# QizhiPei/FABind

Measured on AMD Instinct MI355X. Metric: complexes/sec fwd+bwd (1500p/40l nodes), full IaBNet on the whole graph (pocket model + 4-layer complex model + distance-map head on all nodes / pairs) with the pocket-cls + pocket-centre + coord + distmap + distmap-by-coords + distill losses (BASELINE configs[2] read literally), higher is better.
Workload: dtype bf16

## Files before the change

### fabind_amd/_lib.py

```python
import ctypes
import os

import torch

from . import config as _cfg

_HERE = os.path.dirname(os.path.abspath(__file__))
LIB_PATH = _cfg.knob("FABIND_LIB") or os.path.join(_HERE, "libfabind_hip.so")

ABI_VERSION = 19
DT_F32, DT_BF16 = 0, 1
ACT_NONE, ACT_SILU, ACT_RELU, ACT_SIGMOID, ACT_STORED_DERIV = 0, 1, 2, 3, 4
GEMM_FAM_NT_F32, GEMM_FAM_NT_F32_BF16, GEMM_FAM_NT_BF16, GEMM_FAM_GLDS, GEMM_FAM_PIPE, GEMM_FAM_X3, GEMM_FAM_X3_PRO, GEMM_FAM_PERSIST = range(8)

LNR_8S16, LNR_8S32, LNR_V8_1, LNR_V8_2, LNR_V8_3, LNR_V8_4, LNR_S2, LNR_S8, LNR_S16, LNR_S32, LNR_COUNT = range(11)
LNB_8S16, LNB_8S32, LNB_V8_1, LNB_V8_2, LNB_V8_3, LNB_S2, LNB_S8, LNB_S16, LNB_S20, LNB_S32, LNB_COUNT = range(11)
RST_BF16_1, RST_BF16_2, RST_BF16_4, RST_GENERIC, RST_COUNT = range(5)
ELF_WAVE1, ELF_WAVE1_TAIL, ELF_WAVE2_TAIL, ELF_CHUNK, ELF_COUNT = range(5)
ELB_NPL1, ELB_NPL2, ELB_NPL3, ELB_COUNT = range(4)

_vp, _i, _f, _l = ctypes.c_void_p, ctypes.c_int, ctypes.c_float, ctypes.c_long


class GemmArgs(ctypes.Structure):
    _fields_ = [(n, _vp) for n in ("A", "A2", "W", "C", "bias", "R", "r_index", "dotvec", "dot_out", "aux", "groups", "C2")] + \
               [(n, _i) for n in ("M", "N", "K", "K1", "lda", "lda2", "ldw", "ldc", "ldr", "ldaux", "dot_ld",
                                  "a_dtype", "w_dtype", "c_dtype", "aux_dtype", "act_pro", "act_epi", "dact_epi",
                                  "accumulate", "store_preact", "n_groups", "max_m", "max_n", "groups_ext", "epi_fast", "k_splits")] + \
               [("alpha", _f), ("p_drop", _f), ("drop_seed", ctypes.c_uint)] + \
               [(n, _vp) for n in ("row_mu", "row_rs", "col_c", "C16")] + [("ldc16", _i), ("split3", _i), ("r_dtype", _i), ("c2_bf16", _i)]


class EdgeBwdArgs(ctypes.Structure):
    _fields_ = [(n, _vp) for n in ("AB", "row", "col", "rhohat", "w_r", "W2p", "Wcp", "W2Tp", "WcTp", "b2", "bc", "w3", "ds",
                                  "dagg", "S1", "Mm", "dT", "dP2", "dP1", "drh", "dABrow", "part", "dbg", "bnd", "d2scratch")] + \
               [(n, _i) for n in ("ldab", "lddagg", "lddab", "E")] + [("p_drop", _f), ("seed", ctypes.c_uint), ("xcd_aware", _i), ("lddab16", _i), ("dAB16", _vp),
                                                                  ("d2f", _vp), ("z3f", _vp)]


class PairUpdateArgs(ctypes.Structure):
    _fields_ = [(n, _vp) for n in ("T", "p_node", "c_node", "z_in", "z_out", "Wop", "bo", "ln_w", "ln_b", "W1p", "b1", "W2p", "b2",
                                  "Wbp", "bb", "bias_out")] + \
               [(n, _i) for n in ("ldt", "b_off", "n_pairs")] + [("eps", _f), ("p_drop", _f), ("seed", ctypes.c_uint)]


class TnJob(ctypes.Structure):
    _fields_ = [(n, _vp) for n in ("Y", "X", "C_part", "out", "out_tail")] + \
               [(n, _i) for n in ("ldy", "ldx", "M", "N", "E", "splits", "e_per", "n_tiles", "with_colsum", "out_dt", "ldo",
                                  "wg0", "n_wg", "blk0", "n_blk", "pad_")]


class AttnFusedBwdArgs(ctypes.Structure):
    _fields_ = [(n, _vp) for n in ("qg", "kv", "a0", "bo", "boT", "toff", "koff", "bconst", "desc", "desc_p", "out", "lse", "dout",
                                  "dqg", "dkv", "dO", "Dv", "da0", "acat", "colpart", "part")] + \
               [(n, _i) for n in ("ldq", "ldkv", "lda0", "ldda0", "ldacat", "kcol0", "ldcolpart", "kp")] + [("scale", _f)] + \
               [(n, _i) for n in ("nsplit", "B", "part_rows")]


class AdamRow(ctypes.Structure):
    _fields_ = [(n, _vp) for n in ("p", "g", "m", "v")] + [("numel", ctypes.c_longlong), ("chunk0", _i), ("step_idx", _i)] + \
               [(n, ctypes.c_double) for n in ("lr", "beta1", "beta2", "eps", "weight_decay")] + [("decoupled", _i), ("pad_", _i)]


SIGNATURES = {
    "fabind_gemm": [ctypes.POINTER(GemmArgs), _vp],
    "fabind_gemm_plan": [ctypes.POINTER(GemmArgs), ctypes.POINTER(_i), ctypes.POINTER(_i), ctypes.POINTER(_i)],
    "fabind_gemm_tn_multi": [_vp, _vp, _i, _vp, _i, _vp, _i, _vp, _vp],
    "fabind_gemm_tn": [_vp, _i, _vp, _i, _vp, _i, _i, _i, _i, _vp, _vp, _i, _i, _vp],
    "fabind_transpose_act": [_vp, _i, _i, _vp, _i, _i, _i, _i, _i, _vp],
    "fabind_colsum": [_vp, _i, _i, _vp, _i, _i, _i, _vp, _i, _vp],
    "fabind_edges_count": [_vp, _vp, _vp, _i, _i, _vp, _vp, _f, _f, _vp, _vp, _vp],
    "fabind_edges_fill": [_vp, _vp, _vp, _i, _i, _vp, _vp, _vp, _f, _f, _vp, _vp, _vp, _vp, _vp, _vp, _vp],
    "fabind_exclusive_scan": [_vp, _vp, _i, _vp],
    "fabind_inter_meta": [_vp, _vp, _i, _vp, _vp, _vp, _i, _vp, _vp, _vp, _vp, _vp, _vp],
    "fabind_edge_geom": [_vp, _vp, _vp, _vp, _vp, _i, _vp, _vp, _vp, _vp, _vp],
    "fabind_gcl_pre": [_vp, _i, _i, _i, _vp, _vp, _vp, _vp, _vp, _i, _i, _i, _vp, _vp],
    "fabind_gcl_edge_fused": [_vp, _i, _i, _vp, _vp, _vp, _vp, _vp, _vp, _vp, _vp, _vp, _i, _vp, _vp, _f, ctypes.c_uint, _vp, _vp, _vp],
    "fabind_gcl_edge_fused_train": [_vp, _i, _i, _vp, _vp, _vp, _vp, _vp, _vp, _vp, _vp, _vp, _i, _vp, _vp, _f, ctypes.c_uint, _vp, _vp, _vp, _vp, _vp, _vp],
    "fabind_gcl_edge_fused_x3": [_vp, _i, _i, _i, _vp, _vp, _vp, _vp, _vp, _vp, _vp, _vp, _vp, _vp, _vp, _i, _vp, _vp, _f, ctypes.c_uint, _vp, _vp],
    "fabind_gcl_edge_fused_x3_train": [_vp, _i, _i, _i, _vp, _vp, _vp, _vp, _vp, _vp, _vp, _vp, _vp, _vp, _vp, _i, _vp, _vp, _f, ctypes.c_uint, _vp, _vp, _vp, _vp, _vp],
    "fabind_gcl_edge_fused_bwd": [ctypes.POINTER(EdgeBwdArgs), _i, _i, _vp],
    "fabind_pair_update_fused": [ctypes.POINTER(PairUpdateArgs), _i, _vp],
    "fabind_gcl_edge_fused_bwd_set_tile": [_i],
    "fabind_gcl_edge_fused_bwd_tile": [],
    "fabind_gcl_edge_fused_bwd_set_variant": [_i],
    "fabind_gcl_edge_fused_set_variant": [_i],
    "fabind_gcl_edge_fused_variant": [],
    "fabind_gcl_edge_fused_bwd_variant": [],
    "fabind_gcl_edge_fused_bwd_variant_for": [_i],
    "fabind_row_stats": [_vp, _i, _i, _f, _i, _i, _vp, _vp, _vp],
    "fabind_layernorm_rows": [_vp, _i, _i, _vp, _vp, _f, _i, _i, _vp, _i, _i, _i, _vp],
    "fabind_edge_ln_concat": [_vp, _i, _i, _vp, _vp, _vp, _vp, _vp, _f, _i, _vp, _i, _i, _i, _vp],
    "fabind_edge_lnfold": [_vp, _i, _i, _i, _vp, _vp, _vp, _vp, _f, _vp, _vp, _vp, _vp, _i, _vp, _f, ctypes.c_uint, _vp],
    "fabind_edge_lnfold_bwd_blocks": [_i],
    "fabind_edge_lnfold_bwd": [_vp, _i, _i, _i, _vp, _vp, _vp, _vp, _f, _vp, _vp, _vp, _vp, _vp, _i, _f, _vp, _vp, _vp, _vp, _i, _vp],
    "fabind_layernorm_rows_form": [_vp, _i, _i, _vp, _i, _i],
    "fabind_layernorm_rows_bwd_form": [_vp, _i, _vp, _i, _vp, _i, _i],
    "fabind_row_stats_form": [_vp, _i, _i, _i],
    "fabind_edge_lnfold_form": [_i, _i, ctypes.POINTER(_i)],
    "fabind_edge_lnfold_blocks": [_i],
    "fabind_edge_lnfold_bwd_form": [_i, ctypes.POINTER(_i)],
    "fabind_inter_coord_fold_blocks": [_i],
    "fabind_inter_coord_fold": [_vp, _i, _i, _vp, _vp, _vp, _f, _f, _vp, _vp, _vp, _i, _vp, _f, ctypes.c_uint, _vp],
    "fabind_post_optimize": [_vp, _vp, _vp, _vp, _vp, _i, _i, _i, _i, _f, _vp, _vp, _vp, _vp],
    "fabind_distmap_generate": [_vp, _vp, _vp, _vp, _vp, _vp, _vp, _vp, _vp, _vp, _i, _i, _i, _i, _i, _i, _l, _i, _i, _i, _i,
                                _vp, _vp, _vp, _vp, _vp, _vp, _vp, _vp],
    "fabind_sym_automorphisms": [_vp, _vp, _vp, _vp, _i, _i, _i, _vp, _vp, _vp, _vp, _vp, _vp],
    "fabind_sym_score": [_vp, _i, _i, _vp, _vp, _vp, _vp, _vp, _i, _i, _vp, _vp, _vp, _vp, _vp, _vp],
    "fabind_pose_stats": [_vp, _vp, _vp, _i, _vp, _vp, _vp],
    "fabind_rank_loss_fwd": [_vp, _vp, _vp, _i, _i, _i, _vp, _vp, _vp, _vp],
    "fabind_multi_copy": [_vp, _i, _i, _vp],
    "fabind_adam_chunk": [],
    "fabind_multi_sqnorm": [_vp, _i, _i, _vp, _vp, _vp, _vp],
    "fabind_multi_adam": [_vp, _i, _i, _vp, _vp, _vp, _f, _i, _vp, _vp, _vp],
    "fabind_zero_empty_rows": [_vp, _i, _vp, _i, _i, _i, _vp, _i, _i, _vp],
    "fabind_split_sum": [_vp, _i, ctypes.c_long, _vp, _i, ctypes.c_long, _vp, _vp],
    "fabind_segment_sum": [_vp, _i, _i, _i, _vp, _vp, _i, _i, _i, _vp, _i, _vp, _i, _vp],
    "fabind_coord_update": [_vp, _vp, _vp, _i, _vp, _vp, _i, _i, _f, _vp, _vp, _vp],
    "fabind_cross_attn_fwd": [_vp, _i, _vp, _vp, _i, _vp, _i, _vp, _i, _i, _i, _vp, _i, _i, _f, _vp, _i, _vp, _i, _vp, _i,
                              _vp],
    "fabind_cross_attn_mfma_fwd": [_vp, _i, _vp, _vp, _i, _vp, _i, _vp, _i, _i, _i, _vp, _i, _i, _f, _vp, _i, _vp, _i, _vp, _i,
                                   _vp],
    "fabind_cross_attn_fused_fwd": [_vp, _i, _vp, _vp, _i, _vp, _i, _vp, _i, _vp, _vp, _vp, _vp, _i, _i, _i, _i, _i, _f, _vp, _i, _vp, _i, _vp, _vp],
    "fabind_cross_attn_fused_bwd": [ctypes.POINTER(AttnFusedBwdArgs), _i, _i, _i, _i, _i, _i, _vp],
    "fabind_pair_bot_pack": [_vp, _i, _vp, _i, _vp, _vp, _vp, _vp, _i, _vp, _i, _l, _vp],
    "fabind_pair_bo_pack": [_vp, _i, _vp, _i, _vp, _vp, _vp, _vp, _i, _vp, _i, _l, _vp],
    "fabind_cross_attn_mfma_bwd": [_vp, _i, _vp, _i, _vp, _i, _i, _i, _vp, _i, _i, _i, _f, _vp, _vp, _vp, _vp, _vp, _vp, _vp,
                                   _vp, _vp, _vp],
    "fabind_pair_bmat": [_vp, _i, _vp, _i, _i, _vp, _i, _vp, _i, _vp],
    "fabind_pair_hadamard": [_vp, _vp, _i, _i, _vp, _vp, _i, _i, _vp, _vp, _i, _vp, _i, _i, _vp],
    "fabind_inter_attn_fwd": [_vp, _i, _vp, _i, _i, _vp, _i, _vp, _vp, _vp, _vp, _vp, _vp, _vp, _i, _vp, _vp, _vp,
                              _vp, _f, _i, _vp, _vp, _vp, _vp, _vp, _vp, _vp],
    "fabind_inter_attn_fwd_rows": [_vp, _i, _vp, _i, _i, _vp, _i, _vp, _vp, _vp, _vp, _vp, _vp, _vp, _i, _vp, _vp, _vp,
                                   _vp, _f, _i, _vp, _vp, _vp, _vp, _vp, _vp, _vp, _i, _i, _vp],
    "fabind_layernorm_rows_bwd": [_vp, _i, _i, _vp, _vp, _i, _i, _f, _i, _i, _vp, _i, _i, _vp, _vp, _i, _vp],
    "fabind_edge_concat": [_vp, _i, _i, _vp, _vp, _vp, _i, _vp, _i, _i, _i, _vp],
    "fabind_las_step": [_vp, _vp, _vp, _vp, _vp, _vp, _vp, _i, _i, _f, _f, _vp, _vp, _vp],
    "fabind_select_rows": [_vp, _vp, _vp, _i, _i, _vp, _vp],
    "fabind_add": [_vp, _vp, _vp, _l, _vp],
    "fabind_mul_dact": [_vp, _i, _vp, _i, _i, _vp, _i, _l, _f, _vp],
    "fabind_mul_dact_colsum": [_vp, _i, _vp, _i, _i, _vp, _i, _i, _i, _vp, _vp, _i, _f, _vp],
    "fabind_drop_mix": [_vp, _vp, _vp, _l, _f, ctypes.c_uint, _vp],
    "fabind_drop_mix_bwd": [_vp, _vp, _vp, _l, _f, ctypes.c_uint, _vp],
    "fabind_mul_dropmask_colsum": [_vp, _i, _vp, _i, _i, _i, _f, ctypes.c_uint, _vp, _vp, _i, _vp],
    "fabind_rowdot_bwd": [_vp, _i, _vp, _i, _vp, _i, _i, _i, _vp, _vp, _vp, _i, _vp],
    "fabind_edge_geom_bwd": [_vp, _vp, _vp, _vp, _vp, _vp, _vp, _vp, _vp, _vp, _i, _i, _i, _vp, _vp, _vp, _vp],
    "fabind_gcl_pre_bwd": [_vp, _i, _i, _vp, _vp, _i, _vp, _vp, _vp, _i, _vp],
    "fabind_gather_dact": [_vp, _i, _vp, _vp, _i, _i, _vp, _i, _i, _i, _vp],
    "fabind_coord_update_bwd": [_vp, _vp, _vp, _i, _i, _f, _vp, _vp, _vp, _vp],
    "fabind_cross_attn_bwd": [_vp, _i, _vp, _i, _vp, _i, _i, _i, _vp, _i, _i, _i, _f, _vp, _vp, _vp, _vp, _vp, _vp, _vp,
                              _vp, _vp, _vp],
    "fabind_pair_bias_cat": [_vp, _i, _vp, _i, _i, _i, _vp, _i, _vp, _i, _vp, _vp, _i, _vp, _i, _vp, _vp],
    "fabind_batched_transpose_pad": [_vp, _i, _vp, _i, _i, _i, _i, _vp, _vp],
    "fabind_node_chain_fwd": [_vp, _i, _vp, _i, _vp, _vp, _vp, _vp, _vp, _vp, _i, _i, _vp, _i, _vp, _i, _vp, _i, _i, _i, _vp],
    "fabind_node_chain_x3_fwd": [_vp, _i, _vp, _i, _vp, _vp, _vp, _vp, _vp, _vp, _vp, _vp, _vp, _vp, _i, _i, _vp, _i, _vp, _i, _vp, _i, _vp, _i, _vp, _i,
                                 _i, _i, _vp],
    "fabind_rows_hadamard_bwd": [_vp, _i, _i, _vp, _i, _i, _vp, _vp, _vp, _i, _vp, _i, _vp],
    "fabind_pair_hadamard_bwd_grid": [_vp, _i, _i, _vp, _i, _i, _vp, _vp, _vp, _vp, _i, _vp, _i, _vp],
    "fabind_pair_hadamard_bwd_rows": [_vp, _i, _i, _vp, _i, _i, _vp, _i, _i, _vp, _vp, _vp, _vp, _i, _vp, _i, _vp, _i, _vp],
    "fabind_pair_hadamard_bwd": [_vp, _i, _i, _vp, _vp, _i, _i, _vp, _vp, _i, _i, _vp, _vp, _i, _vp, _vp, _i, _vp, _vp, _i,
                                 _vp],
    "fabind_inter_attn_bwd": [_vp, _i, _vp, _i, _i, _vp, _vp, _vp, _vp, _vp, _vp, _vp, _vp, _vp, _vp, _vp, _vp, _f, _i,
                              _vp, _vp, _vp, _vp, _vp, _vp, _vp, _vp, _vp, _vp, _i, _vp],
    "fabind_inter_attn_bwd_rows": [_vp, _i, _vp, _i, _i, _vp, _vp, _vp, _vp, _vp, _vp, _vp, _vp, _vp, _vp, _vp, _vp, _f, _i,
# ... 104 lines not shown
```

### fabind_amd/csrc/fused_common.h

```cpp
#pragma once
#include "common.h"

#define FE_BM 64
#define FE_PRIO(x) __builtin_amdgcn_s_setprio(x)

__device__ __forceinline__ float fe_sigmoid(float x) { return __builtin_amdgcn_rcpf(1.0f + __builtin_amdgcn_exp2f(-1.44269504f * x)); }
__device__ __forceinline__ float fe_silu(float x) { return x * fe_sigmoid(x); }

__device__ __forceinline__ uint32_t fe_hash(uint32_t x) {
    x ^= x >> 16; x *= 0x7feb352dU; x ^= x >> 15; x *= 0x846ca68bU; x ^= x >> 16;
    return x;
}
__device__ __forceinline__ float fe_keep(uint32_t seed, uint32_t e, uint32_t c, uint32_t H, uint32_t thr16, float scale) {
    const uint32_t h = fe_hash(seed + (e >> 1) * H + c);
    return (((e & 1u) ? (h >> 16) : (h & 0xffffu)) >= thr16) ? scale : 0.f;
}

__device__ __forceinline__ void unpack8(const uint4 u, float* f) {
    f[0] = __uint_as_float(u.x << 16); f[1] = __uint_as_float(u.x & 0xffff0000u);
    f[2] = __uint_as_float(u.y << 16); f[3] = __uint_as_float(u.y & 0xffff0000u);
    f[4] = __uint_as_float(u.z << 16); f[5] = __uint_as_float(u.z & 0xffff0000u);
    f[6] = __uint_as_float(u.w << 16); f[7] = __uint_as_float(u.w & 0xffff0000u);
}
__device__ __forceinline__ uint4 pack8(const float* f) {
// ... 279 lines not shown
__device__ __forceinline__ float fe_scan_runs64(const bf16_t* sX, const int* sRow, const float* sRh, int ne, bool head_cont,
                                                bool tail_cont, float* out, unsigned ld, float* bnd_tile, int c,
                                                bf16_t* out16 = nullptr, unsigned ld16 = 0, const bf16_t* sXlo = nullptr) {
    const int lane = threadIdx.x & 63;
    const int mine = sRow[lane], prev = sRow[max(lane - 1, 0)];
    const float rhl = WITH_RH ? sRh[lane] : 0.f;
    const unsigned long long m = __ballot(lane < ne && lane > 0 && mine != prev);
    const int c8 = c >> 3, c7 = c & 7;
    float v[64];
#pragma unroll
    for (int rw = 0; rw < 64; ++rw) v[rw] = bf16_to_f32(sX[rw * H + ((c8 ^ (rw & SWZ)) * 8) + c7]);
    if (sXlo) {
#pragma unroll
        for (int rw = 0; rw < 64; ++rw) v[rw] += bf16_to_f32(sXlo[rw * H + ((c8 ^ (rw & SWZ)) * 8) + c7]);
    }
    float run = 0.f, pwr = 0.f;
    int rs = 0;
    auto flush = [&](bool last) {
        if (rs == 0 && head_cont) bnd_tile[c] = run;
        else if (last && tail_cont) bnd_tile[H + c] = run;
        else {
            const unsigned node = (unsigned)__builtin_amdgcn_readlane(mine, rs);
            if (out) out[node * ld + c] = run;
            if (out16) out16[node * ld16 + c] = f32_to_bf16(run);
        }
    };
#pragma unroll
    for (int rw = 0; rw < 64; ++rw) {
        if (rw < ne) {
            if ((m >> rw) & 1ull) {
                flush(false);
                run = 0.f;
                rs = rw;
            }
            run += v[rw];
            if (WITH_RH) pwr += __builtin_bit_cast(float, __builtin_amdgcn_readlane(__builtin_bit_cast(int, rhl), rw)) * v[rw];
        }
    }
    if (ne > 0) flush(true);
    return pwr;
}

template <int BM>
__global__ void fe_boundary_fix_kernel(const int* __restrict__ row, int E, int H, const float* __restrict__ bnd, float* out,
                                       unsigned ld, bf16_t* out16 = nullptr, unsigned ld16 = 0) {
    const int t = blockIdx.x, e0 = t * BM, ne = min(BM, E - e0);
    if (ne <= 0 || e0 + ne >= E) return;
    const int r = row[e0 + ne - 1];
    if (row[e0 + ne] != r) return;
    if (row[e0] == r && e0 > 0 && row[e0 - 1] == r) return;
    for (int c = threadIdx.x; c < H; c += blockDim.x) {
        float sum = bnd[((size_t)t * 2 + 1) * H + c];
        for (int u = t + 1;; ++u) {
            const int f0 = u * BM, fn = min(BM, E - f0);
            sum += bnd[((size_t)u * 2) * H + c];
            const bool through = row[f0 + fn - 1] == r && f0 + fn < E && row[f0 + fn] == r;
            if (!through) break;
        }
        if (out) out[(unsigned)r * ld + c] = sum;
        if (out16) out16[(unsigned)r * ld16 + c] = f32_to_bf16(sum);
    }
}

__device__ __forceinline__ float fe3_row16_sum(float v) {
#define FE_DPP_ADD(ctrl_) v += __builtin_bit_cast(float, __builtin_amdgcn_update_dpp(0, __builtin_bit_cast(int, v), (ctrl_), 0xF, 0xF, true))
    FE_DPP_ADD(0xB1);
    FE_DPP_ADD(0x4E);
    FE_DPP_ADD(0x141);
    FE_DPP_ADD(0x140);
#undef FE_DPP_ADD
    return v;
}

typedef float fe_f2 __attribute__((ext_vector_type(2)));
__device__ __forceinline__ void fe3_silu_pair(const fe_f2 z, fe_f2& m, fe_f2& d) {
    const fe_f2 t = z * -1.44269504f;
    const fe_f2 o = fe_f2{__builtin_amdgcn_exp2f(t.x), __builtin_amdgcn_exp2f(t.y)} + 1.0f;
    const fe_f2 s = fe_f2{__builtin_amdgcn_rcpf(o.x), __builtin_amdgcn_rcpf(o.y)};
    m = z * s;
    d = s + (m - m * s);
}
__device__ __forceinline__ uint32_t fe3_pack(const fe_f2 v) { return pack2_bf16(v.x, v.y); }
__device__ __forceinline__ fe_f2 fe3_unpack(const uint32_t u) { return fe_f2{__uint_as_float(u << 16), __uint_as_float(u & 0xffff0000u)}; }

__device__ __forceinline__ uint4 fe3_bload16(const __amdgpu_buffer_rsrc_t rs, const unsigned voff, const unsigned soff) {
    const fe_u32x4_t v = __builtin_amdgcn_raw_buffer_load_b128(rs, (int)voff, (int)soff, 0);
    return make_uint4(v.x, v.y, v.z, v.w);
}
__device__ __forceinline__ void fe3_bstore16(const __amdgpu_buffer_rsrc_t rs, const unsigned voff, const unsigned soff, const uint4 v) {
    __builtin_amdgcn_raw_buffer_store_b128(fe_u32x4_t{v.x, v.y, v.z, v.w}, rs, (int)voff, (int)soff, 0);
}

struct FabindEdgeBwdArgs;
int fe_bwd3_launch(const FabindEdgeBwdArgs* a, int H, int bm, int n_groups, hipStream_t stream);
int fe_fwd3_launch(const float* AB, int ldab, int H, const int* row, const int* col, const float* rhohat, const float* w_r,
                   const void* W2ph, const void* W2pl, const float* b2, const void* Wcph, const void* Wcpl, const float* bc,
                   const float* w3, int E, float* agg, float* s_out, uint32_t thr16, float dscale, unsigned seed, float* bnd,
                   int xcd_aware, hipStream_t stream, void* Msave = nullptr, void* d2f = nullptr, void* z3f = nullptr);
int fe_fwd2_launch(const void* AB, int ldab, int H, const int* row, const int* col, const float* rhohat, const float* w_r,
                   const void* W2p, const float* b2, const void* Wcp, const float* bc, const float* w3, int E, float* agg,
                   float* s_out, uint32_t thr16, float dscale, unsigned seed, float* bnd, void* agg16, int xcd_aware, hipStream_t stream,
                   void* Msave = nullptr, void* d2f = nullptr, void* z3f = nullptr);
int fe_bwd4_launch(const FabindEdgeBwdArgs* a, int H, int n_groups, hipStream_t stream);
```

### fabind_amd/csrc/fused_edge.hip

```cpp
#include "common.h"
#include "fabind_hip.h"
#include "fused_common.h"

static int g_fe_xcd_aware = 1;
extern "C" void fabind_gcl_edge_fused_set_xcd_aware(int on) { g_fe_xcd_aware = on ? 1 : 0; }
static int g_fe_fwd_variant = 1;
extern "C" int fabind_gcl_edge_fused_set_variant(int v) {
    FB_REQUIRE(v == 1, "fabind_gcl_edge_fused_set_variant: 1 (row-wise / operand-swapped) is the only forward form built (variant 0 was retired in round 5)");
    g_fe_fwd_variant = v;
    return 0;
}
extern "C" int fabind_gcl_edge_fused_variant(void) { return g_fe_fwd_variant; }

static int fe_fwd_entry(const void* AB, int ldab, int H, const int* row, const int* col, const float* rhohat,
                        const float* w_r, const void* W2p, const float* b2, const void* Wcp, const float* bc,
                        const float* w3, int E, float* agg, float* s_out, float p_drop, unsigned seed,
                        float* bnd, void* agg16, void* Msave, void* d2f, void* z3f, hipStream_t stream) {
    if (E <= 0) return 0;
    FB_REQUIRE((Msave != nullptr) == (d2f != nullptr) && (Msave != nullptr) == (z3f != nullptr),
               "fabind_gcl_edge_fused_train: M, d2f and z3f come together");
    FB_REQUIRE(Msave == nullptr || g_fe_fwd_variant == 1, "fabind_gcl_edge_fused_train: the saving forward is the row-wise / operand-swapped kernel (variant 1)");
    FB_REQUIRE(bnd != nullptr, "fabind_gcl_edge_fused: bnd (ceil(E/64) x 2 x H floats of scratch) is required");
    FB_REQUIRE(p_drop >= 0.f && p_drop < 1.f, "fabind_gcl_edge_fused: p_drop in [0, 1)");
    const uint32_t thr16 = (uint32_t)(p_drop * 65536.0f + 0.5f);
    const float dscale = 1.0f / (1.0f - (float)thr16 / 65536.0f);
    FB_REQUIRE(H == 512 || H == 256 || H == 128 || H == 64, "fabind_gcl_edge_fused: H must be 64, 128, 256 or 512");
    FB_REQUIRE(ldab % 8 == 0, "fabind_gcl_edge_fused: ldab % 8");
    {
        const int rc = fe_fwd2_launch(AB, ldab, H, row, col, rhohat, w_r, W2p, b2, Wcp, bc, w3, E, agg, s_out, thr16, dscale, seed, bnd,
                                      agg16, g_fe_xcd_aware, stream, Msave, d2f, z3f);
        if (rc) return rc;
    }
    hipLaunchKernelGGL((fe_boundary_fix_kernel<FE_BM>), dim3((E + FE_BM - 1) / FE_BM), dim3(H < 256 ? H : 256), 0, stream, row, E, H,
                       bnd, agg, (unsigned)H, (bf16_t*)agg16, (unsigned)H);
    FB_CHECK_LAUNCH();
    return 0;
}

extern "C" int fabind_gcl_edge_fused(const void* AB, int ldab, int H, const int* row, const int* col, const float* rhohat,
                                     const float* w_r, const void* W2p, const float* b2, const void* Wcp, const float* bc,
                                     const float* w3, int E, float* agg, float* s_out, float p_drop, unsigned seed,
                                     float* bnd, void* agg16, hipStream_t stream) {
    return fe_fwd_entry(AB, ldab, H, row, col, rhohat, w_r, W2p, b2, Wcp, bc, w3, E, agg, s_out, p_drop, seed, bnd, agg16, nullptr, nullptr,
                        nullptr, stream);
}
extern "C" int fabind_gcl_edge_fused_train(const void* AB, int ldab, int H, const int* row, const int* col, const float* rhohat,
                                           const float* w_r, const void* W2p, const float* b2, const void* Wcp, const float* bc,
                                           const float* w3, int E, float* agg, float* s_out, float p_drop, unsigned seed,
                                           float* bnd, void* agg16, void* M, void* d2f, void* z3f, hipStream_t stream) {
    FB_REQUIRE(M != nullptr && d2f != nullptr && z3f != nullptr, "fabind_gcl_edge_fused_train: M, d2f, z3f are required");
    return fe_fwd_entry(AB, ldab, H, row, col, rhohat, w_r, W2p, b2, Wcp, bc, w3, E, agg, s_out, p_drop, seed, bnd, agg16, M, d2f, z3f, stream);
}

static int fe_x3_entry(const float* AB, int ldab, int n_rows, int H, const int* row, const int* col, const float* rhohat,
                       const float* w_r, const void* W2ph, const void* W2pl, const float* b2, const void* Wcph,
                       const void* Wcpl, const float* bc, const float* w3, int E, float* agg, float* s_out,
                       float p_drop, unsigned seed, float* bnd, void* Msave, void* d2f, void* z3f, hipStream_t stream) {
    if (E <= 0) return 0;
    FB_REQUIRE(bnd != nullptr, "fabind_gcl_edge_fused_x3: bnd (ceil(E/64) x 2 x H floats of scratch) is required");
    FB_REQUIRE(p_drop >= 0.f && p_drop < 1.f, "fabind_gcl_edge_fused_x3: p_drop in [0, 1)");
    FB_REQUIRE(H == 512 || H == 256 || H == 128 || H == 64, "fabind_gcl_edge_fused_x3: H must be 64, 128, 256 or 512");
    FB_REQUIRE(ldab % 4 == 0 && ((uintptr_t)AB & 15) == 0, "fabind_gcl_edge_fused_x3: AB must be 16-byte aligned with ldab % 4 == 0");
    FB_REQUIRE(n_rows >= 0 && (size_t)n_rows * (size_t)ldab * 4 < ((size_t)1 << 32), "fabind_gcl_edge_fused_x3: AB larger than 4 GiB (n_rows * ldab * 4 bytes): split the batch");
    const uint32_t thr16 = (uint32_t)(p_drop * 65536.0f + 0.5f);
    const float dscale = 1.0f / (1.0f - (float)thr16 / 65536.0f);
    const int rc = fe_fwd3_launch(AB, ldab, H, row, col, rhohat, w_r, W2ph, W2pl, b2, Wcph, Wcpl, bc, w3, E, agg, s_out, thr16, dscale,
                                  seed, bnd, g_fe_xcd_aware, stream, Msave, d2f, z3f);
    if (rc) return rc;
    hipLaunchKernelGGL((fe_boundary_fix_kernel<FE_BM>), dim3((E + FE_BM - 1) / FE_BM), dim3(H < 256 ? H : 256), 0, stream, row, E, H,
                       bnd, agg, (unsigned)H, (bf16_t*)nullptr, 0u);
    FB_CHECK_LAUNCH();
    return 0;
}
extern "C" int fabind_gcl_edge_fused_x3(const float* AB, int ldab, int n_rows, int H, const int* row, const int* col, const float* rhohat,
                                        const float* w_r, const void* W2ph, const void* W2pl, const float* b2, const void* Wcph,
                                        const void* Wcpl, const float* bc, const float* w3, int E, float* agg, float* s_out,
                                        float p_drop, unsigned seed, float* bnd, hipStream_t stream) {
    return fe_x3_entry(AB, ldab, n_rows, H, row, col, rhohat, w_r, W2ph, W2pl, b2, Wcph, Wcpl, bc, w3, E, agg, s_out, p_drop, seed, bnd,
                       nullptr, nullptr, nullptr, stream);
}
extern "C" int fabind_gcl_edge_fused_x3_train(const float* AB, int ldab, int n_rows, int H, const int* row, const int* col, const float* rhohat,
                                              const float* w_r, const void* W2ph, const void* W2pl, const float* b2, const void* Wcph,
                                              const void* Wcpl, const float* bc, const float* w3, int E, float* agg, float* s_out,
                                              float p_drop, unsigned seed, float* bnd, void* M, void* d2f, void* z3f, hipStream_t stream) {
    FB_REQUIRE(M != nullptr && d2f != nullptr && z3f != nullptr, "fabind_gcl_edge_fused_x3_train: M, d2f, z3f are required");
    return fe_x3_entry(AB, ldab, n_rows, H, row, col, rhohat, w_r, W2ph, W2pl, b2, Wcph, Wcpl, bc, w3, E, agg, s_out, p_drop, seed, bnd,
                       M, d2f, z3f, stream);
}

template <int H, int BM, bool DBG>
__global__ __launch_bounds__(H, (BM == 32 ? 4 : 2)) void gcl_edge_fused_bwd_kernel(const FabindEdgeBwdArgs p) {
    constexpr int TPE = H / BM;
    constexpr int CPT = BM / 8;
    constexpr int MI = BM / 16;
    extern __shared__ __attribute__((aligned(16))) unsigned char smem[];
    bf16_t* sX = (bf16_t*)smem;
    bf16_t* sY = sX + BM * H;
    int* sRow = (int*)(sY + BM * H);
    float* sDs = (float*)(sRow + BM);
    float* sRh = sDs + BM;
    const bf16_t* __restrict__ AB = (const bf16_t*)p.AB;
    const int tid = threadIdx.x, lane = tid & 63, wave = tid >> 6;
    const int fr = lane & 15, cq = lane >> 4;
    const int el = tid / TPE, cth = tid % TPE;
    const int n_tiles = (p.E + BM - 1) / BM;
    const uint32_t thr16 = (uint32_t)(p.p_drop * 65536.0f + 0.5f);
    const float dscale = 1.0f / (1.0f - (float)thr16 / 65536.0f);
    int cbase[2][2];
#pragma unroll
    for (int f0 = 0; f0 < 2; ++f0)
#pragma unroll
        for (int f2 = 0; f2 < 2; ++f2)
            cbase[f0][f2] = cq * 4 * H + (wave * 8 + (((cq & 1) ^ f2) << 2) + ((fr >> 3) ^ f0)) * 8 + (fr & 7);
#define FE_COFF(i, j, r) (cbase[(r) & 1][(j) >> 1] + ((i) * 16 + (r)) * H + ((((j) & 1) ^ ((r) >> 1)) * 16))
    long long tph[12] = {0, 0, 0, 0, 0, 0, 0, 0, 0, 0, 0, 0};
    long long tlast = 0;
#define FE_TICK(k_)                                                   \
    if constexpr (DBG) {                                              \
        const long long now_ = __builtin_readcyclecounter();         \
        tph[k_] += now_ - tlast;                                      \
        tlast = now_;                                                 \
    }
    float pb2[4] = {0.f, 0.f, 0.f, 0.f}, pbc[4] = {0.f, 0.f, 0.f, 0.f}, pw3[4] = {0.f, 0.f, 0.f, 0.f}, pwr = 0.f;

    uint4 pfa[CPT], pfb[CPT];
    const unsigned uld = (unsigned)p.ldab;
    auto fe_prefetch = [&](unsigned r, unsigned c) {
        const unsigned aoff = r * uld + cth * (CPT * 8), boff = c * uld + H + cth * (CPT * 8);
#pragma unroll
        for (int q = 0; q < CPT; ++q) {
            pfa[q] = *(const uint4*)(AB + (aoff + q * 8));
            pfb[q] = *(const uint4*)(AB + (boff + q * 8));
        }
    };
    int t_first, t_end, t_step;
    if (p.xcd_aware && (gridDim.x & 7) == 0) {
        const int tpx = (n_tiles + 7) / 8, xcd = blockIdx.x & 7;
        t_first = xcd * tpx + (int)(blockIdx.x >> 3);
        t_end = min(n_tiles, (xcd + 1) * tpx);
        t_step = (int)(gridDim.x >> 3);
    } else {
        t_first = blockIdx.x; t_end = n_tiles; t_step = gridDim.x;
    }
    unsigned ur = 0, uc = 0;
    if (t_first < t_end) {
        const int e0 = t_first * BM;
        if (el < min(BM, p.E - e0)) {
            ur = (unsigned)(p.row + e0)[(unsigned)el];
            uc = (unsigned)(p.col + e0)[(unsigned)el];
        }
    }
    fe_prefetch(ur, uc);

    for (int tile = t_first; tile < t_end; tile += t_step) {
        const int e0 = tile * BM;
        const int ne = min(BM, p.E - e0);
        int lz = 0;
        asm volatile("" : "+s"(lz));
        const float* w_r = p.w_r + lz;
        const float* b2 = p.b2 + lz;
        const float* bc = p.bc + lz;
        const float* w3 = p.w3 + lz;
        const bf16_t* W2p = (const bf16_t*)p.W2p + lz;
        const bf16_t* Wcp = (const bf16_t*)p.Wcp + lz;
        const bf16_t* W2Tp = (const bf16_t*)p.W2Tp + lz;
        const bf16_t* WcTp = (const bf16_t*)p.WcTp + lz;
        if constexpr (DBG) tlast = __builtin_readcyclecounter();
        const int* grow = p.row + e0;
        const int* gcol = p.col + e0;
        const float* grh = p.rhohat + e0;
// ... 171 lines not shown
                unpack8(pfa[q], fa);
                unpack8(pfb[q], fb);
                uint4* sp = (uint4*)&sX[el * H + (((cth * CPT + q) ^ (el & 7)) * 8)];
                unpack8(*sp, g);
                const float4 w0 = *(const float4*)(wp + q * 8), w1 = *(const float4*)(wp + q * 8 + 4);
                const float wv[8] = {w0.x, w0.y, w0.z, w0.w, w1.x, w1.y, w1.z, w1.w};
#pragma unroll
                for (int k = 0; k < 8; ++k) {
                    const float z = fa[k] + fb[k] + rh * wv[k], sg = fe_sigmoid(z);
                    g[k] *= sg * (1.0f + z * (1.0f - sg));
                    dot += g[k] * wv[k];
                }
                *sp = pack8(g);
            }
#pragma unroll
            for (int o = 1; o < TPE; o <<= 1) dot += __shfl_xor(dot, o, 64);
            if (cth == 0) (p.drh + e0)[(unsigned)el] = dot;
        }
        ur = nr; uc = nc;
        fe_prefetch(ur, uc);
        __syncthreads();
        FE_TICK(8)
        fe_tile_store<H>(sX, (bf16_t*)p.dP1, e0, ne, tid);
        FE_TICK(1)

        {
            const bool head_cont = e0 > 0 && p.row[e0 - 1] == sRow[0];
            const bool tail_cont = e0 + ne < p.E && p.row[e0 + ne] == sRow[ne - 1];
            pwr += fe_scan_rows<H, true, BM>(sX, sRow, sRh, ne, head_cont, tail_cont, p.dABrow, (unsigned)p.lddab,
                                             p.bnd + (size_t)tile * 2 * H, tid);
        }
        __syncthreads();
        FE_TICK(9)
    }
    if constexpr (DBG) {
        if (p.dbg && blockIdx.x == 0 && tid == 0)
            for (int k = 0; k < 12; ++k) ((long long*)p.dbg)[k] = tph[k];
    }

    float* part = p.part + (size_t)blockIdx.x * 4 * H;
#pragma unroll
    for (int j = 0; j < 4; ++j) {
        float a = pb2[j], b = pbc[j], c = pw3[j];
        a += __shfl_xor(a, 16, 64); a += __shfl_xor(a, 32, 64);
        b += __shfl_xor(b, 16, 64); b += __shfl_xor(b, 32, 64);
        c += __shfl_xor(c, 16, 64); c += __shfl_xor(c, 32, 64);
        if (cq == 0) {
            const int colj = wave * 64 + j * 16 + fr;
            part[colj] = a; part[H + colj] = b; part[2 * H + colj] = c;
        }
    }
    part[3 * H + tid] = pwr;
}

#undef FE_COFF
#undef FE_ROT4
#undef FE_ROT_ACC
#undef FE_ROT_D2
#undef FE_JADDR
#undef FE_LOFF
#undef FE_TICK

static int g_fe_bwd_bm = 64;
extern "C" int fabind_gcl_edge_fused_bwd_set_tile(int bm) {
    FB_REQUIRE(bm == 64, "fabind_gcl_edge_fused_bwd_set_tile: 64 edges per tile (the 32-edge build of the two-tile kernel was retired in round 5)");
    g_fe_bwd_bm = bm;
    return 0;
}
extern "C" int fabind_gcl_edge_fused_bwd_tile(void) { return g_fe_bwd_bm; }
static bool g_fe_bwd_variant_set = false;
static int g_fe_bwd_variant = 5;
extern "C" int fabind_gcl_edge_fused_bwd_set_variant(int v) {
    FB_REQUIRE(v == 0 || v == 5,
               "fabind_gcl_edge_fused_bwd_set_variant: 0 (two LDS tiles of 64 edges: the default for H <= 128) or 5 (row-wise, operand-swapped in-place tile + store wave: the recompute default above); variants 1-4 were knobs nobody reached and were retired in round 5");
    g_fe_bwd_variant = v;
    g_fe_bwd_variant_set = true;
    return 0;
}
extern "C" int fabind_gcl_edge_fused_bwd_variant(void) { return g_fe_bwd_variant; }
extern "C" int fabind_gcl_edge_fused_bwd_variant_for(int H) {
    return (!g_fe_bwd_variant_set && g_fe_bwd_variant == 5 && H <= 128) ? 0 : g_fe_bwd_variant;
}

extern "C" int fabind_gcl_edge_fused_bwd(const FabindEdgeBwdArgs* a_in, int H, int n_groups, hipStream_t stream) {
    FabindEdgeBwdArgs a_copy = *a_in;
    a_copy.xcd_aware = g_fe_xcd_aware;
    const FabindEdgeBwdArgs* a = &a_copy;
    if (a->E <= 0 || n_groups <= 0) return 0;
    FB_REQUIRE(H == 512 || H == 256 || H == 128 || H == 64, "fabind_gcl_edge_fused_bwd: H must be 64, 128, 256 or 512");
    FB_REQUIRE(a->ldab % 8 == 0, "fabind_gcl_edge_fused_bwd: ldab % 8");
    FB_REQUIRE(a->p_drop >= 0.f && a->p_drop < 1.f, "fabind_gcl_edge_fused_bwd: p_drop in [0, 1)");
    const int g_fe_bwd_variant = fabind_gcl_edge_fused_bwd_variant_for(H);
    if (a->d2f != nullptr || a->z3f != nullptr) {
        FB_REQUIRE(a->d2f != nullptr && a->z3f != nullptr, "fabind_gcl_edge_fused_bwd: d2f and z3f (saved by fabind_gcl_edge_fused_train) come together");
        return fe_bwd4_launch(a, H, n_groups, stream);
    }
    if (g_fe_bwd_variant == 5) return fe_bwd3_launch(a, H, 64, n_groups, stream);
    FB_REQUIRE(a->dAB16 == nullptr, "fabind_gcl_edge_fused_bwd: dAB16 (bf16 receiving-side sums) exists in variant 5 only");
    FB_REQUIRE(a->bnd != nullptr, "fabind_gcl_edge_fused_bwd: bnd (ceil(E / tile) x 2 x H floats of scratch) is required");
    const int BMr = g_fe_bwd_bm;
    const size_t lds = (size_t)2 * BMr * H * 2 + BMr * (sizeof(int) + 2 * sizeof(float));
#define FE_LAUNCH2(HH, BB)                                                                                         \
    do {                                                                                                           \
        static bool set_ = false;                                                                                  \
        if (!set_) { (void)hipFuncSetAttribute((const void*)gcl_edge_fused_bwd_kernel<HH, BB, false>, hipFuncAttributeMaxDynamicSharedMemorySize, (int)lds); set_ = true; } \
        hipLaunchKernelGGL((gcl_edge_fused_bwd_kernel<HH, BB, false>), dim3(n_groups), dim3(HH), lds, stream, *a);  \
    } while (0)
#define FE_LAUNCH(HH) FE_LAUNCH2(HH, 64)
    if (a->dbg != nullptr && H == 512) {
        static bool setd_ = false;
        if (!setd_) { (void)hipFuncSetAttribute((const void*)gcl_edge_fused_bwd_kernel<512, 64, true>, hipFuncAttributeMaxDynamicSharedMemorySize, (int)lds); }
        hipLaunchKernelGGL((gcl_edge_fused_bwd_kernel<512, 64, true>), dim3(n_groups), dim3(512), lds, stream, *a);
    } else
    if (H == 512) FE_LAUNCH(512); else if (H == 256) FE_LAUNCH(256); else if (H == 128) FE_LAUNCH(128); else FE_LAUNCH(64);
    hipLaunchKernelGGL((fe_boundary_fix_kernel<64>), dim3((a->E + 63) / 64), dim3(H < 256 ? H : 256), 0, stream, a->row, a->E, H,
                           a->bnd, a->dABrow, (unsigned)a->lddab);
#undef FE_LAUNCH
#undef FE_LAUNCH2
#undef FE_COFF
#undef FE_ROT4
#undef FE_ROT_ACC
#undef FE_ROT_D2
#undef FE_JADDR
#undef FE_LOFF
#undef FE_TICK
    FB_CHECK_LAUNCH();
    return 0;
}
```

### fabind_amd/csrc/fused_edge_bwd4.hip

```cpp
#include "common.h"
#include "fabind_hip.h"
#include "fused_common.h"

#ifndef FE4_E3_DB
#define FE4_E3_DB 0
#endif
#ifndef FE4_SCAN64
#define FE4_SCAN64 0
#endif
#ifndef FE4_P5_BATCH
#define FE4_P5_BATCH 4
#endif

#ifndef FE4_NT_LOADS
#define FE4_NT_LOADS 1
#endif
#if FE4_NT_LOADS
typedef unsigned fe_u32x2_nt_t __attribute__((ext_vector_type(2)));
__device__ __forceinline__ uint2 fe4_ldq(const bf16_t* p_) { const fe_u32x2_nt_t v = __builtin_nontemporal_load((const fe_u32x2_nt_t*)p_); return make_uint2(v.x, v.y); }
#else
__device__ __forceinline__ uint2 fe4_ldq(const bf16_t* p_) { return *(const uint2*)p_; }
#endif

template <int H>
__global__ __launch_bounds__(H, 4) void gcl_edge_fused_bwd4_kernel(const FabindEdgeBwdArgs p, const int xf) {
    constexpr int BM = FE_BM, MI = BM / 16;
    constexpr int NW = H / 64;
    constexpr int CH = H / 8;
    constexpr int EPW = 64 / CH;
    constexpr int EPI = NW * EPW;
    constexpr int NIT = BM / EPI;
    constexpr int SWZ = (H >= 128) ? 15 : 7;
    static_assert(BM <= H, "one thread per table row");
    extern __shared__ __attribute__((aligned(16))) unsigned char smem[];
    bf16_t* sX = (bf16_t*)smem;
    int* sTab = (int*)(sX + BM * H);
    float* sPart = (float*)(sTab + 8 * BM);
    const int tid = threadIdx.x, lane = tid & 63, wave = tid >> 6;
    const int fr = lane & 15, cq = lane >> 4;
    const int sub = lane / CH, ch = lane % CH;
    const int n_tiles = (p.E + BM - 1) / BM;
    int t_first, t_end, t_step;
    if (p.xcd_aware && (gridDim.x & 7) == 0) {
        const int tpx = (n_tiles + 7) / 8, xcd = blockIdx.x & 7;
        t_first = xcd * tpx + (int)(blockIdx.x >> 3);
        t_end = min(n_tiles, (xcd + 1) * tpx);
        t_step = (int)(gridDim.x >> 3);
    } else {
        t_first = blockIdx.x; t_end = n_tiles; t_step = gridDim.x;
    }
    for (int k = 0; k < 4; ++k) sPart[k * H + tid] = 0.f;
    const unsigned uld = (unsigned)p.ldab;
    const __amdgpu_buffer_rsrc_t rs_ab = fe_rsrc(const_cast<void*>(p.AB), 0xffffffffu);
    const __amdgpu_buffer_rsrc_t rs_dagg = fe_rsrc(const_cast<float*>(p.dagg), 0xffffffffu);
    const bf16_t* __restrict__ d2f = (const bf16_t*)p.d2f;
    const bf16_t* __restrict__ z3f = (const bf16_t*)p.z3f;
    const int cx = (wave * 8 + (cq >> 1)) ^ (fr & SWZ);
    const int lbase = fr * H + (cq & 1) * 4;
#define FE_OPAQUE(v_) asm volatile("" : "+v"(v_))
#define FE_QOFF(i, j) (lb_ + (i) * 16 * H + ((cx_ ^ ((j) * 2)) * 8))
#define FE_FOFF(i, j) (fbase + (size_t)((i) * 4 + (j)) * 256)
    const int fcol = wave * 64 + cq * 4;

    int tb_r = -1, tb_c = 0;
    float tb_d = 0.f, tb_h = 0.f;
    auto fetch_tables = [&](int tile) {
        const int e0 = tile * BM;
        const int ne = min(BM, p.E - e0);
        if (tid < BM) {
            const bool ok = tid < ne;
            const unsigned ge = (unsigned)(e0 + (ok ? tid : 0));
            const int r = p.row[ge], c = p.col[ge];
            const float d = p.ds[ge], h = p.rhohat[ge];
            tb_r = ok ? r : -1; tb_c = ok ? c : 0; tb_d = ok ? d : 0.f; tb_h = ok ? h : 0.f;
        }
    };
    auto commit_tables = [&](int hb) {
        int* tb = sTab + hb * 4 * BM;
        if (tid < BM) {
            tb[tid] = tb_r;
            tb[BM + tid] = tb_c;
            ((float*)tb)[2 * BM + tid] = tb_d;
            ((float*)tb)[3 * BM + tid] = tb_h;
        }
    };
    if (t_first < t_end) { fetch_tables(t_first); commit_tables(0); }
    __syncthreads();
    int hb = 0;

    for (int tile = t_first; tile < t_end; tile += t_step, hb ^= 1) {
        const int e0 = tile * BM;
        const int ne = min(BM, p.E - e0);
        const int* sRow = sTab + hb * 4 * BM;
        const int* sCol = sRow + BM;
        const float* sDs = (const float*)(sRow + 2 * BM);
        const float* sRh = (const float*)(sRow + 3 * BM);
        int lz = 0;
        asm volatile("" : "+s"(lz));
        const float* w_r = p.w_r + lz;
        const float* w3 = p.w3 + lz;
        const bf16_t* W2Tp = (const bf16_t*)p.W2Tp + lz;
        const bf16_t* WcTp = (const bf16_t*)p.WcTp + lz;
        int ln_ = lane;
        FE_OPAQUE(ln_);
        const size_t fbase = (((size_t)tile * NW + wave) * (MI * 4) * 64 + ln_) * 4;
        auto copy_out = [&](void* dst) {
            const __amdgpu_buffer_rsrc_t rs = fe_rsrc((bf16_t*)dst + (size_t)e0 * H, (unsigned)ne * H * 2);
            int t_ = tid;
            FE_OPAQUE(t_);
#pragma unroll
            for (int it = 0; it < BM * CH / H; ++it) {
                const int q = t_ + it * H;
                const int rw = q / CH, c8 = q % CH;
                const uint4 v = *(const uint4*)&sX[rw * H + ((c8 ^ (rw & SWZ)) * 8)];
                __builtin_amdgcn_raw_buffer_store_b128(fe_u32x4_t{v.x, v.y, v.z, v.w}, rs, (int)((rw * H + c8 * 8) * 2), 0,  2);
            }
        };

        {
            int cx_ = cx, lb_ = lbase;
            FE_OPAQUE(cx_); FE_OPAQUE(lb_);
            uint2 zq[4][MI];
#pragma unroll
            for (int j = 0; j < 4; ++j)
#pragma unroll
                for (int i = 0; i < MI; ++i) zq[j][i] = fe4_ldq(&z3f[FE_FOFF(i, j)]);
            float dsr[MI];
#pragma unroll
            for (int i = 0; i < MI; ++i) dsr[i] = sDs[i * 16 + fr];
            float4 wq4[4];
#pragma unroll
            for (int j = 0; j < 4; ++j) wq4[j] = *(const float4*)(w3 + fcol + j * 16);
#pragma unroll
            for (int j = 0; j < 4; ++j) {
                const fe_f2 w01 = fe_f2{wq4[j].x, wq4[j].y}, w23 = fe_f2{wq4[j].z, wq4[j].w};
                fe_f2 a3a = fe_f2{0.f, 0.f}, a3b = a3a, aca = a3a, acb = a3a;
#pragma unroll
                for (int i = 0; i < MI; ++i) {
                    fe_f2 m01, d01, m23, d23;
                    fe3_silu_pair(fe3_unpack(zq[j][i].x), m01, d01);
                    fe3_silu_pair(fe3_unpack(zq[j][i].y), m23, d23);
                    const fe_f2 t01 = (w01 * dsr[i]) * d01, t23 = (w23 * dsr[i]) * d23;
                    a3a += m01 * dsr[i]; a3b += m23 * dsr[i];
                    aca += t01; acb += t23;
                    *(uint2*)&sX[FE_QOFF(i, j)] = make_uint2(fe3_pack(t01), fe3_pack(t23));
                }
                float a3[4] = {a3a.x, a3a.y, a3b.x, a3b.y}, ac[4] = {aca.x, aca.y, acb.x, acb.y};
#pragma unroll
                for (int r = 0; r < 4; ++r) { a3[r] = fe3_row16_sum(a3[r]); ac[r] = fe3_row16_sum(ac[r]); }
                if (fr < 4) {
                    const float va = fr == 0 ? a3[0] : fr == 1 ? a3[1] : fr == 2 ? a3[2] : a3[3];
                    const float vc = fr == 0 ? ac[0] : fr == 1 ? ac[1] : fr == 2 ? ac[2] : ac[3];
                    sPart[2 * H + fcol + j * 16 + fr] += va;
                    sPart[1 * H + fcol + j * 16 + fr] += vc;
                }
                __builtin_amdgcn_sched_barrier(0);
            }
        }
        __syncthreads();

        if (!(xf & 1)) copy_out(p.dT);
        f32x4_t acc[MI][4];
        fe_zero(acc);
        if (!(xf & 8)) fe_gemm_rolled<H, MI, true, SWZ>(sX, WcTp, wave, lane, acc);
        __syncthreads();

        {
            int cx_ = cx, lb_ = lbase;
            FE_OPAQUE(cx_); FE_OPAQUE(lb_);
            float4 dg[FE4_E3_DB ? 2 : 1][MI];
            uint2 dq[FE4_E3_DB ? 2 : 1][MI];
            unsigned dgo[MI];
            float dgk[MI];
#pragma unroll
            for (int i = 0; i < MI; ++i) {
                const int rr = sRow[i * 16 + fr];
                dgk[i] = rr >= 0 ? 1.f : 0.f;
                dgo[i] = ((unsigned)max(rr, 0) * (unsigned)p.lddagg + fcol) * 4;
            }
            auto fetch_block = [&](int j, int slot) {
#pragma unroll
                for (int i = 0; i < MI; ++i) {
                    const uint4 v = fe3_bload16(rs_dagg, dgo[i], (unsigned)(j * 64));
                    dg[slot][i] = make_float4(__uint_as_float(v.x), __uint_as_float(v.y), __uint_as_float(v.z), __uint_as_float(v.w));
                    dq[slot][i] = fe4_ldq(&d2f[FE_FOFF(i, j)]);
                }
            };
            if (FE4_E3_DB) fetch_block(0, 0);
#pragma unroll
            for (int j = 0; j < 4; ++j) {
                if (FE4_E3_DB) { if (j < 3) fetch_block(j + 1, (j + 1) & 1); } else fetch_block(j, 0);
                fe_f2 a2a = fe_f2{0.f, 0.f}, a2b = a2a;
#pragma unroll
                for (int i = 0; i < MI; ++i) {
                    const float4 g4 = dg[FE4_E3_DB ? (j & 1) : 0][i];
                    const uint2 dd = dq[FE4_E3_DB ? (j & 1) : 0][i];
                    const fe_f2 p01 = (fe_f2{acc[i][j][0], acc[i][j][1]} + fe_f2{g4.x, g4.y} * dgk[i]) * fe3_unpack(dd.x);
                    const fe_f2 p23 = (fe_f2{acc[i][j][2], acc[i][j][3]} + fe_f2{g4.z, g4.w} * dgk[i]) * fe3_unpack(dd.y);
                    a2a += p01; a2b += p23;
                    *(uint2*)&sX[FE_QOFF(i, j)] = make_uint2(fe3_pack(p01), fe3_pack(p23));
                }
                float a2[4] = {a2a.x, a2a.y, a2b.x, a2b.y};
#pragma unroll
                for (int r = 0; r < 4; ++r) a2[r] = fe3_row16_sum(a2[r]);
                if (fr < 4) sPart[fcol + j * 16 + fr] += fr == 0 ? a2[0] : fr == 1 ? a2[1] : fr == 2 ? a2[2] : a2[3];
                __builtin_amdgcn_sched_barrier(0);
            }
        }
        __syncthreads();

        if (!(xf & 1)) copy_out(p.dP2);
        fe_zero(acc);
        if (!(xf & 8)) fe_gemm_rolled<H, MI, true, SWZ>(sX, W2Tp, wave, lane, acc);
        __syncthreads();
        {
            int cx_ = cx, lb_ = lbase;
            FE_OPAQUE(cx_); FE_OPAQUE(lb_);
#pragma unroll
            for (int j = 0; j < 4; ++j)
#pragma unroll
                for (int i = 0; i < MI; ++i)
                    *(uint2*)&sX[FE_QOFF(i, j)] = make_uint2(pack2_bf16(acc[i][j][0], acc[i][j][1]), pack2_bf16(acc[i][j][2], acc[i][j][3]));
        }
        __syncthreads();

        const bool has_next = tile + t_step < t_end;
        {
            int ch_ = ch, es_ = wave * EPW + sub;
            FE_OPAQUE(ch_); FE_OPAQUE(es_);
#define ch ch_
            fe_f2 wv2[4];
            {
                const float4 w0 = *(const float4*)(w_r + ch * 8), w1 = *(const float4*)(w_r + ch * 8 + 4);
                wv2[0] = fe_f2{w0.x, w0.y}; wv2[1] = fe_f2{w0.z, w0.w}; wv2[2] = fe_f2{w1.x, w1.y}; wv2[3] = fe_f2{w1.z, w1.w};
            }
            const __amdgpu_buffer_rsrc_t rs_s1 = fe_rsrc((bf16_t*)p.S1 + (size_t)e0 * H, (unsigned)ne * H * 2);
            const __amdgpu_buffer_rsrc_t rs_p1 = fe_rsrc((bf16_t*)p.dP1 + (size_t)e0 * H, (unsigned)ne * H * 2);
            constexpr int PB = (NIT % FE4_P5_BATCH == 0) ? FE4_P5_BATCH : NIT;
#pragma unroll
            for (int u0 = 0; u0 < NIT; u0 += PB) {
            uint4 ga[PB], gb[PB];
#pragma unroll
            for (int v = 0; v < PB; ++v) {
                const int e = (u0 + v) * EPI + es_;
                const unsigned r = (unsigned)max(sRow[e], 0), c = (unsigned)sCol[e];
                ga[v] = fe3_bload16(rs_ab, (r * uld + ch * 8) * 2, 0);
                gb[v] = fe3_bload16(rs_ab, (c * uld + H + ch * 8) * 2, 0);
            }
#pragma unroll
            for (int v = 0; v < PB; ++v) {
                const int u = v;
                const int e = (u0 + v) * EPI + es_;
                const float rh = sRh[e];
                uint4* sp = (uint4*)&sX[e * H + ((ch ^ (e & SWZ)) * 8)];
                const uint4 gs = *sp;
                const uint32_t ua[4] = {ga[u].x, ga[u].y, ga[u].z, ga[u].w}, ub[4] = {gb[u].x, gb[u].y, gb[u].z, gb[u].w};
                const uint32_t ug[4] = {gs.x, gs.y, gs.z, gs.w};
                uint32_t po[4], pg[4];
                fe_f2 dot2 = fe_f2{0.f, 0.f};
#pragma unroll
                for (int k = 0; k < 4; ++k) {
                    const fe_f2 z = fe3_unpack(ua[k]) + fe3_unpack(ub[k]) + wv2[k] * rh;
                    fe_f2 m, d;
                    fe3_silu_pair(z, m, d);
                    const fe_f2 g = fe3_unpack(ug[k]) * d;
                    dot2 += g * wv2[k];
                    po[k] = fe3_pack(m);
                    pg[k] = fe3_pack(g);
                }
                *sp = make_uint4(pg[0], pg[1], pg[2], pg[3]);
                const unsigned goff = (unsigned)(e * H + ch * 8) * 2;
                if (!(xf & 2)) {
                    __builtin_amdgcn_raw_buffer_store_b128(fe_u32x4_t{po[0], po[1], po[2], po[3]}, rs_s1, (int)goff, 0,  2);
                    __builtin_amdgcn_raw_buffer_store_b128(fe_u32x4_t{pg[0], pg[1], pg[2], pg[3]}, rs_p1, (int)goff, 0,  2);
                }
                float dot = dot2.x + dot2.y;
                if constexpr (CH >= 16) {
                    dot = fe3_row16_sum(dot);
#pragma unroll
                    for (int o = 16; o < CH; o <<= 1) dot += __shfl_xor(dot, o, 64);
                } else {
#pragma unroll
                    for (int o = 1; o < CH; o <<= 1) dot += __shfl_xor(dot, o, 64);
                }
                if (ch == 0 && e < ne) (p.drh + e0)[(unsigned)e] = dot;
            }
            }
#undef ch
        }
        __syncthreads();

        if (has_next) fetch_tables(tile + t_step);
        if (!(xf & 4)) {
            const bool head_cont = e0 > 0 && p.row[e0 - 1] == sRow[0];
            const bool tail_cont = e0 + ne < p.E && p.row[e0 + ne] == sRow[ne - 1];
#if FE4_SCAN64
            sPart[3 * H + tid] += fe_scan_runs64<H, true, SWZ>(sX, sRow, sRh, ne, head_cont, tail_cont, p.dAB16 ? nullptr : p.dABrow, (unsigned)p.lddab,
                                                              p.bnd + (size_t)tile * 2 * H, tid, (bf16_t*)p.dAB16, (unsigned)p.lddab16);
#else
            sPart[3 * H + tid] += fe_scan_rows<H, true, BM, SWZ>(sX, sRow, sRh, ne, head_cont, tail_cont, p.dAB16 ? nullptr : p.dABrow, (unsigned)p.lddab,
                                                                p.bnd + (size_t)tile * 2 * H, tid, (bf16_t*)p.dAB16, (unsigned)p.lddab16);
#endif
        }
        if (has_next) commit_tables(hb ^ 1);
        __syncthreads();
    }
    __syncthreads();
    float* part = p.part + (size_t)blockIdx.x * 4 * H;
    for (int k = 0; k < 4; ++k) part[k * H + tid] = sPart[k * H + tid];
#undef FE_QOFF
#undef FE_FOFF
#undef FE_OPAQUE
}

static int g_fe_bwd4_exp = 0;
extern "C" void fabind_gcl_edge_fused_bwd4_set_exp(int m) { g_fe_bwd4_exp = m; }

int fe_bwd4_launch(const FabindEdgeBwdArgs* a, int H, int n_groups, hipStream_t stream) {
    FB_REQUIRE(a->bnd != nullptr, "fabind_gcl_edge_fused_bwd: bnd (ceil(E / 64) x 2 x H floats of scratch) is required");
    FB_REQUIRE(a->lddagg % 4 == 0 && ((uintptr_t)a->dagg & 15) == 0, "fabind_gcl_edge_fused_bwd: dagg must be 16-byte aligned with lddagg % 4 == 0");
    const size_t lds = (size_t)FE_BM * H * 2 + (size_t)8 * FE_BM * sizeof(int) + (size_t)4 * H * sizeof(float);
#define FE_LAUNCH4(HH)                                                                                                \
    do {                                                                                                           \
        static bool set_ = false;                                                                                  \
        if (!set_) {                                                                                               \
            const hipError_t e_ = hipFuncSetAttribute((const void*)gcl_edge_fused_bwd4_kernel<HH>,                    \
                                                      hipFuncAttributeMaxDynamicSharedMemorySize, (int)lds);       \
            if (e_ != hipSuccess) { fabind_set_error(hipGetErrorString(e_)); return (int)e_; }                     \
            set_ = true;                                                                                           \
        }                                                                                                          \
        hipLaunchKernelGGL((gcl_edge_fused_bwd4_kernel<HH>), dim3(n_groups), dim3(HH), lds, stream, *a, g_fe_bwd4_exp); \
    } while (0)
    if (H == 512) FE_LAUNCH4(512); else if (H == 256) FE_LAUNCH4(256); else if (H == 128) FE_LAUNCH4(128); else FE_LAUNCH4(64);
#undef FE_LAUNCH4
    hipLaunchKernelGGL((fe_boundary_fix_kernel<64>), dim3((a->E + 63) / 64), dim3(H < 256 ? H : 256), 0, stream, a->row, a->E, H,
                       a->bnd, a->dAB16 ? nullptr : a->dABrow, (unsigned)a->lddab, (bf16_t*)a->dAB16, (unsigned)a->lddab16);
    FB_CHECK_LAUNCH();
    return 0;
}
```

### fabind_amd/csrc/fused_edge_fwd2.hip

```cpp
#include "common.h"
#include "fabind_hip.h"
#include "fused_common.h"

typedef float fw_f2 __attribute__((ext_vector_type(2)));
__device__ __forceinline__ fw_f2 fw_silu_pair(const fw_f2 z) {
    const fw_f2 t = z * -1.44269504f;
    const fw_f2 o = fw_f2{__builtin_amdgcn_exp2f(t.x), __builtin_amdgcn_exp2f(t.y)} + 1.0f;
    return z * fw_f2{__builtin_amdgcn_rcpf(o.x), __builtin_amdgcn_rcpf(o.y)};
}
__device__ __forceinline__ uint32_t fw_pack(const fw_f2 v) { return pack2_bf16(v.x, v.y); }
__device__ __forceinline__ fw_f2 fw_unpack(const uint32_t u) { return fw_f2{__uint_as_float(u << 16), __uint_as_float(u & 0xffff0000u)}; }

__device__ __forceinline__ void fw_silu_pair_d(const fw_f2 z, fw_f2& m, fw_f2& d) {
    const fw_f2 t = z * -1.44269504f;
    const fw_f2 o = fw_f2{__builtin_amdgcn_exp2f(t.x), __builtin_amdgcn_exp2f(t.y)} + 1.0f;
    const fw_f2 s = fw_f2{__builtin_amdgcn_rcpf(o.x), __builtin_amdgcn_rcpf(o.y)};
    m = z * s;
    d = s + (m - m * s);
}

#ifndef FW2_NT_SAVE
#define FW2_NT_SAVE 1
#endif
typedef unsigned fw_u32x2_t __attribute__((ext_vector_type(2)));
__device__ __forceinline__ void fw_stq(bf16_t* p_, uint32_t a, uint32_t b) {
#if FW2_NT_SAVE
    __builtin_nontemporal_store(fw_u32x2_t{a, b}, (fw_u32x2_t*)p_);
#else
    *(uint2*)p_ = make_uint2(a, b);
#endif
}

template <int H, bool DROP, bool SAVE>
__global__ __launch_bounds__(H, 4) void gcl_edge_fused2_kernel(const bf16_t* __restrict__ AB, int ldab, const int* __restrict__ row,
                                                            const int* __restrict__ col, const float* __restrict__ rhohat,
                                                            const float* __restrict__ w_r, const bf16_t* __restrict__ W2p,
                                                            const float* __restrict__ b2, const bf16_t* __restrict__ Wcp,
                                                            const float* __restrict__ bc, const float* __restrict__ w3, int E,
                                                            float* agg, float* s_out, uint32_t thr16, float dscale,
                                                            uint32_t seed, float* bnd, bf16_t* agg16, int xcd_aware,
                                                            bf16_t* __restrict__ Msave, bf16_t* __restrict__ d2f, bf16_t* __restrict__ z3f) {
    constexpr int BM = FE_BM, MI = BM / 16;
    constexpr int NW = H / 64;
    constexpr int CH = H / 8;
    constexpr int EPW = 64 / CH;
    constexpr int EPI = NW * EPW;
    constexpr int NIT = BM / EPI;
    constexpr int SWZ = (H >= 128) ? 15 : 7;
    extern __shared__ __attribute__((aligned(16))) unsigned char smem[];
    bf16_t* sX = (bf16_t*)smem;
    int* sRow = (int*)(sX + BM * H);
    int* sCol = sRow + BM;
    float* sRh = (float*)(sCol + BM);
    float* sDot = sRh + BM;
    const int tid = threadIdx.x, lane = tid & 63, wave = tid >> 6;
    const int fr = lane & 15, cq = lane >> 4;
    const int sub = lane / CH, ch = lane % CH;
    const int n_tiles = (E + BM - 1) / BM, tpx = (n_tiles + 7) / 8;
    const int tile = xcd_aware ? (int)((blockIdx.x & 7) * tpx + (blockIdx.x >> 3)) : (int)blockIdx.x;
    if ((xcd_aware && (int)(blockIdx.x >> 3) >= tpx) || tile >= n_tiles) return;
    const int e0 = tile * BM;
    const int ne = min(BM, E - e0);

    if (tid < BM) {
        const bool ok = tid < ne;
        const unsigned ge = (unsigned)(e0 + (ok ? tid : 0));
        const int r = row[ge], c = col[ge];
        const float h = rhohat[ge];
        sRow[tid] = ok ? r : -1;
        sCol[tid] = ok ? c : 0;
        sRh[tid] = ok ? h : 0.f;
    }
    __syncthreads();

    {
        const __amdgpu_buffer_rsrc_t rs_ab = fe_rsrc(const_cast<bf16_t*>(AB), 0xffffffffu);
        fw_f2 wv2[4];
        {
            const float4 w0 = *(const float4*)(w_r + ch * 8), w1 = *(const float4*)(w_r + ch * 8 + 4);
            wv2[0] = fw_f2{w0.x, w0.y}; wv2[1] = fw_f2{w0.z, w0.w}; wv2[2] = fw_f2{w1.x, w1.y}; wv2[3] = fw_f2{w1.z, w1.w};
        }
        fe_u32x4_t ga[NIT], gb[NIT];
#pragma unroll
        for (int u = 0; u < NIT; ++u) {
            const int e = u * EPI + wave * EPW + sub;
            const unsigned r = (unsigned)max(sRow[e], 0), c = (unsigned)sCol[e];
            ga[u] = __builtin_amdgcn_raw_buffer_load_b128(rs_ab, (int)((r * (unsigned)ldab + ch * 8) * 2), 0, 0);
            gb[u] = __builtin_amdgcn_raw_buffer_load_b128(rs_ab, (int)((c * (unsigned)ldab + H + ch * 8) * 2), 0, 0);
        }
#pragma unroll
        for (int u = 0; u < NIT; ++u) {
            const int e = u * EPI + wave * EPW + sub;
            const float rh = sRh[e];
            uint32_t po[4];
#pragma unroll
            for (int k = 0; k < 4; ++k) po[k] = fw_pack(fw_silu_pair(fw_unpack(ga[u][k]) + fw_unpack(gb[u][k]) + wv2[k] * rh));
            *(uint4*)&sX[e * H + ((ch ^ (e & SWZ)) * 8)] = e < ne ? make_uint4(po[0], po[1], po[2], po[3]) : make_uint4(0u, 0u, 0u, 0u);
        }
    }
    __syncthreads();

    const int cx = (wave * 8 + (cq >> 1)) ^ (fr & SWZ);
    const int lbase = fr * H + (cq & 1) * 4;
#define FW_QOFF(i, j) (lbase + (i) * 16 * H + ((cx ^ ((j) * 2)) * 8))
    const size_t fbase = (((size_t)tile * NW + wave) * (MI * 4) * 64 + lane) * 4;
#define FW_FOFF(i, j) (fbase + (size_t)((i) * 4 + (j)) * 256)
    const int fcol = wave * 64 + cq * 4;

    f32x4_t acc[MI][4];
    fe_zero(acc);
    fe_gemm_rolled<H, MI, true, SWZ>(sX, W2p, wave, lane, acc);
    float4 bq4[4];
#pragma unroll
    for (int j = 0; j < 4; ++j) bq4[j] = *(const float4*)(b2 + fcol + j * 16);
    __syncthreads();
#pragma unroll
    for (int j = 0; j < 4; ++j) {
        const fw_f2 b01 = fw_f2{bq4[j].x, bq4[j].y}, b23 = fw_f2{bq4[j].z, bq4[j].w};
#pragma unroll
        for (int i = 0; i < MI; ++i) {
            fw_f2 m01, m23, d01, d23;
            if constexpr (SAVE) {
                fw_silu_pair_d(fw_f2{acc[i][j][0], acc[i][j][1]} + b01, m01, d01);
                fw_silu_pair_d(fw_f2{acc[i][j][2], acc[i][j][3]} + b23, m23, d23);
            } else {
                m01 = fw_silu_pair(fw_f2{acc[i][j][0], acc[i][j][1]} + b01);
                m23 = fw_silu_pair(fw_f2{acc[i][j][2], acc[i][j][3]} + b23);
            }
            if constexpr (DROP) {
                const uint32_t ee = (uint32_t)(e0 + i * 16 + fr), cc = (uint32_t)(fcol + j * 16);
                const fw_f2 k01 = fw_f2{fe_keep(seed, ee, cc, H, thr16, dscale), fe_keep(seed, ee, cc + 1, H, thr16, dscale)};
                const fw_f2 k23 = fw_f2{fe_keep(seed, ee, cc + 2, H, thr16, dscale), fe_keep(seed, ee, cc + 3, H, thr16, dscale)};
                m01 *= k01; m23 *= k23;
                if constexpr (SAVE) { d01 *= k01; d23 *= k23; }
            }
            *(uint2*)&sX[FW_QOFF(i, j)] = make_uint2(fw_pack(m01), fw_pack(m23));
            if constexpr (SAVE) fw_stq(&d2f[FW_FOFF(i, j)], fw_pack(d01), fw_pack(d23));
        }
        __builtin_amdgcn_sched_barrier(0);
    }
    __syncthreads();
    if constexpr (SAVE) {
        const __amdgpu_buffer_rsrc_t rs_m = fe_rsrc(Msave + (size_t)e0 * H, (unsigned)ne * H * 2);
#pragma unroll
        for (int q = tid; q < BM * CH; q += H) {
            const int rw = q / CH, c8 = q % CH;
            const uint4 v = *(const uint4*)&sX[rw * H + ((c8 ^ (rw & SWZ)) * 8)];
            __builtin_amdgcn_raw_buffer_store_b128(fe_u32x4_t{v.x, v.y, v.z, v.w}, rs_m, (int)((rw * H + c8 * 8) * 2), 0,  2);
        }
    }

    {
        const bool head_cont = e0 > 0 && row[e0 - 1] == sRow[0];
        const bool tail_cont = e0 + ne < E && row[e0 + ne] == sRow[ne - 1];
        (void)fe_scan_runs64<H, false, SWZ>(sX, sRow, nullptr, ne, head_cont, tail_cont, agg, (unsigned)H, bnd + (size_t)tile * 2 * H, tid, agg16, (unsigned)H);
    }

    fe_zero(acc);
    fe_gemm_rolled<H, MI, true, SWZ>(sX, Wcp, wave, lane, acc);
    {
        fw_f2 da[MI], db[MI];
#pragma unroll
        for (int i = 0; i < MI; ++i) { da[i] = fw_f2{0.f, 0.f}; db[i] = da[i]; }
#pragma unroll
        for (int j = 0; j < 4; ++j) {
            const float4 bq = *(const float4*)(bc + fcol + j * 16), wq = *(const float4*)(w3 + fcol + j * 16);
            const fw_f2 b01 = fw_f2{bq.x, bq.y}, b23 = fw_f2{bq.z, bq.w}, w01 = fw_f2{wq.x, wq.y}, w23 = fw_f2{wq.z, wq.w};
#pragma unroll
            for (int i = 0; i < MI; ++i) {
                const fw_f2 z01 = fw_f2{acc[i][j][0], acc[i][j][1]} + b01, z23 = fw_f2{acc[i][j][2], acc[i][j][3]} + b23;
                da[i] += fw_silu_pair(z01) * w01;
                db[i] += fw_silu_pair(z23) * w23;
                if constexpr (SAVE) fw_stq(&z3f[FW_FOFF(i, j)], fw_pack(z01), fw_pack(z23));
            }
            __builtin_amdgcn_sched_barrier(0);
        }
#pragma unroll
        for (int i = 0; i < MI; ++i) {
            float t = (da[i].x + da[i].y) + (db[i].x + db[i].y);
            t += __shfl_xor(t, 16, 64);
            t += __shfl_xor(t, 32, 64);
            if (cq == 0) sDot[wave * BM + i * 16 + fr] = t;
        }
    }
    __syncthreads();
    if (tid < ne) {
        float s = 0.f;
#pragma unroll
        for (int w = 0; w < NW; ++w) s += sDot[w * BM + tid];
        s_out[e0 + tid] = s;
    }
#undef FW_QOFF
#undef FW_FOFF
}

int fe_fwd2_launch(const void* AB, int ldab, int H, const int* row, const int* col, const float* rhohat, const float* w_r,
                   const void* W2p, const float* b2, const void* Wcp, const float* bc, const float* w3, int E, float* agg,
                   float* s_out, uint32_t thr16, float dscale, unsigned seed, float* bnd, void* agg16, int xcd_aware, hipStream_t stream,
                   void* Msave, void* d2f, void* z3f) {
    const dim3 grid((((E + FE_BM - 1) / FE_BM + 7) / 8) * 8);
    const size_t lds = (size_t)FE_BM * H * 2 + 3 * FE_BM * sizeof(int) + (size_t)(H / 64) * FE_BM * sizeof(float);
#define FW_LAUNCH_(HH, DD, SS)                                                                                       \
    do {                                                                                                           \
        static bool set_ = false;                                                                                  \
        if (!set_) { (void)hipFuncSetAttribute((const void*)gcl_edge_fused2_kernel<HH, DD, SS>, hipFuncAttributeMaxDynamicSharedMemorySize, (int)lds); set_ = true; } \
        hipLaunchKernelGGL((gcl_edge_fused2_kernel<HH, DD, SS>), grid, dim3(HH), lds, stream, (const bf16_t*)AB, ldab, row, col, rhohat, \
                           w_r, (const bf16_t*)W2p, b2, (const bf16_t*)Wcp, bc, w3, E, agg, s_out, thr16, dscale, \
                           (uint32_t)seed, bnd, (bf16_t*)agg16, xcd_aware, (bf16_t*)Msave, (bf16_t*)d2f, (bf16_t*)z3f); \
    } while (0)
#define FW_LAUNCH(HH)                                                                  \
    do {                                                                               \
        if (Msave) { if (thr16) FW_LAUNCH_(HH, true, true); else FW_LAUNCH_(HH, false, true); } \
        else { if (thr16) FW_LAUNCH_(HH, true, false); else FW_LAUNCH_(HH, false, false); }    \
    } while (0)
    if (H == 512) FW_LAUNCH(512); else if (H == 256) FW_LAUNCH(256); else if (H == 128) FW_LAUNCH(128); else FW_LAUNCH(64);
#undef FW_LAUNCH
#undef FW_LAUNCH_
    return 0;
}
```

### fabind_amd/csrc/fused_edge_fwd3.hip

```cpp
#include "common.h"
#include "fabind_hip.h"
#include "fused_common.h"

typedef float f3_f2 __attribute__((ext_vector_type(2)));
__device__ __forceinline__ f3_f2 f3_silu_pair(const f3_f2 z) {
    const f3_f2 t = z * -1.44269504f;
    const f3_f2 o = f3_f2{__builtin_amdgcn_exp2f(t.x), __builtin_amdgcn_exp2f(t.y)} + 1.0f;
    return z * f3_f2{__builtin_amdgcn_rcpf(o.x), __builtin_amdgcn_rcpf(o.y)};
}

__device__ __forceinline__ void f3_silu_pair_d(const f3_f2 z, f3_f2& m, f3_f2& d) {
    const f3_f2 t = z * -1.44269504f;
    const f3_f2 o = f3_f2{__builtin_amdgcn_exp2f(t.x), __builtin_amdgcn_exp2f(t.y)} + 1.0f;
    const f3_f2 s = f3_f2{__builtin_amdgcn_rcpf(o.x), __builtin_amdgcn_rcpf(o.y)};
    m = z * s;
    d = s + (m - m * s);
}
__device__ __forceinline__ uint32_t f3_pack(const f3_f2 v) { return pack2_bf16(v.x, v.y); }
typedef unsigned f3_u32x2_t __attribute__((ext_vector_type(2)));
__device__ __forceinline__ void f3_stq(bf16_t* p_, uint32_t a, uint32_t b) { __builtin_nontemporal_store(f3_u32x2_t{a, b}, (f3_u32x2_t*)p_); }

template <int H, bool DROP, bool SAVE>
__global__ __launch_bounds__(H, 2) void gcl_edge_fused_x3_kernel(const float* __restrict__ AB, int ldab, const int* __restrict__ row,
                                                              const int* __restrict__ col, const float* __restrict__ rhohat,
                                                              const float* __restrict__ w_r, const bf16_t* __restrict__ W2ph,
                                                              const bf16_t* __restrict__ W2pl, const float* __restrict__ b2,
                                                              const bf16_t* __restrict__ Wcph, const bf16_t* __restrict__ Wcpl,
                                                              const float* __restrict__ bc, const float* __restrict__ w3, int E,
                                                              float* agg, float* s_out, uint32_t thr16, float dscale, uint32_t seed,
                                                              float* bnd, int xcd_aware, bf16_t* __restrict__ Msave,
                                                              bf16_t* __restrict__ d2f, bf16_t* __restrict__ z3f) {
    constexpr int BM = FE_BM, MI = BM / 16;
    constexpr int NW = H / 64;
    constexpr int CH = H / 8;
    constexpr int EPW = 64 / CH;
    constexpr int EPI = NW * EPW;
    constexpr int NIT = BM / EPI;
    constexpr int PB = 4;
    constexpr int SWZ = (H >= 128) ? 15 : 7;
    extern __shared__ __attribute__((aligned(16))) unsigned char smem[];
    bf16_t* sXh = (bf16_t*)smem;
    bf16_t* sXl = sXh + BM * H;
    int* sRow = (int*)(sXl + BM * H);
    int* sCol = sRow + BM;
    float* sRh = (float*)(sCol + BM);
    float* sDot = sRh + BM;
    const int tid = threadIdx.x, lane = tid & 63, wave = tid >> 6;
    const int fr = lane & 15, cq = lane >> 4;
    const int sub = lane / CH, ch = lane % CH;
    const int n_tiles = (E + BM - 1) / BM, tpx = (n_tiles + 7) / 8;
    const int tile = xcd_aware ? (int)((blockIdx.x & 7) * tpx + (blockIdx.x >> 3)) : (int)blockIdx.x;
    if ((xcd_aware && (int)(blockIdx.x >> 3) >= tpx) || tile >= n_tiles) return;
    const int e0 = tile * BM;
    const int ne = min(BM, E - e0);

    if (tid < BM) {
        const bool ok = tid < ne;
        const unsigned ge = (unsigned)(e0 + (ok ? tid : 0));
        const int r = row[ge], c = col[ge];
        const float h = rhohat[ge];
        sRow[tid] = ok ? r : -1;
        sCol[tid] = ok ? c : 0;
        sRh[tid] = ok ? h : 0.f;
    }
    __syncthreads();

    {
        const __amdgpu_buffer_rsrc_t rs_ab = fe_rsrc(const_cast<float*>(AB), 0xffffffffu);
        float wv[8];
        {
            const float4 w0 = *(const float4*)(w_r + ch * 8), w1 = *(const float4*)(w_r + ch * 8 + 4);
            wv[0] = w0.x; wv[1] = w0.y; wv[2] = w0.z; wv[3] = w0.w; wv[4] = w1.x; wv[5] = w1.y; wv[6] = w1.z; wv[7] = w1.w;
        }
#pragma unroll
        for (int b0 = 0; b0 < NIT; b0 += PB) {
            fe_u32x4_t ga[PB][2], gb[PB][2];
#pragma unroll
            for (int u = 0; u < PB; ++u) {
                const int e = (b0 + u) * EPI + wave * EPW + sub;
                const unsigned r = (unsigned)max(sRow[e], 0), c = (unsigned)sCol[e];
                const int oa = (int)((r * (unsigned)ldab + ch * 8) * 4), ob = (int)((c * (unsigned)ldab + H + ch * 8) * 4);
                ga[u][0] = __builtin_amdgcn_raw_buffer_load_b128(rs_ab, oa, 0, 0);
                ga[u][1] = __builtin_amdgcn_raw_buffer_load_b128(rs_ab, oa + 16, 0, 0);
                gb[u][0] = __builtin_amdgcn_raw_buffer_load_b128(rs_ab, ob, 0, 0);
                gb[u][1] = __builtin_amdgcn_raw_buffer_load_b128(rs_ab, ob + 16, 0, 0);
            }
#pragma unroll
            for (int u = 0; u < PB; ++u) {
                const int e = (b0 + u) * EPI + wave * EPW + sub;
                const float rh = sRh[e];
                uint32_t ph[4], pl[4];
#pragma unroll
                for (int k = 0; k < 4; ++k) {
                    const int q = k >> 1, w = (k & 1) * 2;
                    const f3_f2 a = f3_f2{__uint_as_float(ga[u][q][w]), __uint_as_float(ga[u][q][w + 1])};
                    const f3_f2 b = f3_f2{__uint_as_float(gb[u][q][w]), __uint_as_float(gb[u][q][w + 1])};
                    const f3_f2 m = f3_silu_pair(a + b + f3_f2{wv[2 * k], wv[2 * k + 1]} * rh);
                    fe_split2(m.x, m.y, ph[k], pl[k]);
                }
                const bool ok = e < ne;
                const int o = e * H + ((ch ^ (e & SWZ)) * 8);
                *(uint4*)&sXh[o] = ok ? make_uint4(ph[0], ph[1], ph[2], ph[3]) : make_uint4(0u, 0u, 0u, 0u);
                *(uint4*)&sXl[o] = ok ? make_uint4(pl[0], pl[1], pl[2], pl[3]) : make_uint4(0u, 0u, 0u, 0u);
            }
        }
    }
    __syncthreads();

    const int cx = (wave * 8 + (cq >> 1)) ^ (fr & SWZ);
    const int lbase = fr * H + (cq & 1) * 4;
#define F3_QOFF(i, j) (lbase + (i) * 16 * H + ((cx ^ ((j) * 2)) * 8))
    const int fcol = wave * 64 + cq * 4;
    const size_t fbase = (((size_t)tile * NW + wave) * (MI * 4) * 64 + lane) * 4;
#define F3_FOFF(i, j) (fbase + (size_t)((i) * 4 + (j)) * 256)

    f32x4_t acc[MI][4];
    fe_zero(acc);
    fe_gemm_x3<H, MI, SWZ>(sXh, sXl, W2ph, W2pl, wave, lane, acc);
    float4 bq4[4];
#pragma unroll
    for (int j = 0; j < 4; ++j) bq4[j] = *(const float4*)(b2 + fcol + j * 16);
    __syncthreads();
#pragma unroll
    for (int j = 0; j < 4; ++j) {
        const f3_f2 b01 = f3_f2{bq4[j].x, bq4[j].y}, b23 = f3_f2{bq4[j].z, bq4[j].w};
#pragma unroll
        for (int i = 0; i < MI; ++i) {
            f3_f2 m01, m23, d01, d23;
            if constexpr (SAVE) {
                f3_silu_pair_d(f3_f2{acc[i][j][0], acc[i][j][1]} + b01, m01, d01);
                f3_silu_pair_d(f3_f2{acc[i][j][2], acc[i][j][3]} + b23, m23, d23);
            } else {
                m01 = f3_silu_pair(f3_f2{acc[i][j][0], acc[i][j][1]} + b01);
                m23 = f3_silu_pair(f3_f2{acc[i][j][2], acc[i][j][3]} + b23);
            }
            if constexpr (DROP) {
                const uint32_t ee = (uint32_t)(e0 + i * 16 + fr), cc = (uint32_t)(fcol + j * 16);
                const f3_f2 k01 = f3_f2{fe_keep(seed, ee, cc, H, thr16, dscale), fe_keep(seed, ee, cc + 1, H, thr16, dscale)};
                const f3_f2 k23 = f3_f2{fe_keep(seed, ee, cc + 2, H, thr16, dscale), fe_keep(seed, ee, cc + 3, H, thr16, dscale)};
                m01 *= k01; m23 *= k23;
                if constexpr (SAVE) { d01 *= k01; d23 *= k23; }
            }
            if constexpr (SAVE) f3_stq(&d2f[F3_FOFF(i, j)], f3_pack(d01), f3_pack(d23));
            uint32_t h01, l01, h23, l23;
            fe_split2(m01.x, m01.y, h01, l01);
            fe_split2(m23.x, m23.y, h23, l23);
            *(uint2*)&sXh[F3_QOFF(i, j)] = make_uint2(h01, h23);
            *(uint2*)&sXl[F3_QOFF(i, j)] = make_uint2(l01, l23);
        }
        __builtin_amdgcn_sched_barrier(0);
    }
    __syncthreads();
    if constexpr (SAVE) {
        const __amdgpu_buffer_rsrc_t rs_m = fe_rsrc(Msave + (size_t)e0 * H, (unsigned)ne * H * 2);
#pragma unroll
        for (int q = tid; q < BM * CH; q += H) {
            const int rw = q / CH, c8 = q % CH;
            const uint4 v = *(const uint4*)&sXh[rw * H + ((c8 ^ (rw & SWZ)) * 8)];
            __builtin_amdgcn_raw_buffer_store_b128(fe_u32x4_t{v.x, v.y, v.z, v.w}, rs_m, (int)((rw * H + c8 * 8) * 2), 0,  2);
        }
    }

    {
        const bool head_cont = e0 > 0 && row[e0 - 1] == sRow[0];
        const bool tail_cont = e0 + ne < E && row[e0 + ne] == sRow[ne - 1];
        (void)fe_scan_runs64<H, false, SWZ>(sXh, sRow, nullptr, ne, head_cont, tail_cont, agg, (unsigned)H, bnd + (size_t)tile * 2 * H, tid,
                                            nullptr, 0u, sXl);
    }

    fe_zero(acc);
    fe_gemm_x3<H, MI, SWZ>(sXh, sXl, Wcph, Wcpl, wave, lane, acc);
    {
        f3_f2 da[MI], db[MI];
#pragma unroll
        for (int i = 0; i < MI; ++i) { da[i] = f3_f2{0.f, 0.f}; db[i] = da[i]; }
#pragma unroll
        for (int j = 0; j < 4; ++j) {
            const float4 bq = *(const float4*)(bc + fcol + j * 16), wq = *(const float4*)(w3 + fcol + j * 16);
            const f3_f2 b01 = f3_f2{bq.x, bq.y}, b23 = f3_f2{bq.z, bq.w}, w01 = f3_f2{wq.x, wq.y}, w23 = f3_f2{wq.z, wq.w};
#pragma unroll
            for (int i = 0; i < MI; ++i) {
                const f3_f2 z01 = f3_f2{acc[i][j][0], acc[i][j][1]} + b01, z23 = f3_f2{acc[i][j][2], acc[i][j][3]} + b23;
                da[i] += f3_silu_pair(z01) * w01;
                db[i] += f3_silu_pair(z23) * w23;
                if constexpr (SAVE) f3_stq(&z3f[F3_FOFF(i, j)], f3_pack(z01), f3_pack(z23));
            }
            __builtin_amdgcn_sched_barrier(0);
        }
#pragma unroll
        for (int i = 0; i < MI; ++i) {
            float t = (da[i].x + da[i].y) + (db[i].x + db[i].y);
            t += __shfl_xor(t, 16, 64);
            t += __shfl_xor(t, 32, 64);
            if (cq == 0) sDot[wave * BM + i * 16 + fr] = t;
        }
    }
    __syncthreads();
    if (tid < ne) {
        float s = 0.f;
#pragma unroll
        for (int w = 0; w < NW; ++w) s += sDot[w * BM + tid];
        s_out[e0 + tid] = s;
    }
#undef F3_QOFF
#undef F3_FOFF
}

int fe_fwd3_launch(const float* AB, int ldab, int H, const int* row, const int* col, const float* rhohat, const float* w_r,
                   const void* W2ph, const void* W2pl, const float* b2, const void* Wcph, const void* Wcpl, const float* bc,
                   const float* w3, int E, float* agg, float* s_out, uint32_t thr16, float dscale, unsigned seed, float* bnd,
                   int xcd_aware, hipStream_t stream, void* Msave, void* d2f, void* z3f) {
    const dim3 grid((((E + FE_BM - 1) / FE_BM + 7) / 8) * 8);
    const size_t lds = (size_t)2 * FE_BM * H * 2 + 3 * FE_BM * sizeof(int) + (size_t)(H / 64) * FE_BM * sizeof(float);
#define F3_LAUNCH_(HH, DD, SS)                                                                                     \
    do {                                                                                                           \
        static bool set_ = false;                                                                                  \
        if (!set_) { (void)hipFuncSetAttribute((const void*)gcl_edge_fused_x3_kernel<HH, DD, SS>, hipFuncAttributeMaxDynamicSharedMemorySize, (int)lds); set_ = true; } \
        hipLaunchKernelGGL((gcl_edge_fused_x3_kernel<HH, DD, SS>), grid, dim3(HH), lds, stream, AB, ldab, row, col, rhohat, w_r,  \
                           (const bf16_t*)W2ph, (const bf16_t*)W2pl, b2, (const bf16_t*)Wcph, (const bf16_t*)Wcpl, bc, w3, E, agg, \
                           s_out, thr16, dscale, (uint32_t)seed, bnd, xcd_aware, (bf16_t*)Msave, (bf16_t*)d2f, (bf16_t*)z3f); \
    } while (0)
#define F3_LAUNCH(HH)                                                                                              \
    do {                                                                                                           \
        if (Msave) { if (thr16) F3_LAUNCH_(HH, true, true); else F3_LAUNCH_(HH, false, true); }                    \
        else { if (thr16) F3_LAUNCH_(HH, true, false); else F3_LAUNCH_(HH, false, false); }                        \
    } while (0)
    if (H == 512) F3_LAUNCH(512); else if (H == 256) F3_LAUNCH(256); else if (H == 128) F3_LAUNCH(128); else F3_LAUNCH(64);
#undef F3_LAUNCH
#undef F3_LAUNCH_
    return 0;
}
```

### fabind_amd/kernels.py

```python
import ctypes

import numpy as np
import torch

from . import _lib
from . import config as _cfg
from ._lib import ACT_NONE, ACT_RELU, ACT_SIGMOID, ACT_SILU, ACT_STORED_DERIV, GemmArgs, check, dt_code, ptr, stream

__all__ = ["gemm", "colsum", "edges_count", "edges_fill", "exclusive_scan", "inter_meta",
           "edge_geom", "gcl_pre", "segment_sum", "coord_update", "cross_attn_fwd", "pair_bmat", "pair_hadamard",
           "inter_attn_fwd", "las_step", "select_rows", "ACT_NONE", "ACT_SILU", "ACT_RELU", "ACT_SIGMOID", "ACT_STORED_DERIV"]

GEMM_BN = 128
GEMM_DEFAULT_CONFIG = 13
PROFILE = None
PROFILE_ONLY = None


PROFILE_BYTES = {}
PROFILE_ALGO = {}


def _profiled(label, flops, fn, nbytes=0.0, algo=None):
    if PROFILE is None or (PROFILE_ONLY is not None and not label.startswith(PROFILE_ONLY)):
# ... 410 lines not shown
        assert W1.shape == (H, 2 * H) and W2.shape == (H, H)
        return pack_frag(W1[:, :H].contiguous()), pack_frag(W1[:, H:].contiguous()), pack_frag(W2), None
    assert W1.shape == (2 * H, H) and W2.shape == (H, 2 * H)
    return pack_frag(W1[:H].contiguous()), pack_frag(W1[H:].contiguous()), pack_frag(W2[:, :H].contiguous()), pack_frag(W2[:, H:].contiguous())


def node_chain_fwd(X1, X2, packs, b1, b2, act, kind, residual=None, want16=False):
    M, H = X1.shape
    assert X1.dtype == torch.bfloat16 and (X2 is None or X2.dtype == torch.bfloat16)
    out = torch.empty((M, H), dtype=torch.float32, device=X1.device)
    out16 = torch.empty((M, H), dtype=torch.bfloat16, device=X1.device) if want16 else None
    W1a, W1b, W2a, W2b = packs
    hidden = H if kind == 0 else 2 * H
    _profiled("fabind_node_chain_fwd kind=%d M=%d H=%d" % (kind, M, H), 2.0 * M * (2 * H * hidden),
              lambda: check(_lib.load().fabind_node_chain_fwd(
                  ptr(X1), _ld(X1), ptr(X2), _ld(X2) if X2 is not None else 0, ptr(W1a), ptr(W1b), ptr(b1), ptr(W2a), ptr(W2b), ptr(b2), act,
                  kind, ptr(residual), _ld(residual) if residual is not None else 0, ptr(out), _ld(out), ptr(out16),
                  H if want16 else 0, M, H, stream()), "fabind_node_chain_fwd"))
    return out, out16


def node_chain_x3_blocks(W1, W2, kind):
    H = W2.shape[0]
    if kind == 0:
        assert W1.shape == (H, 2 * H) and W2.shape == (H, H)
        return [W1[:, :H], W1[:, H:], W2, None]
    assert W1.shape == (2 * H, H) and W2.shape == (H, 2 * H)
    return [W1[:H], W1[H:], W2[:, :H], W2[:, H:]]


def node_chain_x3_pack_many(chains):
    ws, lo, slots = [], [], []
    for ci, (W1, W2, kind) in enumerate(chains):
        for bi, b_ in enumerate(node_chain_x3_blocks(W1, W2, kind)):
            if b_ is None:
                continue
            ws += [b_, b_]
            lo += [False, True]
            slots.append((ci, bi))
    packs = pack_frag_multi(ws, lo)
    out = [[None] * 8 for _ in chains]
    for k, (ci, bi) in enumerate(slots):
        out[ci][2 * bi], out[ci][2 * bi + 1] = packs[2 * k], packs[2 * k + 1]
    return [tuple(o) for o in out]


def node_chain_x3_pack(W1, W2, kind):
    H = W2.shape[0]
    if kind == 0:
        assert W1.shape == (H, 2 * H) and W2.shape == (H, H)
        blocks = (W1[:, :H], W1[:, H:], W2, None)
    else:
        assert W1.shape == (2 * H, H) and W2.shape == (H, 2 * H)
        blocks = (W1[:H], W1[H:], W2[:, :H], W2[:, H:])
    out = []
    for b_ in blocks:
        out.extend(pack_frag_split(b_.contiguous()) if b_ is not None else (None, None))
    return tuple(out)


def node_chain_x3_fwd(X1, X2, packs, b1, b2, act, kind, residual=None, want16=False, save=False):
    M, H = X1.shape
    assert X1.dtype == torch.float32 and (X2 is None or X2.dtype == torch.float32)
    out = torch.empty((M, H), dtype=torch.float32, device=X1.device)
    out16 = torch.empty((M, H), dtype=torch.bfloat16, device=X1.device) if want16 else None
    hidden = H if kind == 0 else 2 * H
    t16 = torch.empty((M, hidden), dtype=torch.bfloat16, device=X1.device) if save else None
    d16 = torch.empty((M, hidden), dtype=torch.bfloat16, device=X1.device) if (save and act == ACT_SILU) else None
    _profiled("fabind_node_chain_x3_fwd kind=%d M=%d H=%d" % (kind, M, H), 2.0 * M * (2 * H * hidden),
              lambda: check(_lib.load().fabind_node_chain_x3_fwd(
                  ptr(X1), _ld(X1), ptr(X2), _ld(X2) if X2 is not None else 0, *[ptr(t_) for t_ in packs[:4]], ptr(b1),
                  *[ptr(t_) for t_ in packs[4:]], ptr(b2), act, kind, ptr(residual), _ld(residual) if residual is not None else 0,
                  ptr(out), _ld(out), ptr(out16), H if want16 else 0, ptr(t16), hidden if save else 0, ptr(d16), hidden if d16 is not None else 0,
                  M, H, stream()), "fabind_node_chain_x3_fwd"))
    return (out, out16, t16, d16) if save else (out, out16)


def pack_frag_split(W):
    hi = W.to(torch.bfloat16)
    lo = (W.float() - hi.float()).to(torch.bfloat16)
    return pack_frag(hi), pack_frag(lo)


def gcl_edge_fused_x3(AB, H, row, col, rhohat, w_r, W2, b2, Wc, bc, w3, n_rows, p_drop=0.0, seed=0, rowptr=None, save=False):
    E = row.shape[0]
    if save and E > 0:
        nt = (E + 63) // 64
        Msave = torch.empty((E, H), dtype=torch.bfloat16, device=AB.device)
        d2f = torch.empty((nt * 64, H), dtype=torch.bfloat16, device=AB.device)
        z3f = torch.empty((nt * 64, H), dtype=torch.bfloat16, device=AB.device)
    else:
        save = False
    assert AB.dtype == torch.float32 and AB.stride(1) == 1
    alloc = torch.zeros if (rowptr is None or E == 0) else torch.empty
    agg = alloc((n_rows, H), dtype=torch.float32, device=AB.device)
    if alloc is torch.empty:
        zero_empty_rows(rowptr, agg, H)
    s = torch.empty((max(E, 1), 1), dtype=torch.float32, device=AB.device)
    bnd = torch.empty(((E + 63) // 64 * 2 + 2, H), dtype=torch.float32, device=AB.device)
    W2h, W2l = pack_frag_split(W2)
    Wch, Wcl = pack_frag_split(Wc)
    if save:
        _profiled("gcl_edge_fused_x3_kernel<%d> E=%d saving (gather + 2 chained H x H split-bf16 contractions + segment-sum per edge; M, silu'(pre2), pre3 kept)" % (H, E),
                  4.0 * E * H * H,
                  lambda: check(_lib.load().fabind_gcl_edge_fused_x3_train(ptr(AB), _ld(AB), AB.shape[0], H, ptr(row), ptr(col), ptr(rhohat), ptr(w_r),
                                                                           ptr(W2h), ptr(W2l), ptr(b2), ptr(Wch), ptr(Wcl), ptr(bc), ptr(w3), E,
                                                                           ptr(agg), ptr(s), float(p_drop), int(seed) & 0xFFFFFFFF, ptr(bnd),
                                                                           ptr(Msave), ptr(d2f), ptr(z3f), stream()), "fabind_gcl_edge_fused_x3_train"),
                  E * (6.0 * H + 16) + n_rows * (8.0 * H + 4.0 * H),
                  algo=2.0 * n_rows * H * 4 + E * 8.0 + n_rows * 24.0)
        return agg, s[:E], (Msave, d2f, z3f)
    _profiled("gcl_edge_fused_x3_kernel<%d> E=%d (gather + 2 chained H x H split-bf16 contractions + segment-sum per edge)" % (H, E),
              4.0 * E * H * H,
              lambda: check(_lib.load().fabind_gcl_edge_fused_x3(ptr(AB), _ld(AB), AB.shape[0], H, ptr(row), ptr(col), ptr(rhohat), ptr(w_r),
                                                                 ptr(W2h), ptr(W2l), ptr(b2), ptr(Wch), ptr(Wcl), ptr(bc), ptr(w3), E,
                                                                 ptr(agg), ptr(s), float(p_drop), int(seed) & 0xFFFFFFFF, ptr(bnd),
                                                                 stream()), "fabind_gcl_edge_fused_x3"),
              E * 16.0 + n_rows * (8.0 * H + 4.0 * H), algo=2.0 * n_rows * H * 4 + E * 8.0 + n_rows * 24.0)
    return agg, s[:E]


def zero_empty_rows(rowptr, out, C, out2=None):
    n_rows = rowptr.shape[0] - 1
    check(_lib.load().fabind_zero_empty_rows(ptr(rowptr), n_rows, ptr(out), dt_code(out.dtype), _ld(out), C, ptr(out2),
                                             dt_code(out2.dtype) if out2 is not None else 0, _ld(out2) if out2 is not None else 0,
                                             stream()), "fabind_zero_empty_rows")


def gcl_edge_fused(AB16, H, row, col, rhohat, w_r, W2p, b2, Wcp, bc, w3, n_rows, p_drop=0.0, seed=0, want16=False, rowptr=None, save=False):
    E = row.shape[0]
    if save and E > 0:
        nt = (E + 63) // 64
        Msave = torch.empty((E, H), dtype=torch.bfloat16, device=AB16.device)
        d2f = torch.empty((nt * 64, H), dtype=torch.bfloat16, device=AB16.device)
        z3f = torch.empty((nt * 64, H), dtype=torch.bfloat16, device=AB16.device)
    else:
        save, Msave, d2f, z3f = False, None, None, None
    alloc = torch.zeros if (rowptr is None or E == 0) else torch.empty
    agg = alloc((n_rows, H), dtype=torch.float32, device=AB16.device)
    agg16 = alloc((n_rows, H), dtype=torch.bfloat16, device=AB16.device) if want16 else None
    if alloc is torch.empty:
        zero_empty_rows(rowptr, agg, H, agg16)
    s = torch.empty((max(E, 1), 1), dtype=torch.float32, device=AB16.device)
    bnd = torch.empty(((E + 63) // 64 * 2 + 2, H), dtype=torch.float32, device=AB16.device)
    if save:
        _profiled("gcl_edge_fused_kernel<%d> E=%d saving (gather + 2 chained H x H contractions + segment-sum per edge; M, silu'(pre2), pre3 kept)" % (H, E),
                  4.0 * E * H * H,
                  lambda: check(_lib.load().fabind_gcl_edge_fused_train(ptr(AB16), _ld(AB16), H, ptr(row), ptr(col), ptr(rhohat), ptr(w_r),
                                                                        ptr(W2p), ptr(b2), ptr(Wcp), ptr(bc), ptr(w3), E, ptr(agg), ptr(s),
                                                                        float(p_drop), int(seed) & 0xFFFFFFFF, ptr(bnd), ptr(agg16),
                                                                        ptr(Msave), ptr(d2f), ptr(z3f), stream()),
                                "fabind_gcl_edge_fused_train"),
                  E * (6.0 * H + 16) + n_rows * (4.0 * H + 4.0 * H + (2.0 * H if want16 else 0.0)),
                  algo=2.0 * n_rows * H * 2 + E * 8.0 + n_rows * 24.0)
    else:
        _profiled("gcl_edge_fused_kernel<%d> E=%d (gather + 2 chained H x H contractions + segment-sum per edge)" % (H, E), 4.0 * E * H * H,
                  lambda: check(_lib.load().fabind_gcl_edge_fused(ptr(AB16), _ld(AB16), H, ptr(row), ptr(col), ptr(rhohat), ptr(w_r),
                                                                  ptr(W2p), ptr(b2), ptr(Wcp), ptr(bc), ptr(w3), E, ptr(agg), ptr(s),
                                                                  float(p_drop), int(seed) & 0xFFFFFFFF, ptr(bnd), ptr(agg16), stream()),
                                "fabind_gcl_edge_fused"),
                  E * 16.0 + n_rows * (4.0 * H + 4.0 * H + (2.0 * H if want16 else 0.0)),
                  algo=2.0 * n_rows * H * 2 + E * 8.0 + n_rows * 24.0)
    out = (agg, s[:E], agg16) if want16 else (agg, s[:E])
    return out + ((Msave, d2f, z3f),) if save else out


def edge_lnfold(AB16, Kp, H, row, col, rho, stat, eps, w_r, c_r, c_c, dvec, p_drop=0.0, seed=0):
    E = row.shape[0]
    out = torch.empty((E, Kp), dtype=torch.bfloat16, device=AB16.device)
    assert AB16.dtype == torch.bfloat16 and stat.dtype == torch.float32 and stat.is_contiguous()
    check(_lib.load().fabind_edge_lnfold(ptr(AB16), _ld(AB16), Kp, H, ptr(row), ptr(col), ptr(rho), ptr(stat), float(eps),
                                         ptr(w_r), ptr(c_r), ptr(c_c), ptr(dvec), E, ptr(out), float(p_drop), int(seed) & 0xFFFFFFFF,
                                         stream()), "fabind_edge_lnfold")
    return out


def edge_lnfold_bwd(AB16, Kp, H, row, col, rho, stat, eps, w_r, c_r, c_c, out, dout, p_drop=0.0):
    E = row.shape[0]
    dev = AB16.device
    if E == 0:
        return (torch.zeros((0, Kp), dtype=torch.bfloat16, device=dev), torch.zeros((0, 8), dtype=torch.float32, device=dev),
                torch.zeros(0, dtype=torch.float32, device=dev), torch.zeros((4, Kp), dtype=torch.float32, device=dev))
    lib = _lib.load()
    nb = max(1, int(lib.fabind_edge_lnfold_bwd_blocks(E)))
    du = torch.empty((max(E, 1), Kp), dtype=torch.bfloat16, device=dev)
    es = torch.empty((max(E, 1), 8), dtype=torch.float32, device=dev)
    drho = torch.empty(max(E, 1), dtype=torch.float32, device=dev)
    part = torch.empty((nb, 4 * Kp), dtype=torch.float32, device=dev)
    assert AB16.dtype == torch.bfloat16 and out.dtype == torch.bfloat16 and dout.dtype == torch.bfloat16 and dout.is_contiguous() and out.is_contiguous()
    check(lib.fabind_edge_lnfold_bwd(ptr(AB16), _ld(AB16), Kp, H, ptr(row), ptr(col), ptr(rho), ptr(stat), float(eps), ptr(w_r), ptr(c_r),
                                     ptr(c_c), ptr(out), ptr(dout), E, float(p_drop), ptr(du), ptr(es), ptr(drho), ptr(part), nb,
                                     stream()), "fabind_edge_lnfold_bwd")
    return du[:E], es[:E], drho[:E], colsum(part).view(4, Kp)


def inter_coord_fold(P16, H, col, rho, stat, q_w, eps, u, d, w3, p_drop=0.0, seed=0):
    E = col.shape[0]
    out = torch.empty(max(E, 1), dtype=torch.float32, device=P16.device)
    assert P16.dtype == torch.bfloat16 and stat.dtype == torch.float32 and stat.is_contiguous()
    check(_lib.load().fabind_inter_coord_fold(ptr(P16), _ld(P16), H, ptr(col), ptr(rho), ptr(stat), float(q_w), float(eps),
                                              ptr(u), ptr(d), ptr(w3), E, ptr(out), float(p_drop), int(seed) & 0xFFFFFFFF,
                                              stream()), "fabind_inter_coord_fold")
    return out[:E]


def row_stats(x, eps):
    R, C = x.shape
    mu = torch.empty(max(R, 1), dtype=torch.float32, device=x.device)
    rs = torch.empty(max(R, 1), dtype=torch.float32, device=x.device)
    check(_lib.load().fabind_row_stats(ptr(x), dt_code(x.dtype), _ld(x), float(eps), R, C, ptr(mu), ptr(rs), stream()),
          "fabind_row_stats")
    return mu, rs


def layernorm_rows_form(x, out, C=None, pad_to=None):
    C = x.shape[1] if C is None else C
    pad_to = out.shape[1] if pad_to is None else pad_to
    return int(_lib.load().fabind_layernorm_rows_form(ptr(x), _ld(x), C, ptr(out), _ld(out), pad_to))


def layernorm_rows_bwd_form(x, dy, dx, C=None):
    C = x.shape[1] if C is None else C
    return int(_lib.load().fabind_layernorm_rows_bwd_form(ptr(x), _ld(x), ptr(dy), _ld(dy), ptr(dx), _ld(dx), C))


def row_stats_form(x):
    return int(_lib.load().fabind_row_stats_form(ptr(x), dt_code(x.dtype), _ld(x), x.shape[1]))


def edge_lnfold_form(Kp, H):
    u = ctypes.c_int(0)
    lib = _lib.load()
    return int(lib.fabind_edge_lnfold_form(Kp, H, ctypes.byref(u))), u.value, int(lib.fabind_edge_lnfold_blocks(2 ** 31 - 1))


def edge_lnfold_bwd_form(Kp):
    u = ctypes.c_int(0)
    lib = _lib.load()
    return int(lib.fabind_edge_lnfold_bwd_form(Kp, ctypes.byref(u))), u.value, int(lib.fabind_edge_lnfold_bwd_blocks(2 ** 31 - 1))


def inter_coord_fold_blocks(E=2 ** 31 - 1):
    return int(_lib.load().fabind_inter_coord_fold_blocks(E))


def pair_update_fused(T, b_off, p_node, c_node, z, Wop, bo, ln_w, ln_b, eps, W1p, b1, W2p, b2, Wbp=None, bb=None, p_drop=0.0,
                      seed=0):
    n, H = z.shape
    assert z.dtype == torch.bfloat16 and z.is_contiguous() and T.dtype == torch.float32
    z_out = torch.empty_like(z)
    bias_out = torch.empty((max(n, 1), 16), dtype=torch.float32, device=z.device) if Wbp is not None else None
    a = _lib.PairUpdateArgs()
    for name, t in (("T", T), ("p_node", p_node), ("c_node", c_node), ("z_in", z), ("z_out", z_out), ("Wop", Wop), ("bo", bo),
                    ("ln_w", ln_w), ("ln_b", ln_b), ("W1p", W1p), ("b1", b1), ("W2p", W2p), ("b2", b2), ("Wbp", Wbp), ("bb", bb),
                    ("bias_out", bias_out)):
        setattr(a, name, ptr(t))
    a.ldt, a.b_off, a.n_pairs = _ld(T), int(b_off), n
    a.eps, a.p_drop, a.seed = float(eps), float(p_drop), int(seed) & 0xFFFFFFFF
    _profiled("pair_update_fused_kernel<%d> pairs=%d (Hadamard + LN + 2 chained H x H contractions + 16 biases)" % (H, n),
              2.0 * n * H * (2 * H + 32 + 16),
              lambda: check(_lib.load().fabind_pair_update_fused(ctypes.byref(a), H, stream()), "fabind_pair_update_fused"))
    return z_out, (bias_out[:n] if bias_out is not None else None)


_N_CU = {}
EDGE_BWD_GROUPS = 0
EDGE_BWD_TIMES = None


def gcl_edge_fused_bwd(AB16, H, row, col, rhohat, w_r, W2, b2, Wc, bc, w3, ds, dagg, colptr, perm, p_drop=0.0, seed=0,
                       dab_bf16=False, w_dtype=torch.float32, rowptr=None, frags=None, saved=None):
    E, N, dev = row.shape[0], AB16.shape[0], AB16.device
    ng = _N_CU.get(dev)
    if ng is None:
        ng = _N_CU[dev] = torch.cuda.get_device_properties(dev).multi_processor_count
    lib = _lib.load()
    variant = lib.fabind_gcl_edge_fused_bwd_variant_for(H)
    if saved is not None and E > 0:
        variant = 6
    bm = 64
    if variant == 6:
        per_cu = max(1, min(8, (160 * 1024) // (2 * bm * H + 16 * H + 32 * bm), 16 // max(1, H // 64)))
    elif variant == 5:
        per_cu = max(1, min(8, (160 * 1024) // (4 * bm * H + 16 * H + 32 * bm), 12 // (H // 64 + 1)))
    else:
        per_cu = max(1, min(8, (160 * 1024) // (4 * bm * H + 1024), 512 // H))
    ng = max(1, min(ng * per_cu, (E + bm - 1) // bm))
    if EDGE_BWD_GROUPS:
        ng = int(EDGE_BWD_GROUPS)
    if ng >= 8:
        ng -= ng % 8
    d2scratch = torch.empty((2, ng, bm * H), dtype=torch.bfloat16, device=dev) if variant == 5 else None
    bnd = torch.empty(((E + bm - 1) // bm * 2 + 2, H), dtype=torch.float32, device=dev)
    if variant == 6:
        buf = torch.empty((4, max(E, 1), H), dtype=torch.bfloat16, device=dev)
        S1, Mm, dT, dP2, dP1 = buf[0], saved[0], buf[1], buf[2], buf[3]
    else:
        buf = torch.empty((5, max(E, 1), H), dtype=torch.bfloat16, device=dev)
        S1, Mm, dT, dP2, dP1 = buf[0], buf[1], buf[2], buf[3], buf[4]
    dab_bf16 = bool(dab_bf16) and variant in (5, 6)
    dAB = (torch.zeros if (rowptr is None or E == 0) else torch.empty)((N, 2 * H), dtype=torch.bfloat16 if dab_bf16 else torch.float32, device=dev)
    if rowptr is not None and E > 0:
        zero_empty_rows(rowptr, dAB, H)
    drh = torch.empty(max(E, 1), dtype=torch.float32, device=dev)
    part = torch.zeros((ng, 4, H), dtype=torch.float32, device=dev)
    dagg = dagg.contiguous()
    ds = ds.contiguous()
    a = _lib.EdgeBwdArgs()
    W2p, Wcp, W2Tp, WcTp = frags if (frags is not None and len(frags) == 4) else (pack_frag(W2), pack_frag(Wc), pack_frag(W2.t()), pack_frag(Wc.t()))
    keep = (W2p, Wcp, W2Tp, WcTp)
    for name, t in (("AB", AB16), ("row", row), ("col", col), ("rhohat", rhohat), ("w_r", w_r), ("W2p", W2p), ("Wcp", Wcp),
                    ("W2Tp", W2Tp), ("WcTp", WcTp), ("b2", b2), ("bc", bc), ("w3", w3), ("ds", ds), ("dagg", dagg),
                    ("S1", S1), ("Mm", Mm), ("dT", dT), ("dP2", dP2), ("dP1", dP1), ("drh", drh),
                    ("dABrow", None if dab_bf16 else dAB), ("dAB16", dAB if dab_bf16 else None),
                    ("part", part), ("d2scratch", d2scratch), ("bnd", bnd)):
        setattr(a, name, ptr(t))
    a.ldab, a.lddagg, a.lddab, a.E = _ld(AB16), _ld(dagg), _ld(dAB), E
    a.lddab16 = _ld(dAB)
    a.p_drop, a.seed = float(p_drop), int(seed) & 0xFFFFFFFF
    a.dbg = ptr(EDGE_BWD_TIMES) if (EDGE_BWD_TIMES is not None and variant != 6) else None
    if variant == 6:
        a.d2f, a.z3f = ptr(saved[1]), ptr(saved[2])
    _profiled(("gcl_edge_fused_bwd4_kernel<%d> E=%d (2 chained H x H contractions per edge over the forward's saved tiles)" % (H, E)) if variant == 6 else
              "gcl_edge_fused_bwd%s_kernel<%d> E=%d (recompute + 4 chained H x H contractions per edge)" % ("3" if variant == 5 else "", H, E),
              (4.0 if variant == 6 else 8.0) * E * H * H,
              lambda: check(_lib.load().fabind_gcl_edge_fused_bwd(ctypes.byref(a), H, ng, stream()),
                            "fabind_gcl_edge_fused_bwd"),
              E * ((12.0 if variant == 6 else 10.0) * H + 20) + N * (4.0 * H + 4.0 * H + (2.0 if dab_bf16 else 4.0) * H),
              algo=N * (2.0 * H * 2 + 4.0 * H + 2.0 * H * (2.0 if dab_bf16 else 4.0)) + E * 20.0)
    del keep
    if E > 0:
        if dab_bf16:
            segment_sum(dP1[:E], colptr, N, eidx=perm, out16=dAB[:, H:])
        else:
            segment_sum(dP1[:E], colptr, N, eidx=perm, out=dAB[:, H:])
        if tn_can_queue(dP2[:E], S1[:E], W2.data_ptr()) and tn_can_queue(dT[:E], Mm[:E], Wc.data_ptr()):
            dW2, dWc = torch.empty((H, H), dtype=w_dtype, device=dev), torch.empty((H, H), dtype=w_dtype, device=dev)
            gemm_tn_queued(dP2[:E], S1[:E], dW2, key=W2.data_ptr())
            gemm_tn_queued(dT[:E], Mm[:E], dWc, key=Wc.data_ptr())
        else:
            TN_STATS["direct"] += 2
            dW2 = gemm_tn(dP2[:E], S1[:E], out_dtype=w_dtype)
            dWc = gemm_tn(dT[:E], Mm[:E], out_dtype=w_dtype)
    else:
        dW2 = torch.zeros((H, H), dtype=w_dtype, device=dev)
        dWc = torch.zeros((H, H), dtype=w_dtype, device=dev)
    ps = part.sum(0)
    out = (dAB, drh[:E], ps[3], dW2, ps[0], dWc, ps[1], ps[2])
    return out


_ZERO_PAGE = {}


_TN_SPLITS = {}


def _tn_splits(M, N, E, tn):
    key = (M, N, E, tn)
    s = _TN_SPLITS.get(key)
    if s is not None:
        return s
    if tn != 256:
        tiles = ((M + 255) // 256) * ((N + 127) // 128)
        s = max(1, min(256, max(E // 2048, min(E // 256, 16)), max(1, 1024 // tiles)))
    elif E < 4096:
        s = max(1, min(16, E // 256))
    else:
        tiles = ((M + 255) // 256) * ((N + 255) // 256)
        best = None
        for c in range(8, 257, 8):
            if E // c < 256:
                break
            rounds = -(-(tiles * c // 8) // 32)
            cost = rounds * (-(-E // c) / 32.0 * 0.45 + 3.0) + c * M * N * 8 / 3e6
            if best is None or cost < best[0]:
                best = (cost, c)
        s = best[1] if best else 8
    _TN_SPLITS[key] = s
    return s


TN_DEFER = _cfg.knob("FABIND_TN_DEFER")
TN_DEFER_JOB_BYTES = 1024 << 20
TN_DEFER_QUEUE_BYTES = 6144 << 20
_TNQ = {"jobs": [], "bytes": 0, "armed": False, "outs": set()}
_TNJOB = np.dtype([(n_, np.uint64) for n_ in ("Y", "X", "C_part", "out", "out_tail")] +
                  [(n_, np.int32) for n_ in ("ldy", "ldx", "M", "N", "E", "splits", "e_per", "n_tiles", "with_colsum", "out_dt", "ldo",
                                             "wg0", "n_wg", "blk0", "n_blk", "pad_")])
TN_STATS = {"queued": 0, "flushes": 0, "direct": 0}


def tn_pending():
    return len(_TNQ["jobs"])


def _tn_multi_splits(E):
    return max(8, min(64, (E // 4096 + 7) // 8 * 8))


def gemm_tn_queued(Y, X, out, out_tail=None, key=None):
    E, M = Y.shape
    N = X.shape[1]
    nb = (Y.numel() + X.numel()) * 2
    q = _TNQ
    q["jobs"].append((Y, X, out, out_tail, M, N, E))
    q["bytes"] += nb
    if key is not None:
        q["outs"].add(key)
    TN_STATS["queued"] += 1
    if q["bytes"] > TN_DEFER_QUEUE_BYTES:
# ... 149 lines not shown
```

### fabind_amd/ops.py

```python
import ctypes

import numpy as np
import torch

from . import config as _cfg
from . import kernels as K
from ._lib import GemmArgs, check, dt_code, load, ptr, stream


def act_dtype():
    return torch.float32 if _cfg.fp32_storage() else torch.bfloat16


mm_dtype = act_dtype


def needs_grad(*ts):
    return torch.is_grad_enabled() and any(torch.is_tensor(t) and t.requires_grad for t in ts)


_needs_grad = needs_grad


def _nchunk(rows):
# ... 496 lines not shown
    @staticmethod
    def forward(ctx, x, W, b, u, act_pro, act_epi):
        z, part = _gemm_rowdot(x, W, b, u, act_pro, act_epi, store=True)
        ctx.act_pro, ctx.act_epi, ctx.Wt = act_pro, act_epi, _stored_wt(W)
        ctx.save_for_backward(x, W, u, z)
        return part

    @staticmethod
    def backward(ctx, dpart):
        x, W, u, z = ctx.saved_tensors
        assert ctx.act_pro == K.ACT_NONE
        dz, du = _rowdot_bwd(z, dpart.contiguous(), u, ctx.act_epi)
        dx, _ = K.gemm(dz, _wt(ctx.Wt, W), out_dtype=x.dtype)
        dW, db = _param_grads(dz, x, None, W, True, True)
        return dx, dW, db, du, None, None


class _LinearRowdotDrop(torch.autograd.Function):

    @staticmethod
    def forward(ctx, x, W, b, u, p_drop, seed):
        z, part = _gemm_rowdot(x, W, b, u, K.ACT_NONE, K.ACT_RELU, store=True, p_drop=p_drop, seed=seed, post=True)
        ctx.scale, ctx.Wt = _drop_scale(p_drop), _stored_wt(W)
        ctx.save_for_backward(x, W, u, z)
        return part

    @staticmethod
    def backward(ctx, dpart):
        x, W, u, z = ctx.saved_tensors
        dz, du = _rowdot_bwd(z, (dpart * ctx.scale).contiguous(), u, K.ACT_RELU)
        ni = ctx.needs_input_grad
        dx = K.gemm(dz, _wt(ctx.Wt, W), out_dtype=x.dtype)[0] if ni[0] else None
        dW, db = _param_grads(dz, x, None, W, ni[1], ni[2])
        return dx, dW, db, (du / ctx.scale if ni[3] else None), None, None


def linear_rowdot(x, W, b, u, act_pro=K.ACT_NONE, act_epi=K.ACT_NONE, p_drop=0.0, fold=None):
    if _needs_grad(x, W, b, u):
        assert fold is None, "the LayerNorm fold has no autograd path"
        K.tn_hook(W, b)
        if p_drop > 0.0:
            assert act_pro == K.ACT_NONE and act_epi == K.ACT_RELU, "epilogue dropout under autograd: ReLU outputs only"
            assert b is not None, "linear_rowdot with epilogue dropout under autograd needs a bias"
            return _LinearRowdotDrop.apply(x, W, b, u, p_drop, _drop_seed(p_drop))
        return _LinearRowdot.apply(x, W, b, u, act_pro, act_epi)
    return _gemm_rowdot(x, W, b, u, act_pro, act_epi, store=False, p_drop=p_drop, seed=_drop_seed(p_drop), fold=fold)[1]


class _EdgeTail(torch.autograd.Function):
    @staticmethod
    def forward(ctx, Mm, Wc, bc, w3, rowptr, row, n_rows, act_epi):
        z, part = _gemm_rowdot(Mm, Wc, bc, w3, K.ACT_NONE, act_epi, store=True)
        agg = K.segment_sum(Mm, rowptr, n_rows)
        ctx.act_epi, ctx.Wt = act_epi, _stored_wt(Wc)
        ctx.save_for_backward(Mm, Wc, w3, z, row)
        return part, agg

    @staticmethod
    def backward(ctx, dpart, dagg):
        Mm, Wc, w3, z, row = ctx.saved_tensors
        M, N = z.shape
        if dpart is None:
            dpart = torch.zeros((M, (N + K.GEMM_BN - 1) // K.GEMM_BN), dtype=torch.float32, device=z.device)
        dz, du = _rowdot_bwd(z, dpart.contiguous(), w3, ctx.act_epi)
        Wt = _wt(ctx.Wt, Wc)
        if dagg is not None:
            dM, _ = K.gemm(dz, Wt, residual=dagg.contiguous(), r_index=row, out_dtype=Mm.dtype)
        else:
            dM, _ = K.gemm(dz, Wt, out_dtype=Mm.dtype)
        dW, dbc = _param_grads(dz, Mm, None, Wc, True, True)
        return dM, dW, dbc, du, None, None, None, None


def edge_tail(Mm, Wc, bc, w3, rowptr, row, n_rows, act_epi=K.ACT_SILU):
    if _needs_grad(Mm, Wc, bc, w3):
        K.tn_hook(Wc, bc)
        return _EdgeTail.apply(Mm, Wc, bc, w3, rowptr, row, n_rows, act_epi)
    part = _gemm_rowdot(Mm, Wc, bc, w3, K.ACT_NONE, act_epi, store=False)[1]
    return part, K.segment_sum(Mm, rowptr, n_rows)


EDGE_SAVE_FWD = _cfg.knob("FABIND_EDGE_SAVE_FWD")
EDGE_SAVE_MIN_H = 256


class _FusedEdge(torch.autograd.Function):

    @staticmethod
    def forward(ctx, AB16, rhohat, w_r, W2, b2, Wc, bc, w3, H, g, p_drop, seed, holder=None, frags=None):
        ctx.H, ctx.g, ctx.p_drop, ctx.seed, ctx.frags = H, g, p_drop, seed, frags
        W2p, Wcp = (frags[0], frags[1]) if frags is not None else (K.pack_frag(W2), K.pack_frag(Wc))
        E = g.row_ctx.shape[0]
        save = EDGE_SAVE_FWD and H >= EDGE_SAVE_MIN_H and E >= 1 and AB16.dtype == torch.bfloat16
        out = K.gcl_edge_fused(AB16, H, g.row_ctx, g.col_ctx, rhohat, w_r, W2p, b2, Wcp, bc, w3,
                               AB16.shape[0], p_drop, seed, want16=holder is not None, rowptr=g.rp_ctx, save=save)
        ctx.n_saved = 3 if save else 0
        ctx.save_for_backward(AB16, rhohat, w_r, W2, b2, Wc, bc, w3, *(out[-1] if save else ()))
        if holder is not None:
            holder.append(out[2])
        return out[0], out[1]

    @staticmethod
    def backward(ctx, dagg, ds):
        AB16, rhohat, w_r, W2, b2, Wc, bc, w3 = ctx.saved_tensors[:8]
        saved = tuple(ctx.saved_tensors[8:]) if ctx.n_saved else None
        g = ctx.g
        colptr, perm = g.ctx_by_col()
        if dagg is None:
            dagg = torch.zeros((AB16.shape[0], ctx.H), dtype=torch.float32, device=AB16.device)
        if ds is None:
            ds = torch.zeros(g.row_ctx.shape[0], dtype=torch.float32, device=AB16.device)
        dAB, drh, dwr, dW2, db2, dWc, dbc, dw3 = K.gcl_edge_fused_bwd(
            AB16, ctx.H, g.row_ctx, g.col_ctx, rhohat, w_r, W2, b2, Wc, bc, w3, ds.reshape(-1).float(), dagg.float(),
            colptr, perm, ctx.p_drop, ctx.seed, dab_bf16=AB16.dtype == torch.bfloat16, w_dtype=W2.dtype, rowptr=g.rp_ctx, frags=ctx.frags,
            saved=saved)
        return (dAB.to(AB16.dtype), drh, dwr, dW2.to(W2.dtype), db2, dWc.to(Wc.dtype), dbc, dw3, None, None, None, None, None, None)


class _FusedEdgeX3(torch.autograd.Function):

    @staticmethod
    def forward(ctx, AB, rhohat, w_r, W2, b2, Wc, bc, w3, H, g, p_drop, seed):
        ctx.H, ctx.g, ctx.p_drop, ctx.seed = H, g, p_drop, seed
        E = g.row_ctx.shape[0]
        save = EDGE_SAVE_FWD and H >= EDGE_SAVE_MIN_H and E >= 1
        out = K.gcl_edge_fused_x3(AB, H, g.row_ctx, g.col_ctx, rhohat, w_r, W2, b2, Wc, bc, w3, AB.shape[0], p_drop, seed,
                                  rowptr=g.rp_ctx, save=save)
        ctx.n_saved = 3 if save else 0
        ctx.save_for_backward(AB, rhohat, w_r, W2, b2, Wc, bc, w3, *(out[2] if save else ()))
        return out[0], out[1]

    @staticmethod
    def backward(ctx, dagg, ds):
        AB, rhohat, w_r, W2, b2, Wc, bc, w3 = ctx.saved_tensors[:8]
        saved = tuple(ctx.saved_tensors[8:]) if ctx.n_saved else None
        g = ctx.g
        colptr, perm = g.ctx_by_col()
        if dagg is None:
            dagg = torch.zeros((AB.shape[0], ctx.H), dtype=torch.float32, device=AB.device)
        if ds is None:
            ds = torch.zeros(g.row_ctx.shape[0], dtype=torch.float32, device=AB.device)
        dAB, drh, dwr, dW2, db2, dWc, dbc, dw3 = K.gcl_edge_fused_bwd(
            AB.to(torch.bfloat16), ctx.H, g.row_ctx, g.col_ctx, rhohat, w_r, W2, b2, Wc, bc, w3, ds.reshape(-1).float(), dagg.float(),
            colptr, perm, ctx.p_drop, ctx.seed, dab_bf16=False, w_dtype=torch.float32, rowptr=g.rp_ctx, saved=saved)
        return (dAB, drh, dwr, dW2, db2, dWc, dbc, dw3, None, None, None, None)


def fused_edge(AB16, rhohat, w_r, W2, b2, Wc, bc, w3, H, g, p_drop=0.0, frags=None):
    seed = _drop_seed(p_drop)
    if _needs_grad(AB16, rhohat, w_r, W2, b2, Wc, bc, w3):
        K.tn_hook(W2, Wc)
    if _cfg.get_precision() == "bf16x3" and _cfg.x3_edge_bf16() and AB16.dtype == torch.float32:
        ab = AB16.to(torch.bfloat16)
        if _needs_grad(AB16, rhohat, w_r, W2, b2, Wc, bc, w3):
            agg, s = _FusedEdge.apply(ab, rhohat, w_r, W2, b2, Wc, bc, w3, H, g, p_drop, seed, None, None)
            return agg, s
        out = K.gcl_edge_fused(ab, H, g.row_ctx, g.col_ctx, rhohat, w_r, K.pack_frag(W2), b2, K.pack_frag(Wc), bc, w3, ab.shape[0], p_drop, seed,
                               want16=False, rowptr=g.rp_ctx)
        return out[0], out[1]
    if _cfg.get_precision() == "bf16x3":
        if _needs_grad(AB16, rhohat, w_r, W2, b2, Wc, bc, w3):
            return _FusedEdgeX3.apply(AB16, rhohat, w_r, W2, b2, Wc, bc, w3, H, g, p_drop, seed)
        return K.gcl_edge_fused_x3(AB16, H, g.row_ctx, g.col_ctx, rhohat, w_r, W2, b2, Wc, bc, w3, AB16.shape[0], p_drop, seed,
                                   rowptr=g.rp_ctx)
    w16 = _cfg.get_precision() == "bf16"
    if _needs_grad(AB16, rhohat, w_r, W2, b2, Wc, bc, w3):
        holder = [] if w16 else None
        agg, s = _FusedEdge.apply(AB16, rhohat, w_r, W2, b2, Wc, bc, w3, H, g, p_drop, seed, holder, frags)
        return _attach_b16(agg, holder[0] if holder else None), s
    W2p, Wcp = (frags[0], frags[1]) if frags is not None else (K.pack_frag(W2), K.pack_frag(Wc))
    out = K.gcl_edge_fused(AB16, H, g.row_ctx, g.col_ctx, rhohat, w_r, W2p, b2, Wcp, bc, w3,
                           AB16.shape[0], p_drop, seed, want16=w16, rowptr=g.rp_ctx)
    return (_attach_b16(out[0], out[2]), out[1]) if w16 else out


class _EdgeGeom(torch.autograd.Function):
    @staticmethod
    def forward(ctx, x, row, col, rowptr, lay, bycol):
        d, rho, rhohat, norm = K.edge_geom(x, row, col, rowptr, lay.node_off, lay.B)
        ctx.lay, ctx.n, ctx.bycol = lay, x.shape[0], bycol
        ctx.save_for_backward(row, col, rowptr, d, rho, norm)
        return d, rhohat

    @staticmethod
    def backward(ctx, dd, drhohat):
        row, col, rowptr, d, rho, norm = ctx.saved_tensors
        lay, E, dev = ctx.lay, row.shape[0], d.device
        if ctx.bycol is not None:
            colptr, perm = ctx.bycol()
        else:
            colsorted, perm64 = torch.sort(col.long(), stable=True)
            colptr = torch.zeros(ctx.n + 1, dtype=torch.int32, device=dev)
            colptr[1:] = torch.cumsum(torch.bincount(colsorted, minlength=ctx.n), 0).to(torch.int32)
            perm = perm64.to(torch.int32)
        dx = torch.empty((ctx.n, 3), dtype=torch.float32, device=dev)
        dd = dd.contiguous() if dd is not None else torch.zeros_like(d)
        drhohat = drhohat.contiguous() if drhohat is not None else torch.zeros_like(rho)
        gbuf = torch.empty((max(E, 1), 3), dtype=torch.float32, device=dev)
        check(load().fabind_edge_geom_bwd(ptr(d), ptr(rho), ptr(norm), ptr(dd), ptr(drhohat), ptr(row), ptr(rowptr),
                                          ptr(colptr), ptr(perm), ptr(lay.node_off), lay.B, E, ctx.n, ptr(dx), ptr(gbuf),
                                          ptr(torch.empty(lay.B, dtype=torch.float32, device=dev)), stream()),
              "fabind_edge_geom_bwd")
        return dx, None, None, None, None, None


def edge_geom(x, row, col, rowptr, lay, bycol=None):
    if _needs_grad(x):
        return _EdgeGeom.apply(x, row, col, rowptr, lay, bycol)
    d, _, rhohat, _ = K.edge_geom(x, row, col, rowptr, lay.node_off, lay.B)
    return d, rhohat
# ... 1207 lines not shown
```

### include/fabind_hip.h

```cpp
#ifndef FABIND_HIP_H
#define FABIND_HIP_H

#include <stdint.h>

#ifdef __cplusplus
extern "C" {
#endif

#ifndef __HIP_PLATFORM_AMD__
typedef struct ihipStream_t* hipStream_t;
#endif

const char* fabind_last_error(void);
#define FABIND_ABI_VERSION 19
int fabind_abi_version(void);
int fabind_sizeof_args(int which);

typedef struct FabindGemmArgs {
    const void* A;
    const void* A2;
    const void* W;
    void* C;
    const float* bias;
    const void* R;
// ... 39 lines not shown
                   const void* zero_page, const int* groups, int n_groups, int with_colsum, hipStream_t stream);

typedef struct FabindTnJob {
    const void* Y; const void* X; float* C_part; void* out; float* out_tail;
    int ldy, ldx, M, N, E, splits, e_per, n_tiles, with_colsum, out_dt, ldo;
    int wg0, n_wg, blk0, n_blk, pad_;
} FabindTnJob;
int fabind_gemm_tn_multi(const FabindTnJob* jobs_dev, const FabindTnJob* jobs_host, int n_jobs, const int* wg_job_dev, int total_wg,
                         const int* blk_job_dev, int total_blk, const void* zero_page, hipStream_t stream);

int fabind_transpose_act(const void* in, int in_dt, int ldi, void* out, int out_dt, int ldo, int R, int C, int act,
                         hipStream_t stream);
typedef struct FabindCopySeg {
    const void* src;
    void* dst;
    long long src_sr, src_sc, dst_sr, dst_sc;
    int rows, cols;
    int src_dt, dst_dt;
    int vec4, pad_;
} FabindCopySeg;
int fabind_multi_copy(const FabindCopySeg* segs_dev, int n_segs, int blocks_per_seg, hipStream_t stream);
typedef struct FabindAdamRow {
    float* p;
    const float* g;
    float* m;
    float* v;
    long long numel;
    int chunk0, step_idx;
    double lr, beta1, beta2, eps, weight_decay;
    int decoupled, pad_;
} FabindAdamRow;
int fabind_adam_chunk(void);
int fabind_multi_sqnorm(const FabindAdamRow* rows_dev, int n_rows, int n_chunks, const float* steps, float* partials, float* snap,
                        hipStream_t stream);
int fabind_multi_adam(const FabindAdamRow* rows_dev, int n_rows, int n_chunks, const float* partials, const float* snap, float* steps,
                      float max_norm, int flags, float* grad_norm, int* skipped, hipStream_t stream);
typedef struct FabindPackSeg {
    const void* src;
    void* dst;
    long long src_sr, src_sc;
    int N, K, src_dt, pad_;
} FabindPackSeg;
int fabind_pack_frag_multi(const FabindPackSeg* segs_dev, const FabindPackSeg* segs_host, int n_segs, hipStream_t stream);
int fabind_split_sum(const float* part, int splits, long n, void* out, int out_dt, long n_tail, float* out_tail, hipStream_t stream);
int fabind_colsum(const void* in, int in_dt, int ldi, float* out, int R, int C, int accumulate, float* scratch,
                  int nchunk, hipStream_t stream);

int fabind_edges_count(const float* x, const int* node_off, const int* c_cnt, int B, int max_n, const int* bond_row,
                       const int* bond_off, float cut_intra, float cut_inter, int* deg_ctx, int* deg_int,
                       hipStream_t stream);
int fabind_edges_fill(const float* x, const int* node_off, const int* c_cnt, int B, int max_n, const int* bond_row,
                      const int* bond_col, const int* bond_off, float cut_intra, float cut_inter,
                      const int* rowptr_ctx, const int* rowptr_int, int* col_ctx, int* row_ctx, int* col_int,
                      int* row_int, hipStream_t stream);
int fabind_exclusive_scan(const int* in, int* out, int n, hipStream_t stream);
int fabind_lower_bound(const int* vals, int n, const int* keys, int n_keys, int* out, hipStream_t stream);
int fabind_inter_meta(const int* node_off, const int* c_cnt, int B, const int* rowptr_int, const int* col_int,
                      const int* row_int, int E_int, int* red_off, int* red_idx, int* red_c, int* red_p, int* mirror,
                      hipStream_t stream);

int fabind_edge_geom(const float* x, const int* row, const int* col, const int* rowptr, const int* node_off, int B,
                     float* d, float* rho, float* rhohat, float* norm, hipStream_t stream);

int fabind_gcl_pre(const void* AB, int ab_dt, int ldab, int H, const int* row, const int* col, const float* rhohat,
                   const float* w_r, void* pre, int pre_dt, int E, int act, void* dact_out, hipStream_t stream);
int fabind_segment_sum(const void* Z, int z_dt, int ldz, int H, const int* rowptr, const int* eidx, int n_rows, int n_edges,
                       int act, float* out, int ldo,
                       void* out16 , int ldo16,
                       hipStream_t stream);
int fabind_zero_empty_rows(const int* rowptr, int n_rows, void* out, int out_dt, int ld, int C, void* out2, int out2_dt, int ld2,
                           hipStream_t stream);
int fabind_coord_update(const float* x, const float* d, const float* s_part, int n_part, const float* weight,
                        const int* rowptr, int n_rows, int mean, float clampv, float* x_out, float* s_out,
                        hipStream_t stream);

int fabind_gcl_edge_fused_x3(const float* AB, int ldab, int n_rows, int H, const int* row, const int* col, const float* rhohat,
                             const float* w_r, const void* W2ph, const void* W2pl, const float* b2, const void* Wcph,
                             const void* Wcpl, const float* bc, const float* w3, int E, float* agg, float* s_out, float p_drop,
                             unsigned seed, float* bnd, hipStream_t stream);
int fabind_gcl_edge_fused_x3_train(const float* AB, int ldab, int n_rows, int H, const int* row, const int* col, const float* rhohat,
                                   const float* w_r, const void* W2ph, const void* W2pl, const float* b2, const void* Wcph,
                                   const void* Wcpl, const float* bc, const float* w3, int E, float* agg, float* s_out, float p_drop,
                                   unsigned seed, float* bnd, void* M, void* d2f, void* z3f, hipStream_t stream);

int fabind_gcl_edge_fused(const void* AB, int ldab, int H, const int* row, const int* col, const float* rhohat,
                          const float* w_r, const void* W2p, const float* b2, const void* Wcp, const float* bc,
                          const float* w3, int E, float* agg, float* s_out, float p_drop, unsigned seed,
                          float* bnd ,
                          void* agg16 ,
                          hipStream_t stream);

int fabind_gcl_edge_fused_train(const void* AB, int ldab, int H, const int* row, const int* col, const float* rhohat,
                                const float* w_r, const void* W2p, const float* b2, const void* Wcp, const float* bc,
                                const float* w3, int E, float* agg, float* s_out, float p_drop, unsigned seed, float* bnd,
                                void* agg16, void* M, void* d2f, void* z3f, hipStream_t stream);

typedef struct FabindEdgeBwdArgs {
    const void* AB; const int* row; const int* col; const float* rhohat; const float* w_r;
    const void* W2p; const void* Wcp; const void* W2Tp; const void* WcTp;
    const float* b2; const float* bc; const float* w3; const float* ds; const float* dagg;
    void* S1; void* Mm; void* dT; void* dP2; void* dP1;
    float* drh; float* dABrow; float* part;
    void* dbg;
    float* bnd;
    void* d2scratch;
    int ldab, lddagg, lddab, E;
    float p_drop;
    unsigned seed;
    int xcd_aware;
    int lddab16;
    void* dAB16;
    const void* d2f;
    const void* z3f;
} FabindEdgeBwdArgs;
int fabind_gcl_edge_fused_bwd(const FabindEdgeBwdArgs* args, int H, int n_groups, hipStream_t stream);
int fabind_gcl_edge_fused_bwd_set_tile(int bm);
int fabind_gcl_edge_fused_bwd_tile(void);
int fabind_gcl_edge_fused_bwd_set_variant(int v);
int fabind_gcl_edge_fused_bwd_variant(void);
int fabind_gcl_edge_fused_bwd_variant_for(int H);
void fabind_gcl_edge_fused_bwd3_set_exp(int mask);
void fabind_gcl_edge_fused_bwd4_set_exp(int mask);
void fabind_gcl_edge_fused_set_xcd_aware(int on);
int fabind_gcl_edge_fused_set_variant(int v);
int fabind_gcl_edge_fused_variant(void);

typedef struct FabindPairUpdateArgs {
    const float* T; const int* p_node; const int* c_node;
    const void* z_in; void* z_out;
    const void* Wop; const float* bo; const float* ln_w; const float* ln_b;
    const void* W1p; const float* b1; const void* W2p; const float* b2;
    const void* Wbp; const float* bb; float* bias_out;
    int ldt, b_off, n_pairs;
    float eps, p_drop;
    unsigned seed;
} FabindPairUpdateArgs;
int fabind_pair_update_fused(const FabindPairUpdateArgs* args, int H, hipStream_t stream);

int fabind_post_optimize(const float* x0, const float* ref, const int* atom_off, const int* nbr_ptr, const int* nbr_idx,
                         int n_ligands, int max_atoms, int all_pairs, int steps, float lr, float* x_out, float* loss_out,
                         float* rmsd_out, hipStream_t stream);

int fabind_distmap_generate(const float* x0, const float* truth, const float* pocket, const int* pocket_off, const float* y_pred,
                            const long long* y_off, const int* atom_off, const int* con_ptr, const int* con_idx, const float* con_d,
                            int n_ligands, int n_repeat, int n_atoms, int max_atoms, int max_pocket, int max_con, long max_y,
                            int excluded_volume, int mode, int epochs, int config_start, const double* rate_lr, float* x_out,
                            float* loss_out, float* terms_out, float* rmsd_out, float* trace_loss, float* trace_rmsd,
                            hipStream_t stream);

int fabind_sym_automorphisms(const int* labels, const int* nbr_ptr, const int* nbr_idx, const int* atom_off, int n_ligands, int cap,
                             int max_steps, const int* flat_off, int* scratch, int* flat, int* count, int* status, hipStream_t stream);
int fabind_sym_score(const float* pred, int n_pose, int n_atoms, const float* ref, const int* atom_off, const int* flat_off,
                     const int* auto_cnt, const int* flat, int n_ligands, int max_atoms, float* min_rmsd, int* arg_rmsd, float* min_sl1,
                     int* arg_sl1, int* best_idx, hipStream_t stream);
int fabind_pose_stats(const float* pred, const float* truth, const int* atom_off, int B, float* rmsd, float* cdis, hipStream_t stream);
int fabind_rank_loss_fwd(const float* scores, const float* rmsd, const int* group_off, int G, int mode, int with_ce, float* terms,
                         float* d_scores, int* counts, hipStream_t stream);

int fabind_cross_attn_fwd(const float* q, int ldq, const float* k, const float* v, int ldkv, const float* gpre,
                          int ldg, const float* bias, int bias_ld, int lin_col, int gate_col, const int* desc, int B,
                          int max_nq, float scale, float* out, int ldo, float* lse, int ksplit, float* part, int n_rows,
                          hipStream_t stream);

int fabind_cross_attn_fused_fwd(const float* q, int ldq, const float* k, const float* v, int ldkv, const float* gpre, int ldg,
                                const void* a0, int lda0, const void* bo, const int* toff, const float* bconst, const int* desc, int B,
                                int max_P, int max_C, int H, int mode, float scale, float* out, int ldo, float* part, int n_lig_rows,
                                float* lse, hipStream_t stream);
int fabind_pair_bo_pack(const float* b0, int ldb, const float* wcomp, int H, const int* c_index, const int* desc, const int* toff,
                        const int* tile_b, int n_tiles, void* out, int n_blocks, long blk_stride, hipStream_t stream);

typedef struct FabindAttnFusedBwdArgs {
    const float* qg; const float* kv; const void* a0; const void* bo; const void* boT; const int* toff; const int* koff;
    const float* bconst; const int* desc; const int* desc_p; const float* out; const float* lse; const float* dout;
    float* dqg; float* dkv; float* dO; float* Dv; float* da0; void* acat; float* colpart; float* part;
    int ldq, ldkv, lda0, ldda0, ldacat, kcol0, ldcolpart, kp;
    float scale;
    int nsplit, B, part_rows;
} FabindAttnFusedBwdArgs;
int fabind_cross_attn_fused_bwd(const FabindAttnFusedBwdArgs* args, int B, int max_P, int max_C, int H, int mode, int n_lig_rows,
                                hipStream_t stream);
long fabind_cross_attn_fused_bwd_scratch(int B, int max_P, int max_C, int n_lig_rows, int mode);
int fabind_cross_attn_fused_bwd_parts(int B, int max_P);
int fabind_pair_bot_pack(const float* b0, int ldb, const float* wcomp, int H, const int* c_index, const int* desc, const int* koff,
                         const int* kstep_b, int n_ksteps, void* out, int n_blocks, long blk_stride, hipStream_t stream);

int fabind_cross_attn_mfma_fwd(const float* q, int ldq, const float* k, const float* v, int ldkv, const float* gpre, int ldg,
                               const float* bias, int bias_ld, int lin_col, int gate_col, const int* desc, int B, int max_nq,
                               float scale, float* out, int ldo, float* lse, int ksplit, float* part, int n_rows,
                               hipStream_t stream);

int fabind_pair_bmat(const float* b0, int ldb, const float* wcomp, int NO, int H, const int* c_node, int n_c,
                     void* bmat, int bmat_dt, hipStream_t stream);
int fabind_pair_hadamard(const float* a0, const float* b0, int ld0, int H, const float* a1, const float* b1, int ld1,
                         int H2, const int* red_p, const int* red_c, int n_red, void* hd, int hd_dt, int ldh,
                         hipStream_t stream);

int fabind_inter_attn_fwd(const float* qkv, int ldqkv, const float* cv, int ldcv, int H, const float* h, int ldh,
                          const float* x, const float* d, const float* rhohat, const int* rowptr, const int* col,
// ... 216 lines not shown
```

Measured before the change: 539.6.

## Save S1 tile in edge forward and store silu-derivative tile as 8-bit codes

The fused edge forward can now also keep the first-stage activation tile (S1), so the saved-tile backward no longer recomputes it. The saved silu-derivative tile (d2f) is stored as an 8-bit fixed-point code with the dropout mask folded in, instead of bf16, which halves that tile's write and read traffic. Both are on by default through new module-level flags. The cost is an extra E x H bf16 write in forward, and 8-bit quantisation error (steps of about 0.005 over [-0.1, 1.1]) in the gradient of the edge MLP.

```diff
diff --git a/fabind_amd/_lib.py b/fabind_amd/_lib.py
--- a/fabind_amd/_lib.py
+++ b/fabind_amd/_lib.py
@@ -77,9 +77,12 @@
     "fabind_gcl_pre": [_vp, _i, _i, _i, _vp, _vp, _vp, _vp, _vp, _i, _i, _i, _vp, _vp],
     "fabind_gcl_edge_fused": [_vp, _i, _i, _vp, _vp, _vp, _vp, _vp, _vp, _vp, _vp, _vp, _i, _vp, _vp, _f, ctypes.c_uint, _vp, _vp, _vp],
     "fabind_gcl_edge_fused_train": [_vp, _i, _i, _vp, _vp, _vp, _vp, _vp, _vp, _vp, _vp, _vp, _i, _vp, _vp, _f, ctypes.c_uint, _vp, _vp, _vp, _vp, _vp, _vp],
+    "fabind_gcl_edge_fused_train_tiles": [_vp, _i, _i, _vp, _vp, _vp, _vp, _vp, _vp, _vp, _vp, _vp, _i, _vp, _vp, _f, ctypes.c_uint, _vp, _vp, _vp, _vp, _vp, _vp, _i, _vp],
+    "fabind_gcl_edge_fused_x3_train_tiles": [_vp, _i, _i, _i, _vp, _vp, _vp, _vp, _vp, _vp, _vp, _vp, _vp, _vp, _vp, _i, _vp, _vp, _f, ctypes.c_uint, _vp, _vp, _vp, _vp, _i, _vp],
     "fabind_gcl_edge_fused_x3": [_vp, _i, _i, _i, _vp, _vp, _vp, _vp, _vp, _vp, _vp, _vp, _vp, _vp, _vp, _i, _vp, _vp, _f, ctypes.c_uint, _vp, _vp],
     "fabind_gcl_edge_fused_x3_train": [_vp, _i, _i, _i, _vp, _vp, _vp, _vp, _vp, _vp, _vp, _vp, _vp, _vp, _vp, _i, _vp, _vp, _f, ctypes.c_uint, _vp, _vp, _vp, _vp, _vp],
     "fabind_gcl_edge_fused_bwd": [ctypes.POINTER(EdgeBwdArgs), _i, _i, _vp],
+    "fabind_gcl_edge_fused_bwd_tiles": [ctypes.POINTER(EdgeBwdArgs), _i, _i, _i, _i, _vp],
     "fabind_pair_update_fused": [ctypes.POINTER(PairUpdateArgs), _i, _vp],
     "fabind_gcl_edge_fused_bwd_set_tile": [_i],
     "fabind_gcl_edge_fused_bwd_tile": [],
diff --git a/fabind_amd/csrc/fused_common.h b/fabind_amd/csrc/fused_common.h
--- a/fabind_amd/csrc/fused_common.h
+++ b/fabind_amd/csrc/fused_common.h
@@ -385,6 +385,26 @@
 }
 __device__ __forceinline__ uint32_t fe3_pack(const fe_f2 v) { return pack2_bf16(v.x, v.y); }
 __device__ __forceinline__ fe_f2 fe3_unpack(const uint32_t u) { return fe_f2{__uint_as_float(u << 16), __uint_as_float(u & 0xffff0000u)}; }
+__device__ __forceinline__ void fe_pre1_silu_pair(const uint32_t a, const uint32_t b, const fe_f2 w, const float rh, fe_f2& m, fe_f2& d) {
+    fe3_silu_pair(fe3_unpack(a) + fe3_unpack(b) + w * rh, m, d);
+}
+
+#define FE_D8_LO (-0.1f)
+#define FE_D8_STEP (1.2f / 254.0f)
+__device__ __forceinline__ uint32_t fe_d8_code(const float d, const bool kept) {
+    const float c = fminf(fmaxf(__builtin_rintf((d - FE_D8_LO) * (1.0f / FE_D8_STEP)), 0.0f), 254.0f);
+    return kept ? (uint32_t)c + 1u : 0u;
+}
+__device__ __forceinline__ uint32_t fe_d8_pack(const fe_f2 d01, const fe_f2 d23, const bool k0, const bool k1, const bool k2, const bool k3) {
+    return fe_d8_code(d01.x, k0) | (fe_d8_code(d01.y, k1) << 8) | (fe_d8_code(d23.x, k2) << 16) | (fe_d8_code(d23.y, k3) << 24);
+}
+__device__ __forceinline__ float fe_d8_value(const uint32_t b, const float sc) {
+    return b ? ((float)(b - 1u) * FE_D8_STEP + FE_D8_LO) * sc : 0.f;
+}
+__device__ __forceinline__ void fe_d8_unpack(const uint32_t w, const float sc, fe_f2& d01, fe_f2& d23) {
+    d01 = fe_f2{fe_d8_value(w & 0xffu, sc), fe_d8_value((w >> 8) & 0xffu, sc)};
+    d23 = fe_f2{fe_d8_value((w >> 16) & 0xffu, sc), fe_d8_value(w >> 24, sc)};
+}
 
 __device__ __forceinline__ uint4 fe3_bload16(const __amdgpu_buffer_rsrc_t rs, const unsigned voff, const unsigned soff) {
     const fe_u32x4_t v = __builtin_amdgcn_raw_buffer_load_b128(rs, (int)voff, (int)soff, 0);
@@ -399,9 +419,9 @@
 int fe_fwd3_launch(const float* AB, int ldab, int H, const int* row, const int* col, const float* rhohat, const float* w_r,
                    const void* W2ph, const void* W2pl, const float* b2, const void* Wcph, const void* Wcpl, const float* bc,
                    const float* w3, int E, float* agg, float* s_out, uint32_t thr16, float dscale, unsigned seed, float* bnd,
-                   int xcd_aware, hipStream_t stream, void* Msave = nullptr, void* d2f = nullptr, void* z3f = nullptr);
+                   int xcd_aware, hipStream_t stream, void* Msave = nullptr, void* d2f = nullptr, void* z3f = nullptr, bool d2_u8 = false);
 int fe_fwd2_launch(const void* AB, int ldab, int H, const int* row, const int* col, const float* rhohat, const float* w_r,
                    const void* W2p, const float* b2, const void* Wcp, const float* bc, const float* w3, int E, float* agg,
                    float* s_out, uint32_t thr16, float dscale, unsigned seed, float* bnd, void* agg16, int xcd_aware, hipStream_t stream,
-                   void* Msave = nullptr, void* d2f = nullptr, void* z3f = nullptr);
-int fe_bwd4_launch(const FabindEdgeBwdArgs* a, int H, int n_groups, hipStream_t stream);
+                   void* Msave = nullptr, void* d2f = nullptr, void* z3f = nullptr, void* S1save = nullptr, bool d2_u8 = false);
+int fe_bwd4_launch(const FabindEdgeBwdArgs* a, int H, int n_groups, hipStream_t stream, bool s1_given = false, bool d2_u8 = false);
diff --git a/fabind_amd/csrc/fused_edge.hip b/fabind_amd/csrc/fused_edge.hip
--- a/fabind_amd/csrc/fused_edge.hip
+++ b/fabind_amd/csrc/fused_edge.hip
@@ -15,7 +15,7 @@
 static int fe_fwd_entry(const void* AB, int ldab, int H, const int* row, const int* col, const float* rhohat,
                         const float* w_r, const void* W2p, const float* b2, const void* Wcp, const float* bc,
                         const float* w3, int E, float* agg, float* s_out, float p_drop, unsigned seed,
-                        float* bnd, void* agg16, void* Msave, void* d2f, void* z3f, hipStream_t stream) {
+                        float* bnd, void* agg16, void* Msave, void* d2f, void* z3f, void* S1save, bool d2_u8, hipStream_t stream) {
     if (E <= 0) return 0;
     FB_REQUIRE((Msave != nullptr) == (d2f != nullptr) && (Msave != nullptr) == (z3f != nullptr),
                "fabind_gcl_edge_fused_train: M, d2f and z3f come together");
@@ -28,7 +28,7 @@
     FB_REQUIRE(ldab % 8 == 0, "fabind_gcl_edge_fused: ldab % 8");
     {
         const int rc = fe_fwd2_launch(AB, ldab, H, row, col, rhohat, w_r, W2p, b2, Wcp, bc, w3, E, agg, s_out, thr16, dscale, seed, bnd,
-                                      agg16, g_fe_xcd_aware, stream, Msave, d2f, z3f);
+                                      agg16, g_fe_xcd_aware, stream, Msave, d2f, z3f, S1save, d2_u8);
         if (rc) return rc;
     }
     hipLaunchKernelGGL((fe_boundary_fix_kernel<FE_BM>), dim3((E + FE_BM - 1) / FE_BM), dim3(H < 256 ? H : 256), 0, stream, row, E, H,
@@ -42,20 +42,30 @@
                                      const float* w3, int E, float* agg, float* s_out, float p_drop, unsigned seed,
                                      float* bnd, void* agg16, hipStream_t stream) {
     return fe_fwd_entry(AB, ldab, H, row, col, rhohat, w_r, W2p, b2, Wcp, bc, w3, E, agg, s_out, p_drop, seed, bnd, agg16, nullptr, nullptr,
-                        nullptr, stream);
+                        nullptr, nullptr, false, stream);
 }
 extern "C" int fabind_gcl_edge_fused_train(const void* AB, int ldab, int H, const int* row, const int* col, const float* rhohat,
                                            const float* w_r, const void* W2p, const float* b2, const void* Wcp, const float* bc,
                                            const float* w3, int E, float* agg, float* s_out, float p_drop, unsigned seed,
                                            float* bnd, void* agg16, void* M, void* d2f, void* z3f, hipStream_t stream) {
     FB_REQUIRE(M != nullptr && d2f != nullptr && z3f != nullptr, "fabind_gcl_edge_fused_train: M, d2f, z3f are required");
-    return fe_fwd_entry(AB, ldab, H, row, col, rhohat, w_r, W2p, b2, Wcp, bc, w3, E, agg, s_out, p_drop, seed, bnd, agg16, M, d2f, z3f, stream);
+    return fe_fwd_entry(AB, ldab, H, row, col, rhohat, w_r, W2p, b2, Wcp, bc, w3, E, agg, s_out, p_drop, seed, bnd, agg16, M, d2f, z3f, nullptr, false, stream);
+}
+extern "C" int fabind_gcl_edge_fused_train_tiles(const void* AB, int ldab, int H, const int* row, const int* col, const float* rhohat,
+                                                 const float* w_r, const void* W2p, const float* b2, const void* Wcp, const float* bc,
+                                                 const float* w3, int E, float* agg, float* s_out, float p_drop, unsigned seed,
+                                                 float* bnd, void* agg16, void* M, void* d2f, void* z3f, void* S1, int d2_bits,
+                                                 hipStream_t stream) {
+    FB_REQUIRE(M != nullptr && d2f != nullptr && z3f != nullptr, "fabind_gcl_edge_fused_train_tiles: M, d2f, z3f are required");
+    FB_REQUIRE(d2_bits == 16 || d2_bits == 8, "fabind_gcl_edge_fused_train_tiles: d2_bits is 16 (bf16) or 8 (fixed-point code)");
+    return fe_fwd_entry(AB, ldab, H, row, col, rhohat, w_r, W2p, b2, Wcp, bc, w3, E, agg, s_out, p_drop, seed, bnd, agg16, M, d2f, z3f, S1,
+                        d2_bits == 8, stream);
 }
 
 static int fe_x3_entry(const float* AB, int ldab, int n_rows, int H, const int* row, const int* col, const float* rhohat,
                        const float* w_r, const void* W2ph, const void* W2pl, const float* b2, const void* Wcph,
                        const void* Wcpl, const float* bc, const float* w3, int E, float* agg, float* s_out,
-                       float p_drop, unsigned seed, float* bnd, void* Msave, void* d2f, void* z3f, hipStream_t stream) {
+                       float p_drop, unsigned seed, float* bnd, void* Msave, void* d2f, void* z3f, bool d2_u8, hipStream_t stream) {
     if (E <= 0) return 0;
     FB_REQUIRE(bnd != nullptr, "fabind_gcl_edge_fused_x3: bnd (ceil(E/64) x 2 x H floats of scratch) is required");
     FB_REQUIRE(p_drop >= 0.f && p_drop < 1.f, "fabind_gcl_edge_fused_x3: p_drop in [0, 1)");
@@ -65,7 +75,7 @@
     const uint32_t thr16 = (uint32_t)(p_drop * 65536.0f + 0.5f);
     const float dscale = 1.0f / (1.0f - (float)thr16 / 65536.0f);
     const int rc = fe_fwd3_launch(AB, ldab, H, row, col, rhohat, w_r, W2ph, W2pl, b2, Wcph, Wcpl, bc, w3, E, agg, s_out, thr16, dscale,
-                                  seed, bnd, g_fe_xcd_aware, stream, Msave, d2f, z3f);
+                                  seed, bnd, g_fe_xcd_aware, stream, Msave, d2f, z3f, d2_u8);
     if (rc) return rc;
     hipLaunchKernelGGL((fe_boundary_fix_kernel<FE_BM>), dim3((E + FE_BM - 1) / FE_BM), dim3(H < 256 ? H : 256), 0, stream, row, E, H,
                        bnd, agg, (unsigned)H, (bf16_t*)nullptr, 0u);
@@ -77,7 +87,7 @@
                                         const void* Wcpl, const float* bc, const float* w3, int E, float* agg, float* s_out,
                                         float p_drop, unsigned seed, float* bnd, hipStream_t stream) {
     return fe_x3_entry(AB, ldab, n_rows, H, row, col, rhohat, w_r, W2ph, W2pl, b2, Wcph, Wcpl, bc, w3, E, agg, s_out, p_drop, seed, bnd,
-                       nullptr, nullptr, nullptr, stream);
+                       nullptr, nullptr, nullptr, false, stream);
 }
 extern "C" int fabind_gcl_edge_fused_x3_train(const float* AB, int ldab, int n_rows, int H, const int* row, const int* col, const float* rhohat,
                                               const float* w_r, const void* W2ph, const void* W2pl, const float* b2, const void* Wcph,
@@ -85,7 +95,17 @@
                                               float p_drop, unsigned seed, float* bnd, void* M, void* d2f, void* z3f, hipStream_t stream) {
     FB_REQUIRE(M != nullptr && d2f != nullptr && z3f != nullptr, "fabind_gcl_edge_fused_x3_train: M, d2f, z3f are required");
     return fe_x3_entry(AB, ldab, n_rows, H, row, col, rhohat, w_r, W2ph, W2pl, b2, Wcph, Wcpl, bc, w3, E, agg, s_out, p_drop, seed, bnd,
-                       M, d2f, z3f, stream);
+                       M, d2f, z3f, false, stream);
+}
+extern "C" int fabind_gcl_edge_fused_x3_train_tiles(const float* AB, int ldab, int n_rows, int H, const int* row, const int* col, const float* rhohat,
+                                                    const float* w_r, const void* W2ph, const void* W2pl, const float* b2, const void* Wcph,
+                                                    const void* Wcpl, const float* bc, const float* w3, int E, float* agg, float* s_out,
+                                                    float p_drop, unsigned seed, float* bnd, void* M, void* d2f, void* z3f, int d2_bits,
+                                                    hipStream_t stream) {
+    FB_REQUIRE(M != nullptr && d2f != nullptr && z3f != nullptr, "fabind_gcl_edge_fused_x3_train_tiles: M, d2f, z3f are required");
+    FB_REQUIRE(d2_bits == 16 || d2_bits == 8, "fabind_gcl_edge_fused_x3_train_tiles: d2_bits is 16 (bf16) or 8 (fixed-point code)");
+    return fe_x3_entry(AB, ldab, n_rows, H, row, col, rhohat, w_r, W2ph, W2pl, b2, Wcph, Wcpl, bc, w3, E, agg, s_out, p_drop, seed, bnd,
+                       M, d2f, z3f, d2_bits == 8, stream);
 }
 
 template <int H, int BM, bool DBG>
@@ -423,7 +443,7 @@
     return (!g_fe_bwd_variant_set && g_fe_bwd_variant == 5 && H <= 128) ? 0 : g_fe_bwd_variant;
 }
 
-extern "C" int fabind_gcl_edge_fused_bwd(const FabindEdgeBwdArgs* a_in, int H, int n_groups, hipStream_t stream) {
+static int fe_bwd_entry(const FabindEdgeBwdArgs* a_in, int H, int n_groups, hipStream_t stream, bool s1_given, bool d2_u8) {
     FabindEdgeBwdArgs a_copy = *a_in;
     a_copy.xcd_aware = g_fe_xcd_aware;
     const FabindEdgeBwdArgs* a = &a_copy;
@@ -434,8 +454,9 @@
     const int g_fe_bwd_variant = fabind_gcl_edge_fused_bwd_variant_for(H);
     if (a->d2f != nullptr || a->z3f != nullptr) {
         FB_REQUIRE(a->d2f != nullptr && a->z3f != nullptr, "fabind_gcl_edge_fused_bwd: d2f and z3f (saved by fabind_gcl_edge_fused_train) come together");
-        return fe_bwd4_launch(a, H, n_groups, stream);
-    }
+        return fe_bwd4_launch(a, H, n_groups, stream, s1_given, d2_u8);
+    }
+    FB_REQUIRE(!s1_given && !d2_u8, "fabind_gcl_edge_fused_bwd_tiles: needs d2f and z3f (the two-contraction kernel; the recompute forms keep no tiles)");
     if (g_fe_bwd_variant == 5) return fe_bwd3_launch(a, H, 64, n_groups, stream);
     FB_REQUIRE(a->dAB16 == nullptr, "fabind_gcl_edge_fused_bwd: dAB16 (bf16 receiving-side sums) exists in variant 5 only");
     FB_REQUIRE(a->bnd != nullptr, "fabind_gcl_edge_fused_bwd: bnd (ceil(E / tile) x 2 x H floats of scratch) is required");
@@ -468,3 +489,11 @@
     FB_CHECK_LAUNCH();
     return 0;
 }
+
+extern "C" int fabind_gcl_edge_fused_bwd(const FabindEdgeBwdArgs* args, int H, int n_groups, hipStream_t stream) {
+    return fe_bwd_entry(args, H, n_groups, stream, false, false);
+}
+extern "C" int fabind_gcl_edge_fused_bwd_tiles(const FabindEdgeBwdArgs* args, int H, int n_groups, int s1_given, int d2_bits, hipStream_t stream) {
+    FB_REQUIRE(d2_bits == 16 || d2_bits == 8, "fabind_gcl_edge_fused_bwd_tiles: d2_bits is 16 (bf16) or 8 (fixed-point code)");
+    return fe_bwd_entry(args, H, n_groups, stream, s1_given != 0, d2_bits == 8);
+}
diff --git a/fabind_amd/csrc/fused_edge_bwd4.hip b/fabind_amd/csrc/fused_edge_bwd4.hip
--- a/fabind_amd/csrc/fused_edge_bwd4.hip
+++ b/fabind_amd/csrc/fused_edge_bwd4.hip
@@ -22,8 +22,8 @@
 __device__ __forceinline__ uint2 fe4_ldq(const bf16_t* p_) { return *(const uint2*)p_; }
 #endif
 
-template <int H>
-__global__ __launch_bounds__(H, 4) void gcl_edge_fused_bwd4_kernel(const FabindEdgeBwdArgs p, const int xf) {
+template <int H, bool S1IN = false, bool D8 = false>
+__global__ __launch_bounds__(H, 4) void gcl_edge_fused_bwd4_kernel(const FabindEdgeBwdArgs p, const int xf, const float dsc) {
     constexpr int BM = FE_BM, MI = BM / 16;
     constexpr int NW = H / 64;
     constexpr int CH = H / 8;
@@ -183,7 +183,8 @@
                 for (int i = 0; i < MI; ++i) {
                     const uint4 v = fe3_bload16(rs_dagg, dgo[i], (unsigned)(j * 64));
                     dg[slot][i] = make_float4(__uint_as_float(v.x), __uint_as_float(v.y), __uint_as_float(v.z), __uint_as_float(v.w));
-                    dq[slot][i] = fe4_ldq(&d2f[FE_FOFF(i, j)]);
+                    if constexpr (D8) dq[slot][i] = make_uint2(__builtin_nontemporal_load((const uint32_t*)d2f + FE_FOFF(i, j) / 4), 0u);
+                    else dq[slot][i] = fe4_ldq(&d2f[FE_FOFF(i, j)]);
                 }
             };
             if (FE4_E3_DB) fetch_block(0, 0);
@@ -195,8 +196,11 @@
                 for (int i = 0; i < MI; ++i) {
                     const float4 g4 = dg[FE4_E3_DB ? (j & 1) : 0][i];
                     const uint2 dd = dq[FE4_E3_DB ? (j & 1) : 0][i];
-                    const fe_f2 p01 = (fe_f2{acc[i][j][0], acc[i][j][1]} + fe_f2{g4.x, g4.y} * dgk[i]) * fe3_unpack(dd.x);
-                    const fe_f2 p23 = (fe_f2{acc[i][j][2], acc[i][j][3]} + fe_f2{g4.z, g4.w} * dgk[i]) * fe3_unpack(dd.y);
+                    fe_f2 s01, s23;
+                    if constexpr (D8) fe_d8_unpack(dd.x, dsc, s01, s23);
+                    else { s01 = fe3_unpack(dd.x); s23 = fe3_unpack(dd.y); }
+                    const fe_f2 p01 = (fe_f2{acc[i][j][0], acc[i][j][1]} + fe_f2{g4.x, g4.y} * dgk[i]) * s01;
+                    const fe_f2 p23 = (fe_f2{acc[i][j][2], acc[i][j][3]} + fe_f2{g4.z, g4.w} * dgk[i]) * s23;
                     a2a += p01; a2b += p23;
                     *(uint2*)&sX[FE_QOFF(i, j)] = make_uint2(fe3_pack(p01), fe3_pack(p23));
                 }
@@ -260,9 +264,8 @@
                 fe_f2 dot2 = fe_f2{0.f, 0.f};
 #pragma unroll
                 for (int k = 0; k < 4; ++k) {
-                    const fe_f2 z = fe3_unpack(ua[k]) + fe3_unpack(ub[k]) + wv2[k] * rh;
                     fe_f2 m, d;
-                    fe3_silu_pair(z, m, d);
+                    fe_pre1_silu_pair(ua[k], ub[k], wv2[k], rh, m, d);
                     const fe_f2 g = fe3_unpack(ug[k]) * d;
                     dot2 += g * wv2[k];
                     po[k] = fe3_pack(m);
@@ -271,7 +274,7 @@
                 *sp = make_uint4(pg[0], pg[1], pg[2], pg[3]);
                 const unsigned goff = (unsigned)(e * H + ch * 8) * 2;
                 if (!(xf & 2)) {
-                    __builtin_amdgcn_raw_buffer_store_b128(fe_u32x4_t{po[0], po[1], po[2], po[3]}, rs_s1, (int)goff, 0,  2);
+                    if constexpr (!S1IN) __builtin_amdgcn_raw_buffer_store_b128(fe_u32x4_t{po[0], po[1], po[2], po[3]}, rs_s1, (int)goff, 0,  2);
                     __builtin_amdgcn_raw_buffer_store_b128(fe_u32x4_t{pg[0], pg[1], pg[2], pg[3]}, rs_p1, (int)goff, 0,  2);
                 }
                 float dot = dot2.x + dot2.y;
@@ -316,23 +319,32 @@
 static int g_fe_bwd4_exp = 0;
 extern "C" void fabind_gcl_edge_fused_bwd4_set_exp(int m) { g_fe_bwd4_exp = m; }
 
-int fe_bwd4_launch(const FabindEdgeBwdArgs* a, int H, int n_groups, hipStream_t stream) {
+int fe_bwd4_launch(const FabindEdgeBwdArgs* a, int H, int n_groups, hipStream_t stream, bool s1_given, bool d2_u8) {
     FB_REQUIRE(a->bnd != nullptr, "fabind_gcl_edge_fused_bwd: bnd (ceil(E / 64) x 2 x H floats of scratch) is required");
+    FB_REQUIRE(!s1_given || a->S1 != nullptr, "fabind_gcl_edge_fused_bwd_tiles: S1 (saved by fabind_gcl_edge_fused_train_tiles) is required");
     FB_REQUIRE(a->lddagg % 4 == 0 && ((uintptr_t)a->dagg & 15) == 0, "fabind_gcl_edge_fused_bwd: dagg must be 16-byte aligned with lddagg % 4 == 0");
     const size_t lds = (size_t)FE_BM * H * 2 + (size_t)8 * FE_BM * sizeof(int) + (size_t)4 * H * sizeof(float);
-#define FE_LAUNCH4(HH)                                                                                                \
+    const uint32_t thr16 = (uint32_t)(a->p_drop * 65536.0f + 0.5f);
+    const float dscale = 1.0f / (1.0f - (float)thr16 / 65536.0f);
+#define FE_LAUNCH4_(HH, SS, DD)                                                                                        \
     do {                                                                                                           \
         static bool set_ = false;                                                                                  \
         if (!set_) {                                                                                               \
-            const hipError_t e_ = hipFuncSetAttribute((const void*)gcl_edge_fused_bwd4_kernel<HH>,                    \
+            const hipError_t e_ = hipFuncSetAttribute((const void*)gcl_edge_fused_bwd4_kernel<HH, SS, DD>,            \
                                                       hipFuncAttributeMaxDynamicSharedMemorySize, (int)lds);       \
             if (e_ != hipSuccess) { fabind_set_error(hipGetErrorString(e_)); return (int)e_; }                     \
             set_ = true;                                                                                           \
         }                                                                                                          \
-        hipLaunchKernelGGL((gcl_edge_fused_bwd4_kernel<HH>), dim3(n_groups), dim3(HH), lds, stream, *a, g_fe_bwd4_exp); \
+        hipLaunchKernelGGL((gcl_edge_fused_bwd4_kernel<HH, SS, DD>), dim3(n_groups), dim3(HH), lds, stream, *a, g_fe_bwd4_exp, dscale); \
+    } while (0)
+#define FE_LAUNCH4(HH)                                                                                               \
+    do {                                                                                                           \
+        if (s1_given) { if (d2_u8) FE_LAUNCH4_(HH, true, true); else FE_LAUNCH4_(HH, true, false); }               \
+        else { if (d2_u8) FE_LAUNCH4_(HH, false, true); else FE_LAUNCH4_(HH, false, false); }                      \
     } while (0)
     if (H == 512) FE_LAUNCH4(512); else if (H == 256) FE_LAUNCH4(256); else if (H == 128) FE_LAUNCH4(128); else FE_LAUNCH4(64);
 #undef FE_LAUNCH4
+#undef FE_LAUNCH4_
     hipLaunchKernelGGL((fe_boundary_fix_kernel<64>), dim3((a->E + 63) / 64), dim3(H < 256 ? H : 256), 0, stream, a->row, a->E, H,
                        a->bnd, a->dAB16 ? nullptr : a->dABrow, (unsigned)a->lddab, (bf16_t*)a->dAB16, (unsigned)a->lddab16);
     FB_CHECK_LAUNCH();
diff --git a/fabind_amd/csrc/fused_edge_fwd2.hip b/fabind_amd/csrc/fused_edge_fwd2.hip
--- a/fabind_amd/csrc/fused_edge_fwd2.hip
+++ b/fabind_amd/csrc/fused_edge_fwd2.hip
@@ -31,7 +31,7 @@
 #endif
 }
 
-template <int H, bool DROP, bool SAVE>
+template <int H, bool DROP, int SAVE>
 __global__ __launch_bounds__(H, 4) void gcl_edge_fused2_kernel(const bf16_t* __restrict__ AB, int ldab, const int* __restrict__ row,
                                                             const int* __restrict__ col, const float* __restrict__ rhohat,
                                                             const float* __restrict__ w_r, const bf16_t* __restrict__ W2p,
@@ -39,7 +39,7 @@
                                                             const float* __restrict__ bc, const float* __restrict__ w3, int E,
                                                             float* agg, float* s_out, uint32_t thr16, float dscale,
                                                             uint32_t seed, float* bnd, bf16_t* agg16, int xcd_aware,
-                                                            bf16_t* __restrict__ Msave, bf16_t* __restrict__ d2f, bf16_t* __restrict__ z3f) {
+                                                            bf16_t* __restrict__ Msave, bf16_t* __restrict__ d2f, bf16_t* __restrict__ z3f, bf16_t* __restrict__ S1save) {
     constexpr int BM = FE_BM, MI = BM / 16;
     constexpr int NW = H / 64;
     constexpr int CH = H / 8;
@@ -94,11 +94,28 @@
             const float rh = sRh[e];
             uint32_t po[4];
 #pragma unroll
-            for (int k = 0; k < 4; ++k) po[k] = fw_pack(fw_silu_pair(fw_unpack(ga[u][k]) + fw_unpack(gb[u][k]) + wv2[k] * rh));
+            for (int k = 0; k < 4; ++k) {
+                fw_f2 m, d;
+                fe_pre1_silu_pair(ga[u][k], gb[u][k], wv2[k], rh, m, d);
+                po[k] = fw_pack(m);
+            }
             *(uint4*)&sX[e * H + ((ch ^ (e & SWZ)) * 8)] = e < ne ? make_uint4(po[0], po[1], po[2], po[3]) : make_uint4(0u, 0u, 0u, 0u);
         }
     }
     __syncthreads();
+    if constexpr (SAVE != 0) {
+        if (S1save) {
+            const __amdgpu_buffer_rsrc_t rs_s = fe_rsrc(S1save + (size_t)e0 * H, (unsigned)ne * H * 2);
+            int t_ = tid;
+            if constexpr (H < 512) asm volatile("" : "+v"(t_));
+#pragma unroll
+            for (int q = t_; q < BM * CH; q += H) {
+                const int rw = q / CH, c8 = q % CH;
+                const uint4 v = *(const uint4*)&sX[rw * H + ((c8 ^ (rw & SWZ)) * 8)];
+                __builtin_amdgcn_raw_buffer_store_b128(fe_u32x4_t{v.x, v.y, v.z, v.w}, rs_s, (int)((rw * H + c8 * 8) * 2), 0,  2);
+            }
+        }
+    }
 
     const int cx = (wave * 8 + (cq >> 1)) ^ (fr & SWZ);
     const int lbase = fr * H + (cq & 1) * 4;
@@ -120,7 +137,8 @@
 #pragma unroll
         for (int i = 0; i < MI; ++i) {
             fw_f2 m01, m23, d01, d23;
-            if constexpr (SAVE) {
+            bool kp0 = true, kp1 = true, kp2 = true, kp3 = true;
+            if constexpr (SAVE != 0) {
                 fw_silu_pair_d(fw_f2{acc[i][j][0], acc[i][j][1]} + b01, m01, d01);
                 fw_silu_pair_d(fw_f2{acc[i][j][2], acc[i][j][3]} + b23, m23, d23);
             } else {
@@ -132,15 +150,17 @@
                 const fw_f2 k01 = fw_f2{fe_keep(seed, ee, cc, H, thr16, dscale), fe_keep(seed, ee, cc + 1, H, thr16, dscale)};
                 const fw_f2 k23 = fw_f2{fe_keep(seed, ee, cc + 2, H, thr16, dscale), fe_keep(seed, ee, cc + 3, H, thr16, dscale)};
                 m01 *= k01; m23 *= k23;
-                if constexpr (SAVE) { d01 *= k01; d23 *= k23; }
+                if constexpr (SAVE == 1) { d01 *= k01; d23 *= k23; }
+                if constexpr (SAVE == 2) { kp0 = k01.x != 0.f; kp1 = k01.y != 0.f; kp2 = k23.x != 0.f; kp3 = k23.y != 0.f; }
             }
             *(uint2*)&sX[FW_QOFF(i, j)] = make_uint2(fw_pack(m01), fw_pack(m23));
-            if constexpr (SAVE) fw_stq(&d2f[FW_FOFF(i, j)], fw_pack(d01), fw_pack(d23));
+            if constexpr (SAVE == 1) fw_stq(&d2f[FW_FOFF(i, j)], fw_pack(d01), fw_pack(d23));
+            if constexpr (SAVE == 2) __builtin_nontemporal_store(fe_d8_pack(d01, d23, kp0, kp1, kp2, kp3), (uint32_t*)d2f + FW_FOFF(i, j) / 4);
         }
         __builtin_amdgcn_sched_barrier(0);
     }
     __syncthreads();
-    if constexpr (SAVE) {
+    if constexpr (SAVE != 0) {
         const __amdgpu_buffer_rsrc_t rs_m = fe_rsrc(Msave + (size_t)e0 * H, (unsigned)ne * H * 2);
 #pragma unroll
         for (int q = tid; q < BM * CH; q += H) {
@@ -171,7 +191,7 @@
                 const fw_f2 z01 = fw_f2{acc[i][j][0], acc[i][j][1]} + b01, z23 = fw_f2{acc[i][j][2], acc[i][j][3]} + b23;
                 da[i] += fw_silu_pair(z01) * w01;
                 db[i] += fw_silu_pair(z23) * w23;
-                if constexpr (SAVE) fw_stq(&z3f[FW_FOFF(i, j)], fw_pack(z01), fw_pack(z23));
+                if constexpr (SAVE != 0) fw_stq(&z3f[FW_FOFF(i, j)], fw_pack(z01), fw_pack(z23));
             }
             __builtin_amdgcn_sched_barrier(0);
         }
@@ -197,7 +217,7 @@
 int fe_fwd2_launch(const void* AB, int ldab, int H, const int* row, const int* col, const float* rhohat, const float* w_r,
                    const void* W2p, const float* b2, const void* Wcp, const float* bc, const float* w3, int E, float* agg,
                    float* s_out, uint32_t thr16, float dscale, unsigned seed, float* bnd, void* agg16, int xcd_aware, hipStream_t stream,
-                   void* Msave, void* d2f, void* z3f) {
+                   void* Msave, void* d2f, void* z3f, void* S1save, bool d2_u8) {
     const dim3 grid((((E + FE_BM - 1) / FE_BM + 7) / 8) * 8);
     const size_t lds = (size_t)FE_BM * H * 2 + 3 * FE_BM * sizeof(int) + (size_t)(H / 64) * FE_BM * sizeof(float);
 #define FW_LAUNCH_(HH, DD, SS)                                                                                       \
@@ -206,12 +226,13 @@
         if (!set_) { (void)hipFuncSetAttribute((const void*)gcl_edge_fused2_kernel<HH, DD, SS>, hipFuncAttributeMaxDynamicSharedMemorySize, (int)lds); set_ = true; } \
         hipLaunchKernelGGL((gcl_edge_fused2_kernel<HH, DD, SS>), grid, dim3(HH), lds, stream, (const bf16_t*)AB, ldab, row, col, rhohat, \
                            w_r, (const bf16_t*)W2p, b2, (const bf16_t*)Wcp, bc, w3, E, agg, s_out, thr16, dscale, \
-                           (uint32_t)seed, bnd, (bf16_t*)agg16, xcd_aware, (bf16_t*)Msave, (bf16_t*)d2f, (bf16_t*)z3f); \
+                           (uint32_t)seed, bnd, (bf16_t*)agg16, xcd_aware, (bf16_t*)Msave, (bf16_t*)d2f, (bf16_t*)z3f, (bf16_t*)S1save); \
     } while (0)
 #define FW_LAUNCH(HH)                                                                  \
     do {                                                                               \
-        if (Msave) { if (thr16) FW_LAUNCH_(HH, true, true); else FW_LAUNCH_(HH, false, true); } \
-        else { if (thr16) FW_LAUNCH_(HH, true, false); else FW_LAUNCH_(HH, false, false); }    \
+        if (Msave && d2_u8) { if (thr16) FW_LAUNCH_(HH, true, 2); else FW_LAUNCH_(HH, false, 2); } \
+        else if (Msave) { if (thr16) FW_LAUNCH_(HH, true, 1); else FW_LAUNCH_(HH, false, 1); } \
+        else { if (thr16) FW_LAUNCH_(HH, true, 0); else FW_LAUNCH_(HH, false, 0); }    \
     } while (0)
     if (H == 512) FW_LAUNCH(512); else if (H == 256) FW_LAUNCH(256); else if (H == 128) FW_LAUNCH(128); else FW_LAUNCH(64);
 #undef FW_LAUNCH
diff --git a/fabind_amd/csrc/fused_edge_fwd3.hip b/fabind_amd/csrc/fused_edge_fwd3.hip
--- a/fabind_amd/csrc/fused_edge_fwd3.hip
+++ b/fabind_amd/csrc/fused_edge_fwd3.hip
@@ -20,7 +20,7 @@
 typedef unsigned f3_u32x2_t __attribute__((ext_vector_type(2)));
 __device__ __forceinline__ void f3_stq(bf16_t* p_, uint32_t a, uint32_t b) { __builtin_nontemporal_store(f3_u32x2_t{a, b}, (f3_u32x2_t*)p_); }
 
-template <int H, bool DROP, bool SAVE>
+template <int H, bool DROP, int SAVE>
 __global__ __launch_bounds__(H, 2) void gcl_edge_fused_x3_kernel(const float* __restrict__ AB, int ldab, const int* __restrict__ row,
                                                               const int* __restrict__ col, const float* __restrict__ rhohat,
                                                               const float* __restrict__ w_r, const bf16_t* __restrict__ W2ph,
@@ -127,7 +127,8 @@
 #pragma unroll
         for (int i = 0; i < MI; ++i) {
             f3_f2 m01, m23, d01, d23;
-            if constexpr (SAVE) {
+            bool kp0 = true, kp1 = true, kp2 = true, kp3 = true;
+            if constexpr (SAVE != 0) {
                 f3_silu_pair_d(f3_f2{acc[i][j][0], acc[i][j][1]} + b01, m01, d01);
                 f3_silu_pair_d(f3_f2{acc[i][j][2], acc[i][j][3]} + b23, m23, d23);
             } else {
@@ -139,9 +140,11 @@
                 const f3_f2 k01 = f3_f2{fe_keep(seed, ee, cc, H, thr16, dscale), fe_keep(seed, ee, cc + 1, H, thr16, dscale)};
                 const f3_f2 k23 = f3_f2{fe_keep(seed, ee, cc + 2, H, thr16, dscale), fe_keep(seed, ee, cc + 3, H, thr16, dscale)};
                 m01 *= k01; m23 *= k23;
-                if constexpr (SAVE) { d01 *= k01; d23 *= k23; }
-            }
-            if constexpr (SAVE) f3_stq(&d2f[F3_FOFF(i, j)], f3_pack(d01), f3_pack(d23));
+                if constexpr (SAVE == 1) { d01 *= k01; d23 *= k23; }
+                if constexpr (SAVE == 2) { kp0 = k01.x != 0.f; kp1 = k01.y != 0.f; kp2 = k23.x != 0.f; kp3 = k23.y != 0.f; }
+            }
+            if constexpr (SAVE == 1) f3_stq(&d2f[F3_FOFF(i, j)], f3_pack(d01), f3_pack(d23));
+            if constexpr (SAVE == 2) __builtin_nontemporal_store(fe_d8_pack(d01, d23, kp0, kp1, kp2, kp3), (uint32_t*)d2f + F3_FOFF(i, j) / 4);
             uint32_t h01, l01, h23, l23;
             fe_split2(m01.x, m01.y, h01, l01);
             fe_split2(m23.x, m23.y, h23, l23);
@@ -151,7 +154,7 @@
         __builtin_amdgcn_sched_barrier(0);
     }
     __syncthreads();
-    if constexpr (SAVE) {
+    if constexpr (SAVE != 0) {
         const __amdgpu_buffer_rsrc_t rs_m = fe_rsrc(Msave + (size_t)e0 * H, (unsigned)ne * H * 2);
 #pragma unroll
         for (int q = tid; q < BM * CH; q += H) {
@@ -183,7 +186,7 @@
                 const f3_f2 z01 = f3_f2{acc[i][j][0], acc[i][j][1]} + b01, z23 = f3_f2{acc[i][j][2], acc[i][j][3]} + b23;
                 da[i] += f3_silu_pair(z01) * w01;
                 db[i] += f3_silu_pair(z23) * w23;
-                if constexpr (SAVE) f3_stq(&z3f[F3_FOFF(i, j)], f3_pack(z01), f3_pack(z23));
+                if constexpr (SAVE != 0) f3_stq(&z3f[F3_FOFF(i, j)], f3_pack(z01), f3_pack(z23));
             }
             __builtin_amdgcn_sched_barrier(0);
         }
@@ -209,7 +212,7 @@
 int fe_fwd3_launch(const float* AB, int ldab, int H, const int* row, const int* col, const float* rhohat, const float* w_r,
                    const void* W2ph, const void* W2pl, const float* b2, const void* Wcph, const void* Wcpl, const float* bc,
                    const float* w3, int E, float* agg, float* s_out, uint32_t thr16, float dscale, unsigned seed, float* bnd,
-                   int xcd_aware, hipStream_t stream, void* Msave, void* d2f, void* z3f) {
+                   int xcd_aware, hipStream_t stream, void* Msave, void* d2f, void* z3f, bool d2_u8) {
     const dim3 grid((((E + FE_BM - 1) / FE_BM + 7) / 8) * 8);
     const size_t lds = (size_t)2 * FE_BM * H * 2 + 3 * FE_BM * sizeof(int) + (size_t)(H / 64) * FE_BM * sizeof(float);
 #define F3_LAUNCH_(HH, DD, SS)                                                                                     \
@@ -222,8 +225,9 @@
     } while (0)
 #define F3_LAUNCH(HH)                                                                                              \
     do {                                                                                                           \
-        if (Msave) { if (thr16) F3_LAUNCH_(HH, true, true); else F3_LAUNCH_(HH, false, true); }                    \
-        else { if (thr16) F3_LAUNCH_(HH, true, false); else F3_LAUNCH_(HH, false, false); }                        \
+        if (Msave && d2_u8) { if (thr16) F3_LAUNCH_(HH, true, 2); else F3_LAUNCH_(HH, false, 2); }                 \
+        else if (Msave) { if (thr16) F3_LAUNCH_(HH, true, 1); else F3_LAUNCH_(HH, false, 1); }                     \
+        else { if (thr16) F3_LAUNCH_(HH, true, 0); else F3_LAUNCH_(HH, false, 0); }                                \
     } while (0)
     if (H == 512) F3_LAUNCH(512); else if (H == 256) F3_LAUNCH(256); else if (H == 128) F3_LAUNCH(128); else F3_LAUNCH(64);
 #undef F3_LAUNCH
diff --git a/fabind_amd/kernels.py b/fabind_amd/kernels.py
--- a/fabind_amd/kernels.py
+++ b/fabind_amd/kernels.py
@@ -516,12 +516,13 @@
     return pack_frag(hi), pack_frag(lo)
 
 
-def gcl_edge_fused_x3(AB, H, row, col, rhohat, w_r, W2, b2, Wc, bc, w3, n_rows, p_drop=0.0, seed=0, rowptr=None, save=False):
+def gcl_edge_fused_x3(AB, H, row, col, rhohat, w_r, W2, b2, Wc, bc, w3, n_rows, p_drop=0.0, seed=0, rowptr=None, save=False, d2_bits=16):
     E = row.shape[0]
+    assert d2_bits in (8, 16)
     if save and E > 0:
         nt = (E + 63) // 64
         Msave = torch.empty((E, H), dtype=torch.bfloat16, device=AB.device)
-        d2f = torch.empty((nt * 64, H), dtype=torch.bfloat16, device=AB.device)
+        d2f = torch.empty((nt * 64, H), dtype=torch.uint8 if d2_bits == 8 else torch.bfloat16, device=AB.device)
         z3f = torch.empty((nt * 64, H), dtype=torch.bfloat16, device=AB.device)
     else:
         save = False
@@ -537,11 +538,12 @@
     if save:
         _profiled("gcl_edge_fused_x3_kernel<%d> E=%d saving (gather + 2 chained H x H split-bf16 contractions + segment-sum per edge; M, silu'(pre2), pre3 kept)" % (H, E),
                   4.0 * E * H * H,
-                  lambda: check(_lib.load().fabind_gcl_edge_fused_x3_train(ptr(AB), _ld(AB), AB.shape[0], H, ptr(row), ptr(col), ptr(rhohat), ptr(w_r),
-                                                                           ptr(W2h), ptr(W2l), ptr(b2), ptr(Wch), ptr(Wcl), ptr(bc), ptr(w3), E,
-                                                                           ptr(agg), ptr(s), float(p_drop), int(seed) & 0xFFFFFFFF, ptr(bnd),
-                                                                           ptr(Msave), ptr(d2f), ptr(z3f), stream()), "fabind_gcl_edge_fused_x3_train"),
-                  E * (6.0 * H + 16) + n_rows * (8.0 * H + 4.0 * H),
+                  lambda: check(_lib.load().fabind_gcl_edge_fused_x3_train_tiles(ptr(AB), _ld(AB), AB.shape[0], H, ptr(row), ptr(col), ptr(rhohat), ptr(w_r),
+                                                                                 ptr(W2h), ptr(W2l), ptr(b2), ptr(Wch), ptr(Wcl), ptr(bc), ptr(w3), E,
+                                                                                 ptr(agg), ptr(s), float(p_drop), int(seed) & 0xFFFFFFFF, ptr(bnd),
+                                                                                 ptr(Msave), ptr(d2f), ptr(z3f), d2_bits, stream()),
+                                "fabind_gcl_edge_fused_x3_train_tiles"),
+                  E * ((5.0 if d2_bits == 8 else 6.0) * H + 16) + n_rows * (8.0 * H + 4.0 * H),
                   algo=2.0 * n_rows * H * 4 + E * 8.0 + n_rows * 24.0)
         return agg, s[:E], (Msave, d2f, z3f)
     _profiled("gcl_edge_fused_x3_kernel<%d> E=%d (gather + 2 chained H x H split-bf16 contractions + segment-sum per edge)" % (H, E),
@@ -561,13 +563,18 @@
                                              stream()), "fabind_zero_empty_rows")
 
 
-def gcl_edge_fused(AB16, H, row, col, rhohat, w_r, W2p, b2, Wcp, bc, w3, n_rows, p_drop=0.0, seed=0, want16=False, rowptr=None, save=False):
+def gcl_edge_fused(AB16, H, row, col, rhohat, w_r, W2p, b2, Wcp, bc, w3, n_rows, p_drop=0.0, seed=0, want16=False, rowptr=None, save=False,
+                   save_s1=False, d2_bits=16):
     E = row.shape[0]
+    assert d2_bits in (8, 16)
+    S1save = None
     if save and E > 0:
         nt = (E + 63) // 64
         Msave = torch.empty((E, H), dtype=torch.bfloat16, device=AB16.device)
-        d2f = torch.empty((nt * 64, H), dtype=torch.bfloat16, device=AB16.device)
+        d2f = torch.empty((nt * 64, H), dtype=torch.uint8 if d2_bits == 8 else torch.bfloat16, device=AB16.device)
         z3f = torch.empty((nt * 64, H), dtype=torch.bfloat16, device=AB16.device)
+        if save_s1:
+            S1save = torch.empty((E, H), dtype=torch.bfloat16, device=AB16.device)
     else:
         save, Msave, d2f, z3f = False, None, None, None
     alloc = torch.zeros if (rowptr is None or E == 0) else torch.empty
@@ -578,14 +585,15 @@
     s = torch.empty((max(E, 1), 1), dtype=torch.float32, device=AB16.device)
     bnd = torch.empty(((E + 63) // 64 * 2 + 2, H), dtype=torch.float32, device=AB16.device)
     if save:
-        _profiled("gcl_edge_fused_kernel<%d> E=%d saving (gather + 2 chained H x H contractions + segment-sum per edge; M, silu'(pre2), pre3 kept)" % (H, E),
+        head = (ptr(AB16), _ld(AB16), H, ptr(row), ptr(col), ptr(rhohat), ptr(w_r), ptr(W2p), ptr(b2), ptr(Wcp), ptr(bc), ptr(w3), E, ptr(agg), ptr(s),
+                float(p_drop), int(seed) & 0xFFFFFFFF, ptr(bnd), ptr(agg16), ptr(Msave), ptr(d2f), ptr(z3f))
+        _profiled("gcl_edge_fused_kernel<%d> E=%d saving (gather + 2 chained H x H contractions + segment-sum per edge; M, silu'(pre2), pre3%s kept)"
+                  % (H, E, ", S1" if S1save is not None else ""),
                   4.0 * E * H * H,
-                  lambda: check(_lib.load().fabind_gcl_edge_fused_train(ptr(AB16), _ld(AB16), H, ptr(row), ptr(col), ptr(rhohat), ptr(w_r),
-                                                                        ptr(W2p), ptr(b2), ptr(Wcp), ptr(bc), ptr(w3), E, ptr(agg), ptr(s),
-                                                                        float(p_drop), int(seed) & 0xFFFFFFFF, ptr(bnd), ptr(agg16),
-                                                                        ptr(Msave), ptr(d2f), ptr(z3f), stream()),
-                                "fabind_gcl_edge_fused_train"),
-                  E * (6.0 * H + 16) + n_rows * (4.0 * H + 4.0 * H + (2.0 * H if want16 else 0.0)),
+                  (lambda: check(_lib.load().fabind_gcl_edge_fused_train_tiles(*head, ptr(S1save), d2_bits, stream()), "fabind_gcl_edge_fused_train_tiles"))
+                  if (S1save is not None or d2_bits == 8) else
+                  (lambda: check(_lib.load().fabind_gcl_edge_fused_train(*head, stream()), "fabind_gcl_edge_fused_train")),
+                  E * ((8.0 if S1save is not None else 6.0) * H - (H if d2_bits == 8 else 0) + 16) + n_rows * (4.0 * H + 4.0 * H + (2.0 * H if want16 else 0.0)),
                   algo=2.0 * n_rows * H * 2 + E * 8.0 + n_rows * 24.0)
     else:
         _profiled("gcl_edge_fused_kernel<%d> E=%d (gather + 2 chained H x H contractions + segment-sum per edge)" % (H, E), 4.0 * E * H * H,
@@ -596,7 +604,9 @@
                   E * 16.0 + n_rows * (4.0 * H + 4.0 * H + (2.0 * H if want16 else 0.0)),
                   algo=2.0 * n_rows * H * 2 + E * 8.0 + n_rows * 24.0)
     out = (agg, s[:E], agg16) if want16 else (agg, s[:E])
-    return out + ((Msave, d2f, z3f),) if save else out
+    if save:
+        out = out + ((Msave, d2f, z3f) if S1save is None else (Msave, d2f, z3f, S1save),)
+    return out
 
 
 def edge_lnfold(AB16, Kp, H, row, col, rho, stat, eps, w_r, c_r, c_c, dvec, p_drop=0.0, seed=0):
@@ -726,7 +736,12 @@
         ng -= ng % 8
     d2scratch = torch.empty((2, ng, bm * H), dtype=torch.bfloat16, device=dev) if variant == 5 else None
     bnd = torch.empty(((E + bm - 1) // bm * 2 + 2, H), dtype=torch.float32, device=dev)
-    if variant == 6:
+    s1_given = variant == 6 and len(saved) == 4
+    d2_bits = 8 if (variant == 6 and saved[1].dtype == torch.uint8) else 16
+    if s1_given:
+        buf = torch.empty((3, max(E, 1), H), dtype=torch.bfloat16, device=dev)
+        S1, Mm, dT, dP2, dP1 = saved[3], saved[0], buf[0], buf[1], buf[2]
+    elif variant == 6:
         buf = torch.empty((4, max(E, 1), H), dtype=torch.bfloat16, device=dev)
         S1, Mm, dT, dP2, dP1 = buf[0], saved[0], buf[1], buf[2], buf[3]
     else:
@@ -758,9 +773,10 @@
     _profiled(("gcl_edge_fused_bwd4_kernel<%d> E=%d (2 chained H x H contractions per edge over the forward's saved tiles)" % (H, E)) if variant == 6 else
               "gcl_edge_fused_bwd%s_kernel<%d> E=%d (recompute + 4 chained H x H contractions per edge)" % ("3" if variant == 5 else "", H, E),
               (4.0 if variant == 6 else 8.0) * E * H * H,
-              lambda: check(_lib.load().fabind_gcl_edge_fused_bwd(ctypes.byref(a), H, ng, stream()),
-                            "fabind_gcl_edge_fused_bwd"),
-              E * ((12.0 if variant == 6 else 10.0) * H + 20) + N * (4.0 * H + 4.0 * H + (2.0 if dab_bf16 else 4.0) * H),
+              (lambda: check(_lib.load().fabind_gcl_edge_fused_bwd_tiles(ctypes.byref(a), H, ng, int(s1_given), d2_bits, stream()), "fabind_gcl_edge_fused_bwd_tiles"))
+              if (s1_given or d2_bits == 8) else
+              (lambda: check(_lib.load().fabind_gcl_edge_fused_bwd(ctypes.byref(a), H, ng, stream()), "fabind_gcl_edge_fused_bwd")),
+              E * ((10.0 if s1_given else 12.0 if variant == 6 else 10.0) * H - (H if d2_bits == 8 else 0) + 20) + N * (4.0 * H + 4.0 * H + (2.0 if dab_bf16 else 4.0) * H),
               algo=N * (2.0 * H * 2 + 4.0 * H + 2.0 * H * (2.0 if dab_bf16 else 4.0)) + E * 20.0)
     del keep
     if E > 0:
diff --git a/fabind_amd/ops.py b/fabind_amd/ops.py
--- a/fabind_amd/ops.py
+++ b/fabind_amd/ops.py
@@ -602,6 +602,8 @@
 
 EDGE_SAVE_FWD = _cfg.knob("FABIND_EDGE_SAVE_FWD")
 EDGE_SAVE_MIN_H = 256
+EDGE_FWD_S1 = True
+EDGE_D2_BITS = 8
 
 
 class _FusedEdge(torch.autograd.Function):
@@ -613,8 +615,8 @@
         E = g.row_ctx.shape[0]
         save = EDGE_SAVE_FWD and H >= EDGE_SAVE_MIN_H and E >= 1 and AB16.dtype == torch.bfloat16
         out = K.gcl_edge_fused(AB16, H, g.row_ctx, g.col_ctx, rhohat, w_r, W2p, b2, Wcp, bc, w3,
-                               AB16.shape[0], p_drop, seed, want16=holder is not None, rowptr=g.rp_ctx, save=save)
-        ctx.n_saved = 3 if save else 0
+                               AB16.shape[0], p_drop, seed, want16=holder is not None, rowptr=g.rp_ctx, save=save, save_s1=bool(save and EDGE_FWD_S1), d2_bits=EDGE_D2_BITS)
+        ctx.n_saved = len(out[-1]) if save else 0
         ctx.save_for_backward(AB16, rhohat, w_r, W2, b2, Wc, bc, w3, *(out[-1] if save else ()))
         if holder is not None:
             holder.append(out[2])
@@ -645,7 +647,7 @@
         E = g.row_ctx.shape[0]
         save = EDGE_SAVE_FWD and H >= EDGE_SAVE_MIN_H and E >= 1
         out = K.gcl_edge_fused_x3(AB, H, g.row_ctx, g.col_ctx, rhohat, w_r, W2, b2, Wc, bc, w3, AB.shape[0], p_drop, seed,
-                                  rowptr=g.rp_ctx, save=save)
+                                  rowptr=g.rp_ctx, save=save, d2_bits=EDGE_D2_BITS)
         ctx.n_saved = 3 if save else 0
         ctx.save_for_backward(AB, rhohat, w_r, W2, b2, Wc, bc, w3, *(out[2] if save else ()))
         return out[0], out[1]
diff --git a/include/fabind_hip.h b/include/fabind_hip.h
--- a/include/fabind_hip.h
+++ b/include/fabind_hip.h
@@ -145,6 +145,10 @@
                                    const float* w_r, const void* W2ph, const void* W2pl, const float* b2, const void* Wcph,
                                    const void* Wcpl, const float* bc, const float* w3, int E, float* agg, float* s_out, float p_drop,
                                    unsigned seed, float* bnd, void* M, void* d2f, void* z3f, hipStream_t stream);
+int fabind_gcl_edge_fused_x3_train_tiles(const float* AB, int ldab, int n_rows, int H, const int* row, const int* col, const float* rhohat,
+                                         const float* w_r, const void* W2ph, const void* W2pl, const float* b2, const void* Wcph,
+                                         const void* Wcpl, const float* bc, const float* w3, int E, float* agg, float* s_out, float p_drop,
+                                         unsigned seed, float* bnd, void* M, void* d2f, void* z3f, int d2_bits, hipStream_t stream);
 
 int fabind_gcl_edge_fused(const void* AB, int ldab, int H, const int* row, const int* col, const float* rhohat,
                           const float* w_r, const void* W2p, const float* b2, const void* Wcp, const float* bc,
@@ -157,6 +161,10 @@
                                 const float* w_r, const void* W2p, const float* b2, const void* Wcp, const float* bc,
                                 const float* w3, int E, float* agg, float* s_out, float p_drop, unsigned seed, float* bnd,
                                 void* agg16, void* M, void* d2f, void* z3f, hipStream_t stream);
+int fabind_gcl_edge_fused_train_tiles(const void* AB, int ldab, int H, const int* row, const int* col, const float* rhohat,
+                                      const float* w_r, const void* W2p, const float* b2, const void* Wcp, const float* bc,
+                                      const float* w3, int E, float* agg, float* s_out, float p_drop, unsigned seed, float* bnd,
+                                      void* agg16, void* M, void* d2f, void* z3f, void* S1, int d2_bits, hipStream_t stream);
 
 typedef struct FabindEdgeBwdArgs {
     const void* AB; const int* row; const int* col; const float* rhohat; const float* w_r;
@@ -177,6 +185,7 @@
     const void* z3f;
 } FabindEdgeBwdArgs;
 int fabind_gcl_edge_fused_bwd(const FabindEdgeBwdArgs* args, int H, int n_groups, hipStream_t stream);
+int fabind_gcl_edge_fused_bwd_tiles(const FabindEdgeBwdArgs* args, int H, int n_groups, int s1_given, int d2_bits, hipStream_t stream);
 int fabind_gcl_edge_fused_bwd_set_tile(int bm);
 int fabind_gcl_edge_fused_bwd_tile(void);
 int fabind_gcl_edge_fused_bwd_set_variant(int v);
```

Result: slower. 532.3 (-1.4%).
